# SurrealAI/surreal

Measured on AMD Instinct MI355X. Metric: env-steps/sec (learner ingest) PPO 1024 actors×128 steps, 1/2/4/8 MI355X, higher is better.
Workload: dtype f32

## Files before the change

### include/surreal_amd.h

```cpp
#ifndef SURREAL_AMD_H
#define SURREAL_AMD_H

#include <stddef.h>
#include <stdint.h>

#ifdef __cplusplus
extern "C" {
#endif

typedef void* smx_stream_t;

enum {
    SMX_OK = 0,
    SMX_E_NULL = -1,
    SMX_E_SHAPE = -2,
    SMX_E_UNSUPPORTED = -3,
    SMX_E_WORKSPACE = -4,
    SMX_E_ALIGN = -5
};

enum { SMX_ACT_NONE = 0, SMX_ACT_RELU = 1, SMX_ACT_TANH = 2 };
enum { SMX_PPO_CLIP = 0, SMX_PPO_ADAPT = 1 };

int smx_abi_version(void);
const char* smx_error_string(int code);

typedef struct {
    const float* W1; const float* b1;
    const float* W2; const float* b2;
    const float* W3; const float* b3;
    int32_t D, H1, H2, OUT;
} smx_mlp3_t;

int smx_zfilter_stats_f32(const float* running_sum, const float* running_sumsq,
                          const float* count, int32_t D, float eps,
                          float* mean_out, float* std_out, smx_stream_t stream);
int smx_zfilter_forward_f32(const float* x, int64_t ldx, int64_t rows, int32_t D,
                            const float* mean, const float* std, float* out,
                            smx_stream_t stream);
int smx_zfilter_forward_sums_f32(const float* x, int64_t ldx, int64_t rows, int32_t D,
                                 const float* running_sum, const float* running_sumsq,
                                 const float* count, float eps, float* out, smx_stream_t stream);
int smx_zfilter_update_f32(const float* x, int64_t ldx, int64_t rows, int32_t D,
                           float* running_sum, float* running_sumsq, float* count,
                           float count_rows, smx_stream_t stream);
int64_t smx_zfilter_update_ws_floats(int64_t rows, int32_t D);
int smx_zfilter_update_ws_f32(const float* x, int64_t ldx, int64_t rows, int32_t D, float* running_sum,
                              float* running_sumsq, float* count, float count_rows, float* ws, int64_t ws_floats,
                              smx_stream_t stream);

int smx_mlp3_fused_exact_zfilter(int32_t on);

size_t smx_mlp3_packed_bytes(int32_t D, int32_t H1, int32_t H2, int32_t OUT);
int smx_mlp3_pack_f32(const smx_mlp3_t* net, float* packed, size_t packed_bytes,
                      smx_stream_t stream);
int smx_mlp3_pack_zstats_f32(const smx_mlp3_t* net, float* packed, size_t packed_bytes,
                             const float* running_sum, const float* running_sumsq, const float* count,
                             int32_t D, float eps, float* mean_out, float* std_out, smx_stream_t stream);
int smx_mlp3_forward_fused_f32(const float* packed, int32_t D, int32_t H1, int32_t H2,
                               int32_t OUT, const float* x_main, const float* x_tail,
                               int64_t G, int32_t T0, int32_t T1, const float* zmean,
                               const float* zstd, float* out, int32_t out_act,
                               smx_stream_t stream);

int smx_linear_f32(const float* A, int32_t lda, int32_t a_kcontig, const float* B,
                   int32_t ldb, int32_t b_kcontig, const float* bias, float* C,
                   int32_t ldc, int32_t M, int32_t N, int32_t K, int32_t act,
                   const float* relu_mask, const int32_t* stop_flag, smx_stream_t stream);

typedef struct smx_linear_job {
    int32_t kind, act;
    const float* A; const float* B; const float* bias; const float* relu_mask;
    float* C; float* dbias;
    int32_t lda, ldb, ldc, a_kcontig, b_kcontig, M, N, K;
    const int32_t* stop_flag;
} smx_linear_job_t;
int smx_linear_multi_f32(const smx_linear_job_t* jobs, int32_t njobs, smx_stream_t stream);

int smx_linear_wgrad_f32(const float* dZ, int32_t ldz, const float* X, int32_t ldx, float* dW,
                         int32_t ldw, float* db, int32_t M, int32_t N, int32_t rows,
                         smx_stream_t stream);

int64_t smx_linear_wgrad_ws_floats(int32_t M, int32_t N, int32_t rows);
int smx_linear_wgrad_splitk_f32(const float* dZ, int32_t ldz, const float* X, int32_t ldx,
                                float* dW, int32_t ldw, float* db, int32_t M, int32_t N,
                                int32_t rows, float* ws, int64_t ws_floats, smx_stream_t stream);
int smx_linear_wgrad_splitk_pair_f32(const float* dZ, int32_t ldz, int32_t M, int32_t rows, const float* X1,
                                     int32_t ldx1, float* dW1, float* db1, int32_t N1, const float* X2,
                                     int32_t ldx2, float* dW2, float* db2, int32_t N2, float* ws,
                                     int64_t ws_floats, smx_stream_t stream);

typedef struct {
    const smx_mlp3_t* net;
    const float* x;
    int64_t rows;
    float* h1;
    float* h2;
    float* out;
    int32_t out_act;
    int32_t out_ld;
    const float* dz3;
    float* dz2;
    float* dz1;
    float* grads;
    float* sumsq_partials;
    const int32_t* stop_flag;
    float* h1T;
    float* h2T;
    const float* xT;
    const float* dz3T;
    float* dz2T;
    float* dz1T;
    int64_t ldT;
} smx_mlp3_job_t;
int smx_mlp3_forward_multi_f32(const smx_mlp3_job_t* jobs, int32_t njobs, smx_stream_t stream);
int smx_mlp3_backward_multi_f32(const smx_mlp3_job_t* jobs, int32_t njobs, smx_stream_t stream);

int smx_mlp3_forward_f32(const smx_mlp3_t* net, const float* x, int64_t rows, float* h1,
                         float* h2, float* out, int32_t out_act,
                         const int32_t* stop_flag, smx_stream_t stream);
int32_t smx_mlp3_forward_rows_supported(int32_t D, int32_t H1, int32_t H2, int32_t OUT);
int smx_mlp3_forward_rows_f32(const smx_mlp3_t* net, const float* x, int64_t rows, float* h1, float* h2,
                              float* out, int32_t out_act, int32_t out_ld, float* packed, size_t packed_bytes,
                              const int32_t* stop_flag, smx_stream_t stream);

int32_t smx_mlp3_backward_partials(int32_t D, int32_t H1, int32_t H2, int32_t OUT);
int smx_mlp3_backward_f32(const smx_mlp3_t* net, const float* x, const float* h1,
                          const float* h2, const float* dz3, int64_t rows, float* dz2,
                          float* dz1, float* grads, float* sumsq_partials,
                          const int32_t* stop_flag, smx_stream_t stream);
int64_t smx_mlp3_backward_ws_floats(int32_t D, int32_t H1, int32_t H2, int32_t OUT, int64_t rows);
int smx_mlp3_backward_splitk_f32(const smx_mlp3_t* net, const float* x, const float* h1, const float* h2,
                                 const float* dz3, int64_t rows, float* dz2, float* dz1, float* grads, float* ws,
                                 int64_t ws_floats, const int32_t* stop_flag, smx_stream_t stream);
int32_t smx_mlp3_dgrad_rows_supported(int32_t D, int32_t H1, int32_t H2, int32_t OUT);
int64_t smx_mlp3_dgrad_rows_ws_floats(int32_t D, int32_t H1, int32_t H2, int32_t OUT);
int smx_mlp3_backward_rows_f32(const smx_mlp3_t* net, const float* x, const float* h1, const float* h2,
                               const float* dz3, int64_t rows, float* dz2, float* dz1, float* dx, float* grads,
                               float* ws, int64_t ws_floats, float* packedT, int64_t packedT_floats,
                               const int32_t* stop_flag, smx_stream_t stream);

int smx_windowed_gae_returns_f32(const float* values, const float* values_tail,
                                 const float* rewards,
                                 const float* dones, const float* gamma_pow,
                                 const float* lam_pow, float gamma, float gamma_H,
                                 int32_t B, int32_t N, int32_t H, float* adv, float* ret,
// ... 74 lines not shown
    const float* actions;
    const float* behave;
    const float* ref;
    const float* adv;
    int32_t ld_act, ld_beh, ld_ref, check_stop;
    int64_t rows;
    float* g_surr;
    float* g_kl;
    float* row_partials;
    float* dz3;
    float* dz3_t;
    int64_t ld_t;
    float* dlogvar;
    float* dlogvar_sumsq;
    float* stats;
    const float* values;
    const float* returns;
    float* v_dz3;
    float* v_partials;
    int32_t will_update, v_will_update;
} smx_ppo_losses_t;
int smx_ppo_epoch_losses_f32(const smx_ppo_losses_t* args, smx_ppo_ctrl_t* ctrl,
                             smx_stream_t stream);
int smx_ppo_epoch_losses_dp_f32(const smx_ppo_losses_t* args, int64_t n_total, float* g_surr_t,
                                float* g_kl_t, smx_ppo_ctrl_t* ctrl, smx_stream_t stream);
typedef struct smx_ppo_combine {
    int32_t mode, A;
    const float* row_partials;
    int32_t nblk;
    int32_t check_stop;
    int64_t n_total;
    const float* log_var;
    float* stats;
    float* grads_a;
    const float* grads_kl;
    int64_t n_mlp, n_a;
    float* sumsq_a;
    const float* grads_c;
    int64_t n_c;
    float* sumsq_c;
    int32_t will_update, reserved;
} smx_ppo_combine_t;
int smx_ppo_epoch_combine_f32(const smx_ppo_combine_t* args, smx_ppo_ctrl_t* ctrl,
                              smx_stream_t stream);
int smx_mlp3_wgrad_multi_f32(const smx_mlp3_job_t* jobs, int32_t njobs, smx_stream_t stream);

enum { SMX_EPOCH_LOSS_NONE = 0, SMX_EPOCH_LOSS_POLICY = 1, SMX_EPOCH_LOSS_VALUE = 2, SMX_EPOCH_RHS_SURR = 3,
       SMX_EPOCH_RHS_KL = 4 };
typedef struct smx_epoch_job {
    const smx_mlp3_t* net;
    const float* x;
    int64_t rows;
    float* h1T;
    float* h2T;
    int64_t ldT;
    float* out;
    int32_t out_ld;
    int32_t out_act;
    int32_t loss;
    int32_t reserved;
    const int32_t* stop_flag;
    const float* dz3;
    float* dz3T;
    float* dz2T;
    float* dz1T;
    const float* packed;
} smx_epoch_job_t;
typedef struct smx_epoch_pack {
    const smx_mlp3_t* net;
    float* packed;
} smx_epoch_pack_t;
int64_t smx_epoch_packed_floats(int32_t D, int32_t H1, int32_t H2, int32_t OUT);
int smx_epoch_pack_f32(const smx_epoch_pack_t* items, int32_t n, smx_stream_t stream);
typedef struct smx_epoch_prep {
    const float* obs0; int64_t ld_obs0; int64_t rows; int32_t D; int32_t A;
    const float* zmean; const float* zstd;
    float* xn; float* xnT; int64_t ldT;
    const float* ref_sum; const float* ref_sumsq; const float* ref_count; float ref_eps; int32_t ref_filter;
    float* xr;
    const float* obs_next; int64_t ld_next; float* xnext;
    const float* ref_log_var; float* ref_std; int64_t ld_ref;
    int32_t* zero_words; int32_t n_zero; int32_t n_pack;
    smx_epoch_pack_t pack[4];
} smx_epoch_prep_t;
int smx_epoch_prepare_f32(const smx_epoch_prep_t* args, smx_stream_t stream);
struct smx_ppo_losses;
int32_t smx_epoch_blocks(int64_t rows);
int32_t smx_epoch_supported(int32_t D, int32_t H1, int32_t H2, int32_t OUT);
int smx_epoch_forward_f32(const smx_epoch_job_t* jobs, int32_t njobs, const struct smx_ppo_losses* loss,
                          smx_ppo_ctrl_t* ctrl, int64_t n_total, smx_stream_t stream);
int smx_epoch_backward_f32(const smx_epoch_job_t* jobs, int32_t njobs, const struct smx_ppo_losses* loss,
                           smx_ppo_ctrl_t* ctrl, int64_t n_total, smx_stream_t stream);
int32_t smx_epoch_fwdbwd_supported(int32_t D, int32_t H1, int32_t H2, int32_t OUT);
int smx_epoch_fwdbwd_f32(const smx_epoch_job_t* jobs, int32_t njobs, const struct smx_ppo_losses* loss,
                         smx_ppo_ctrl_t* ctrl, int64_t n_total, int32_t* sync_word, uint64_t* kl_slots,
                         smx_stream_t stream);
int smx_device_occupy(int32_t blocks, int64_t microseconds, smx_stream_t stream);

int smx_diaggauss_sample_f32(const float* mean, int64_t ld_mean, const float* log_var,
                             const float* noise_scale, const float* eps, int64_t ld_eps,
                             int64_t rows, int32_t A, float* actions, int64_t ld_act, float* pd,
                             int64_t ld_pd, smx_stream_t stream);
int smx_ppo_final_stats_f32(const float* log_var, int32_t A, const float* running_sum,
                            const float* running_sumsq, const float* count, int32_t D, float* out4,
                            smx_stream_t stream);
int smx_value_loss_finalize_f32(const float* partials, int32_t count, int32_t nblk,
                                float* stats, int32_t stats_stride, smx_stream_t stream);

int smx_clip_adam_step_f32(float* theta, const float* grads, float* exp_avg,
                           float* exp_avg_sq, int64_t n, const float* sumsq_partials,
                           int32_t npart, const smx_ppo_ctrl_t* ctrl, int32_t which,
                           int32_t honour_stop, float* grad_norm_out, smx_stream_t stream);
typedef struct smx_adam_group {
    float* theta;
    const float* grads;
    float* exp_avg;
    float* exp_avg_sq;
    int64_t n;
    const float* sumsq_partials;
    int32_t npart;
    int32_t honour_stop;
    float* grad_norm_out;
    const smx_mlp3_t* pack_net;
    float* packed;
} smx_adam_group_t;
int smx_clip_adam_step_group_f32(const smx_adam_group_t* group, int32_t which, const smx_ppo_ctrl_t* ctrl,
                                 smx_stream_t stream);
int smx_clip_adam_step_pair_f32(const smx_adam_group_t* actor, const smx_adam_group_t* critic,
                                const smx_ppo_ctrl_t* ctrl, smx_stream_t stream);
int32_t smx_sumsq_blocks(int64_t n);
int smx_sumsq_partials_f32(const float* x, int64_t n, float* partials, smx_stream_t stream);

int smx_ring_insert_f32(float* table, int64_t capacity, int32_t width, int64_t cursor,
                        const float* src, int64_t n, smx_stream_t stream);
int smx_gather_rows_f32(const float* table, int64_t capacity, int32_t width,
                        const int64_t* idx, int64_t n, float* dst, smx_stream_t stream);
int smx_uniform_indices(int64_t* idx, int64_t n, int64_t len, uint64_t seed,
                        uint64_t offset, smx_stream_t stream);
int smx_philox4x32_10(const uint32_t* ctr_key, int64_t n, uint32_t* out, smx_stream_t stream);
typedef struct {
    const void* table;
    void* dst;
    int64_t row_bytes;
} smx_gather_job_t;
int smx_uniform_gather_multi(const smx_gather_job_t* jobs, int32_t njobs, int64_t capacity, int64_t rows,
                             const int64_t* idx, int64_t len, uint64_t seed, uint64_t offset, int64_t* idx_out,
                             smx_stream_t stream);

int smx_ring_insert_bytes(void* table, int64_t capacity, int64_t row_bytes, int64_t cursor,
                          const void* src, int64_t n, smx_stream_t stream);
int smx_gather_rows_bytes(const void* table, int64_t capacity, int64_t row_bytes, const int64_t* idx,
                          int64_t n, void* dst, smx_stream_t stream);

int smx_window_emit_f32(const float* src, int32_t actors, int32_t T, int32_t width,
                        int32_t start, int32_t n_step, int32_t stride, int32_t W, float* dst,
                        smx_stream_t stream);
int smx_window_emit_bytes(const void* src, int32_t actors, int32_t T, int64_t row_bytes, int32_t start,
                          int32_t n_step, int32_t stride, int32_t W, void* dst, smx_stream_t stream);

int smx_frame_stack_u8(const void* frames, int32_t actors, int32_t R, int64_t frame_bytes, int32_t n_stack,
                       const int32_t* episode_first, int32_t start, int32_t n_step, int32_t stride, int32_t W,
                       void* dst, smx_stream_t stream);
int smx_synth_frame_u8(const float* s0, int64_t ld_s0, int32_t n, int32_t C, int32_t H, int32_t W, int32_t t,
                       void* dst, int64_t ld_dst, smx_stream_t stream);

int smx_synth_env_step_f32(float* state, const float* init_state, const float* actions,
// ... 197 lines not shown
```

### surreal_amd/_lib.py

```python
import ctypes
import os
from ctypes import (POINTER, Structure, c_char_p, c_double, c_float, c_int32, c_int64, c_size_t,
                    c_uint64, c_void_p)

_HERE = os.path.dirname(os.path.abspath(__file__))
LIB_PATH = os.environ.get('SMX_LIB_PATH') or os.path.join(_HERE, 'libsurreal_amd.so')

SMX_ACT_NONE, SMX_ACT_RELU, SMX_ACT_TANH = 0, 1, 2
SMX_PPO_CLIP, SMX_PPO_ADAPT = 0, 1
SMX_E_UNSUPPORTED = -3
PS_SURR, PS_LOSS, PS_ENTROPY, PS_KL, PS_GRADNORM, PS_LB, PS_ISW, PS_REFBEH, PS_STRIDE = range(9)
VS_LOSS, VS_EXPVAR, VS_GRADNORM = 0, 1, 2
VS_STRIDE = 4


class Mlp3(Structure):
    _fields_ = [('W1', c_void_p), ('b1', c_void_p), ('W2', c_void_p), ('b2', c_void_p),
                ('W3', c_void_p), ('b3', c_void_p),
                ('D', c_int32), ('H1', c_int32), ('H2', c_int32), ('OUT', c_int32)]


class Mlp3Job(Structure):
    _fields_ = [('net', POINTER(Mlp3)), ('x', c_void_p), ('rows', c_int64), ('h1', c_void_p),
                ('h2', c_void_p), ('out', c_void_p), ('out_act', c_int32), ('out_ld', c_int32),
                ('dz3', c_void_p), ('dz2', c_void_p), ('dz1', c_void_p), ('grads', c_void_p),
                ('sumsq_partials', c_void_p), ('stop_flag', c_void_p),
                ('h1T', c_void_p), ('h2T', c_void_p), ('xT', c_void_p), ('dz3T', c_void_p),
                ('dz2T', c_void_p), ('dz1T', c_void_p), ('ldT', c_int64)]


class EpochJob(Structure):
    _fields_ = [('net', POINTER(Mlp3)), ('x', c_void_p), ('rows', c_int64), ('h1T', c_void_p),
                ('h2T', c_void_p), ('ldT', c_int64), ('out', c_void_p), ('out_ld', c_int32),
                ('out_act', c_int32), ('loss', c_int32), ('reserved', c_int32), ('stop_flag', c_void_p),
                ('dz3', c_void_p), ('dz3T', c_void_p), ('dz2T', c_void_p), ('dz1T', c_void_p),
                ('packed', c_void_p)]


class EpochPack(Structure):
    _fields_ = [('net', POINTER(Mlp3)), ('packed', c_void_p)]


class LearnEpilogue(Structure):
    _fields_ = [('x', c_void_p), ('ldx', c_int64), ('rows', c_int64), ('D', c_int32), ('A', c_int32),
                ('running_sum', c_void_p), ('running_sumsq', c_void_p), ('count', c_void_p), ('count_rows', c_float),
                ('n_epochs', c_int32), ('ret', c_void_p), ('n_ret', c_int64), ('ret_moments', c_void_p),
                ('v_partials', c_void_p), ('nblk', c_int32), ('stats_stride', c_int32), ('v_stats', c_void_p),
                ('log_var', c_void_p), ('out4', c_void_p), ('ticket', c_void_p)]


class EpochPrep(Structure):
    _fields_ = [('obs0', c_void_p), ('ld_obs0', c_int64), ('rows', c_int64), ('D', c_int32), ('A', c_int32),
                ('zmean', c_void_p), ('zstd', c_void_p), ('xn', c_void_p), ('xnT', c_void_p), ('ldT', c_int64),
                ('ref_sum', c_void_p), ('ref_sumsq', c_void_p), ('ref_count', c_void_p), ('ref_eps', c_float),
                ('ref_filter', c_int32), ('xr', c_void_p), ('obs_next', c_void_p), ('ld_next', c_int64),
                ('xnext', c_void_p), ('ref_log_var', c_void_p), ('ref_std', c_void_p), ('ld_ref', c_int64),
                ('zero_words', c_void_p), ('n_zero', c_int32), ('n_pack', c_int32), ('pack', EpochPack * 4)]


EPOCH_LOSS_NONE, EPOCH_LOSS_POLICY, EPOCH_LOSS_VALUE, EPOCH_RHS_SURR, EPOCH_RHS_KL = 0, 1, 2, 3, 4


class Lstm(Structure):
    _fields_ = [('W_ih', c_void_p), ('W_hh', c_void_p), ('b_ih', c_void_p), ('b_hh', c_void_p),
                ('D', c_int32), ('H', c_int32)]


class AdamGroup(Structure):
    _fields_ = [('theta', c_void_p), ('grads', c_void_p), ('exp_avg', c_void_p),
                ('exp_avg_sq', c_void_p), ('n', c_int64), ('sumsq_partials', c_void_p),
                ('npart', c_int32), ('honour_stop', c_int32), ('grad_norm_out', c_void_p),
                ('pack_net', POINTER(Mlp3)), ('packed', c_void_p)]


class PpoLosses(Structure):
    _fields_ = [('mode', c_int32), ('A', c_int32), ('mean', c_void_p), ('log_var', c_void_p),
                ('actions', c_void_p), ('behave', c_void_p), ('ref', c_void_p), ('adv', c_void_p),
                ('ld_act', c_int32), ('ld_beh', c_int32), ('ld_ref', c_int32), ('check_stop', c_int32),
                ('rows', c_int64), ('g_surr', c_void_p), ('g_kl', c_void_p),
                ('row_partials', c_void_p), ('dz3', c_void_p), ('dz3_t', c_void_p), ('ld_t', c_int64),
                ('dlogvar', c_void_p), ('dlogvar_sumsq', c_void_p), ('stats', c_void_p),
                ('values', c_void_p), ('returns', c_void_p), ('v_dz3', c_void_p),
                ('v_partials', c_void_p), ('will_update', c_int32), ('v_will_update', c_int32)]


class PpoCombine(Structure):
    _fields_ = [('mode', c_int32), ('A', c_int32), ('row_partials', c_void_p), ('nblk', c_int32),
                ('check_stop', c_int32), ('n_total', c_int64), ('log_var', c_void_p),
                ('stats', c_void_p), ('grads_a', c_void_p), ('grads_kl', c_void_p),
                ('n_mlp', c_int64), ('n_a', c_int64), ('sumsq_a', c_void_p), ('grads_c', c_void_p),
                ('n_c', c_int64), ('sumsq_c', c_void_p), ('will_update', c_int32),
                ('reserved', c_int32)]


class LinearJob(Structure):
    _fields_ = [('kind', c_int32), ('act', c_int32), ('A', c_void_p), ('B', c_void_p), ('bias', c_void_p),
                ('relu_mask', c_void_p), ('C', c_void_p), ('dbias', c_void_p), ('lda', c_int32), ('ldb', c_int32),
                ('ldc', c_int32), ('a_kcontig', c_int32), ('b_kcontig', c_int32), ('M', c_int32), ('N', c_int32),
                ('K', c_int32), ('stop_flag', c_void_p)]


class DdpgNet(Structure):
    _fields_ = [(n, c_void_p) for n in ('W1', 'b1', 'W2', 'b2', 'W3', 'b3')]


class DdpgUpdate(Structure):
    _fields_ = ([(n, c_void_p) for n in ('theta', 'grads', 'exp_avg', 'exp_avg_sq', 'target')] + [('n', c_int64)] +
                [(n, c_void_p) for n in ('lr', 'step')] +
                [(n, c_float) for n in ('weight_decay', 'clip_value', 'tau')] + [('interval', c_int32), ('stats', c_void_p), ('stats_host', c_void_p)])


class DdpgRows(Structure):
    _fields_ = ([('rows', c_int64)] + [(n, c_int32) for n in ('D', 'A', 'H1', 'H2', 'c1', 'c2')] +
                [(n, DdpgNet) for n in ('actor', 'critic', 'target_actor', 'target_critic')] +
                [(n, c_void_p) for n in ('packed', 'x', 'x_next', 'actions', 'rewards', 'dones')] +
                [('gamma_n', c_float)] +
                [(n, c_void_p) for n in ('xcat', 'h2c', 'q', 'q_next', 'y', 'dz3', 'dz2', 'dxcat', 'h1a', 'h2a', 'act',
                                         'q_actor', 'dz3a', 'dz2a', 'dz1a', 'step')])


class GatherJob(Structure):
    _fields_ = [('table', c_void_p), ('dst', c_void_p), ('row_bytes', c_int64)]


class SynthRollout(Structure):
    _fields_ = [('net', POINTER(Mlp3)), ('packed', c_void_p), ('out_act', c_int32), ('n', c_int32),
                ('log_var', c_void_p), ('noise_scale', c_void_p), ('eps', c_void_p), ('zsum', c_void_p),
                ('zsumsq', c_void_p), ('zcount', c_void_p), ('zeps', c_float), ('t', c_int32),
                ('episode_len', c_int32), ('steps', c_int32), ('rows_per_actor', c_int32), ('slot', c_int32),
                ('state', c_void_p), ('init_state', c_void_p), ('obs_roll', c_void_p), ('act_roll', c_void_p),
                ('rew_roll', c_void_p), ('done_roll', c_void_p), ('pd_roll', c_void_p), ('obs_last', c_void_p)]


class Xchg(Structure):
    _fields_ = [('world', c_int32), ('rank', c_int32), ('capacity', c_int64), ('peer', c_void_p * 8)]


class SynthActStep(Structure):
    _fields_ = [('state', c_void_p), ('init_state', c_void_p), ('mean', c_void_p), ('log_var', c_void_p),
                ('noise_scale', c_void_p), ('eps', c_void_p), ('ld_mean', c_int64), ('ld_eps', c_int64),
                ('n', c_int32), ('D', c_int32), ('A', c_int32), ('t', c_int32), ('episode_len', c_int32),
                ('slot', c_int32), ('T', c_int32), ('reserved', c_int32),
                ('obs_roll', c_void_p), ('act_roll', c_void_p), ('rew_roll', c_void_p),
                ('done_roll', c_void_p), ('pd_roll', c_void_p), ('zsum', c_void_p), ('zsumsq', c_void_p),
                ('zcount', c_void_p), ('zeps', c_float), ('reserved_f', c_float), ('xn_out', c_void_p)]


CTRL_WORDS = 16
(C_LR_ACTOR, C_LR_CRITIC, C_BETA, C_ETA, C_CLIP_EPS, C_KL_TARGET, C_ACTOR_MAX_NORM,
 C_CRITIC_MAX_NORM, C_ACTOR_WD, C_CRITIC_WD, C_STEP_ACTOR, C_STEP_CRITIC, C_STOP,
 C_EPOCHS_DONE) = range(14)
C_XCHG_ERR = 14
C_SYNC_ERR = 15

_P = c_void_p
_SIGS = {
    'smx_abi_version': (c_int32, []),
    'smx_error_string': (c_char_p, [c_int32]),
    'smx_zfilter_stats_f32': (c_int32, [_P, _P, _P, c_int32, c_float, _P, _P, _P]),
    'smx_zfilter_forward_f32': (c_int32, [_P, c_int64, c_int64, c_int32, _P, _P, _P, _P]),
    'smx_zfilter_forward_sums_f32': (c_int32, [_P, c_int64, c_int64, c_int32, _P, _P, _P, c_float, _P, _P]),
    'smx_diaggauss_sample_f32': (c_int32, [_P, c_int64, _P, _P, _P, c_int64, c_int64, c_int32, _P,
                                           c_int64, _P, c_int64, _P]),
    'smx_zfilter_update_f32': (c_int32, [_P, c_int64, c_int64, c_int32, _P, _P, _P, c_float, _P]),
    'smx_mlp3_packed_bytes': (c_size_t, [c_int32, c_int32, c_int32, c_int32]),
    'smx_mlp3_pack_f32': (c_int32, [POINTER(Mlp3), _P, c_size_t, _P]),
    'smx_mlp3_pack_zstats_f32': (c_int32, [POINTER(Mlp3), _P, c_size_t, _P, _P, _P, c_int32, c_float, _P, _P, _P]),
    'smx_mlp3_fused_exact_zfilter': (c_int32, [c_int32]),
    'smx_mlp3_forward_fused_f32': (c_int32, [_P, c_int32, c_int32, c_int32, c_int32, _P, _P,
                                             c_int64, c_int32, c_int32, _P, _P, _P, c_int32, _P]),
    'smx_linear_f32': (c_int32, [_P, c_int32, c_int32, _P, c_int32, c_int32, _P, _P, c_int32,
                                 c_int32, c_int32, c_int32, c_int32, _P, _P, _P]),
    'smx_linear_wgrad_f32': (c_int32, [_P, c_int32, _P, c_int32, _P, c_int32, _P, c_int32, c_int32,
                                       c_int32, _P]),
    'smx_mlp3_forward_f32': (c_int32, [POINTER(Mlp3), _P, c_int64, _P, _P, _P, c_int32, _P, _P]),
    'smx_mlp3_forward_multi_f32': (c_int32, [POINTER(Mlp3Job), c_int32, _P]),
    'smx_mlp3_backward_multi_f32': (c_int32, [POINTER(Mlp3Job), c_int32, _P]),
    'smx_mlp3_wgrad_multi_f32': (c_int32, [POINTER(Mlp3Job), c_int32, _P]),
    'smx_epoch_blocks': (c_int32, [c_int64]),
    'smx_epoch_supported': (c_int32, [c_int32, c_int32, c_int32, c_int32]),
    'smx_epoch_packed_floats': (c_int64, [c_int32, c_int32, c_int32, c_int32]),
    'smx_epoch_pack_f32': (c_int32, [POINTER(EpochPack), c_int32, _P]),
    'smx_epoch_prepare_f32': (c_int32, [POINTER(EpochPrep), _P]),
    'smx_epoch_forward_f32': (c_int32, [POINTER(EpochJob), c_int32, POINTER(PpoLosses), _P, c_int64, _P]),
    'smx_epoch_backward_f32': (c_int32, [POINTER(EpochJob), c_int32, POINTER(PpoLosses), _P, c_int64, _P]),
    'smx_epoch_fwdbwd_supported': (c_int32, [c_int32, c_int32, c_int32, c_int32]),
    'smx_epoch_fwdbwd_f32': (c_int32, [POINTER(EpochJob), c_int32, POINTER(PpoLosses), _P, c_int64, _P, _P, _P]),
    'smx_device_occupy': (c_int32, [c_int32, c_int64, _P]),
    'smx_layernorm_forward_f32': (c_int32, [_P, c_int64, c_int64, c_int32, _P, _P, c_float, _P, c_int64, _P, _P, _P]),
    'smx_layernorm_backward_ws_floats': (c_int64, [c_int64, c_int32]),
    'smx_layernorm_backward_f32': (c_int32, [_P, c_int64, _P, c_int64, _P, _P, _P, c_int64, c_int32, c_int32, _P, c_int64, _P, _P,
                                             _P, c_int64, _P]),
    'smx_zfilter_update_ws_floats': (c_int64, [c_int64, c_int32]),
    'smx_zfilter_update_ws_f32': (c_int32, [_P, c_int64, c_int64, c_int32, _P, _P, _P, c_float, _P, c_int64, _P]),
    'smx_ppo_partials_fold_f32': (c_int32, [_P, c_int32, c_int32, _P, c_int32, _P, _P]),
    'smx_mlp3_forward_rows_supported': (c_int32, [c_int32, c_int32, c_int32, c_int32]),
    'smx_mlp3_forward_rows_f32': (c_int32, [POINTER(Mlp3), _P, c_int64, _P, _P, _P, c_int32, c_int32, _P, c_size_t, _P, _P]),
    'smx_mlp3_backward_partials': (c_int32, [c_int32, c_int32, c_int32, c_int32]),
    'smx_mlp3_backward_f32': (c_int32, [POINTER(Mlp3), _P, _P, _P, _P, c_int64, _P, _P, _P, _P,
                                        _P, _P]),
    'smx_mlp3_backward_ws_floats': (c_int64, [c_int32, c_int32, c_int32, c_int32, c_int64]),
    'smx_mlp3_backward_splitk_f32': (c_int32, [POINTER(Mlp3), _P, _P, _P, _P, c_int64, _P, _P, _P, _P, c_int64, _P, _P]),
    'smx_mlp3_dgrad_rows_supported': (c_int32, [c_int32, c_int32, c_int32, c_int32]),
    'smx_mlp3_dgrad_rows_ws_floats': (c_int64, [c_int32, c_int32, c_int32, c_int32]),
    'smx_mlp3_backward_rows_f32': (c_int32, [POINTER(Mlp3), _P, _P, _P, _P, c_int64, _P, _P, _P, _P, _P, c_int64, _P, c_int64,
                                             _P, _P]),
    'smx_windowed_gae_returns_f32': (c_int32, [_P, _P, _P, _P, _P, _P, c_float, c_float, c_int32,
                                               c_int32, c_int32, _P, _P, _P]),
    'smx_windowed_gae_norm_f32': (c_int32, [_P, _P, _P, _P, _P, _P, c_float, c_float, c_int32, c_int32, c_int32, _P, _P, _P,
                                            c_float, _P, _P]),
    'smx_ppo_learn_epilogue_f32': (c_int32, [POINTER(LearnEpilogue), _P]),
    'smx_reward_filter_f32': (c_int32, [_P, c_int64, c_float, c_int32, _P, c_float, c_int32, _P, _P, _P, _P, _P]),
    'smx_reward_filter_partials': (c_int32, []),
    'smx_moments_f32': (c_int32, [_P, c_int64, _P, _P]),
    'smx_moments_merge_f32': (c_int32, [_P, c_int32, _P, _P]),
    'smx_adv_normalize_f32': (c_int32, [_P, c_int64, _P, c_float, _P]),
    'smx_ppo_loss_blocks': (c_int32, [c_int64]),
    'smx_ppo_loss_partial_stride': (c_int32, [c_int32]),
    'smx_ppo_policy_loss_f32': (c_int32, [c_int32, _P, _P, _P, c_int32, _P, c_int32, _P, c_int32,
                                          _P, c_int64, c_int32, _P, _P, _P, _P, _P]),
    'smx_ppo_loss_finalize_f32': (c_int32, [c_int32, _P, c_int32, _P, _P, _P, c_int64, c_int64,
                                            c_int32, _P, c_int32, c_int32, _P, _P, c_int64, _P, _P,
                                            _P, _P]),
    'smx_ppo_epoch_losses_f32': (c_int32, [POINTER(PpoLosses), _P, _P]),
    'smx_ppo_epoch_losses_dp_f32': (c_int32, [POINTER(PpoLosses), c_int64, _P, _P, _P, _P]),
    'smx_ppo_epoch_combine_f32': (c_int32, [POINTER(PpoCombine), _P, _P]),
    'smx_ppo_final_stats_f32': (c_int32, [_P, c_int32, _P, _P, _P, c_int32, _P, _P]),
    'smx_value_loss_blocks': (c_int32, [c_int64]),
    'smx_value_loss_f32': (c_int32, [_P, _P, c_int64, c_int64, _P, _P, _P, c_int32, _P]),
    'smx_value_loss_finalize_f32': (c_int32, [_P, c_int32, c_int32, _P, c_int32, _P]),
    'smx_clip_adam_step_f32': (c_int32, [_P, _P, _P, _P, c_int64, _P, c_int32, _P, c_int32,
                                         c_int32, _P, _P]),
    'smx_clip_adam_step_group_f32': (c_int32, [POINTER(AdamGroup), c_int32, _P, _P]),
    'smx_clip_adam_step_pair_f32': (c_int32, [POINTER(AdamGroup), POINTER(AdamGroup), _P, _P]),
    'smx_sumsq_blocks': (c_int32, [c_int64]),
    'smx_sumsq_partials_f32': (c_int32, [_P, c_int64, _P, _P]),
    'smx_synth_act_env_step_head_f32': (c_int32, [POINTER(SynthActStep), _P, _P, _P, c_int64, c_int32, c_int32, _P]),
    'smx_conv_u8_forward_f32': (c_int32, [_P, c_int64, c_int32, c_int32, c_int32, c_int32, c_int32, _P, _P, c_int32,
                                          _P, _P, _P]),
    'smx_conv_u8_wgrad_ws_floats': (c_int64, [c_int32, c_int32]),
    'smx_conv_u8_wgrad_f32': (c_int32, [_P, c_int64, c_int32, c_int32, c_int32, c_int32, c_int32, _P, c_int32, _P, _P, _P,
                                        c_int64, _P, _P]),
    'smx_conv_cl_forward_f32': (c_int32, [_P, c_int64, c_int32, c_int32, c_int32, c_int32, c_int32, _P, _P, c_int32,
                                          _P, _P, _P]),
    'smx_conv_cl_wgrad_ws_floats': (c_int64, [c_int32, c_int32]),
    'smx_conv_cl_wgrad_f32': (c_int32, [_P, c_int64, c_int32, c_int32, c_int32, c_int32, c_int32, _P, c_int32, _P, _P, _P,
                                        c_int64, _P, _P]),
    'smx_conv_cl_dgrad_f32': (c_int32, [_P, c_int64, c_int32, c_int32, c_int32, c_int32, c_int32, _P, c_int32, _P, _P,
                                        _P, _P]),
    'smx_ring_insert_bytes': (c_int32, [_P, c_int64, c_int64, c_int64, _P, c_int64, _P]),
    'smx_gather_rows_bytes': (c_int32, [_P, c_int64, c_int64, _P, c_int64, _P, _P]),
    'smx_window_emit_bytes': (c_int32, [_P, c_int32, c_int32, c_int64, c_int32, c_int32, c_int32, c_int32, _P, _P]),
    'smx_ring_insert_f32': (c_int32, [_P, c_int64, c_int32, c_int64, _P, c_int64, _P]),
# ... 124 lines not shown
```

### surreal_amd/csrc/smx_epoch.hip

```cpp
#include "smx_common.h"
#include <stdlib.h>
#include <string.h>

#define SMX_LDS_BARRIER() asm volatile("s_waitcnt lgkmcnt(0)\n\ts_barrier" ::: "memory")

namespace {
#include "smx_ppo_loss.inc.h"
#include "smx_epoch_pack.inc.h"
#include "smx_epoch_mma.inc.h"

constexpr int TB = 3;
constexpr int MAX_EJOBS = 4;
constexpr int XV = 7;
constexpr int LIN = 6;
constexpr int LINF = 3;
constexpr int EXCLUSIVE_LDS = 84 * 1024;
constexpr int LDZ = 68;
constexpr int LDO = 36;
static_assert(ER == LOSS_ROWS_PER_BLOCK, "a row block is a loss block");
static_assert(NTH == 256, "the shared loss code strides by 256 threads");

#ifdef SMX_EPOCH_TIMING
#define TSTAMP(i) do { if (G.tbuf && threadIdx.x == 0) G.tbuf[(size_t)ts_blk * 32 + (i)] = (long long)__builtin_readcyclecounter(); } while (0)
#else
#define TSTAMP(i) do { } while (0)
#endif
struct EJob {
    const float *W1, *b1, *W2, *b2, *W3, *b3;
    int D, H1, H2, OUT;
    const float* x;
    int rows;
    float *h1T, *h2T;
    long ldT;
    float* out;
    int out_ld, out_act, loss, blk_base;
    const int* stop;
    const float* dz3;
    float *dz3T, *dz2T, *dz1T;
    const float *P1, *P2, *P3, *P2T, *P3T;
};

struct PolArgs {
    int mode, A;
    const float *log_var, *actions, *behave, *ref, *adv;
    int ld_act, ld_beh, ld_ref, check_stop, will_update;
    float *g_surr, *g_kl, *row_partials;
    float *dlogvar, *dlogvar_sumsq, *stats;
};

struct ValArgs {
    const float* returns;
    float *v_dz3, *v_partials;
    int will_update;
};

struct EArgs {
    EJob j[MAX_EJOBS];
    int n;
    PolArgs pl;
    ValArgs vl;
    long n_total;
    int ldx, ldh1, ldh2, off_h1, off_h2, off_out, off_red, off_loss;
    int off_g;
    int* sync;
    int nb_pol;
    const int* pol_stop;
    unsigned long long* kl_slots;
    int fsplit;
    int xsplit;
    long long* tbuf;
};

__device__ __forceinline__ int xcd_job_order(const EArgs& G, int raw) {
    const int nb = G.xsplit;
    if (nb == 0) return raw;
    const int xcd = raw & 7, slot = raw >> 3;
    return (xcd >> 2) * nb + slot * 4 + (xcd & 3);
}

__device__ __forceinline__ EJob select_job(const EArgs& G, int bid) {
    int pi = 0;
#pragma unroll
    for (int k = 1; k < MAX_EJOBS; ++k) pi += (k < G.n && bid >= G.j[k].blk_base) ? 1 : 0;
// ... 627 lines not shown
#pragma unroll
            for (int g = 0; g < TB; ++g) {
                if (g < nt) {
                    const int f0 = 16 * (t0 + ts * g) + 4 * kq;
                    float4 v;
                    v.x = (mk[g][0] > 0.f) ? acc[g][0] : 0.f;
                    v.y = (mk[g][1] > 0.f) ? acc[g][1] : 0.f;
                    v.z = (mk[g][2] > 0.f) ? acc[g][2] : 0.f;
                    v.w = (mk[g][3] > 0.f) ? acc[g][3] : 0.f;
                    if (out_lds) *(float4*)(out_lds + fm * ldh2 + f0) = v;
                    const bool ok = outT != nullptr && f0 < M && fm < nrows;
                    const unsigned o = ((unsigned)f0 * (unsigned)J.ldT + (unsigned)(row0 + fm)) * 4u, st = (unsigned)J.ldT * 4u;
                    __builtin_amdgcn_raw_buffer_store_b32(__float_as_uint(v.x), rout, ok ? o : OOB, 0, 0);
                    __builtin_amdgcn_raw_buffer_store_b32(__float_as_uint(v.y), rout, ok ? o + st : OOB, 0, 0);
                    __builtin_amdgcn_raw_buffer_store_b32(__float_as_uint(v.z), rout, ok ? o + 2 * st : OOB, 0, 0);
                    __builtin_amdgcn_raw_buffer_store_b32(__float_as_uint(v.w), rout, ok ? o + 3 * st : OOB, 0, 0);
                }
            }
        }
        TSTAMP(10 + 4 * l);
        SMX_LDS_BARRIER();
        TSTAMP(4 + l);
    }
}

inline int r64(int v) { return (v + 63) & ~63; }

struct PackNet {
    const float *W1, *W2, *W3;
    float* packed;
    int D, H1, H2, OUT;
    long base;
};
struct PackArgs {
    PackNet n[MAX_EJOBS];
    int count;
    long total;
};

__device__ __forceinline__ void pack_word(const PackArgs& P, long i) {
    int pi = 0;
#pragma unroll
    for (int k = 1; k < MAX_EJOBS; ++k) pi += (k < P.count && i >= P.n[k].base) ? 1 : 0;
    const PackNet N = P.n[pi];
    long w = i - N.base;
    int bn = 0;
#pragma unroll
    for (int k = 1; k < 5; ++k) bn += (w >= pack_off(N.D, N.H1, N.H2, N.OUT, k)) ? 1 : 0;
    w -= pack_off(N.D, N.H1, N.H2, N.OUT, bn);
    const float* W = bn == 0 ? N.W1 : ((bn == 1 || bn == 3) ? N.W2 : N.W3);
    const bool tr = bn >= 3;
    const int M = bn == 0 ? N.H1 : (bn == 1 ? N.H2 : (bn == 2 ? N.OUT : (bn == 3 ? N.H1 : N.H2)));
    const int K = bn == 0 ? N.D : (bn == 1 ? N.H1 : (bn == 2 ? N.H2 : (bn == 3 ? N.H2 : N.OUT)));
    const int C2 = pack_chunks(K);
    const int lane = (int)(w & 63), half = (int)((w >> 6) & 1);
    const long tc = w >> 7;
    const int c = (int)(tc % C2), t = (int)(tc / C2);
    const int m = 16 * t + (lane & 15), k = 32 * c + 8 * (lane >> 4) + 4 * half;
    float v[4] = {0.f, 0.f, 0.f, 0.f};
    if (m < M) {
#pragma unroll
        for (int r = 0; r < 4; ++r)
            if (k + r < K) v[r] = tr ? W[(size_t)(k + r) * M + m] : W[(size_t)m * K + k + r];
    }
    *(float4*)(N.packed + 4 * (i - N.base)) = make_float4(v[0], v[1], v[2], v[3]);
}

__global__ __launch_bounds__(256) void epoch_pack_kernel(PackArgs P) {
    const long i = (long)blockIdx.x * 256 + threadIdx.x;
    if (i < P.total) pack_word(P, i);
}

struct PrepArgs {
    const float* obs0; long ld_obs0; long rows; int D;
    const float *zmean, *zstd;
    float *xn, *xnT; long ldT;
    const float *rsum, *rsumsq, *rcount; float reps; int ref_filter;
    float* xr;
    const float* obs_next; long ld_next; float* xnext;
    const float* ref_log_var; int A; float* ref_std; long ld_ref;
    int* zero_words; int n_zero;
    PackArgs pack;
    long n_x, n_std;
};

__device__ __forceinline__ float zclamp_e(float x, float m, float sdev) {
    float v = (x - m) / sdev;
    if (v == v) v = fminf(fmaxf(v, -5.0f), 5.0f);
    return v;
}

__global__ __launch_bounds__(256) void epoch_prepare_kernel(PrepArgs P) {
    const long tid0 = (long)blockIdx.x * 256 + threadIdx.x, stride = (long)gridDim.x * 256;
    for (long i = tid0; i < P.n_zero; i += stride) P.zero_words[i] = 0;
    const long nx = P.n_x, n_next = P.xnext ? nx : 0;
    const long total = 2 * nx + n_next + P.n_std + P.pack.total;
    for (long i = tid0; i < total; i += stride) {
        if (i < 2 * nx + n_next) {
            const int which = i < nx ? 0 : (i < 2 * nx ? 1 : 2);
            const long e = i - (which == 0 ? 0 : (which == 1 ? nx : 2 * nx));
            const long r = e / P.D;
            const int k = (int)(e - r * P.D);
            const float x = which == 2 ? P.obs_next[r * P.ld_next + k] : P.obs0[r * P.ld_obs0 + k];
            float v = x;
            if (which == 1) {
                if (P.ref_filter) {
                    const float c = P.rcount[0];
                    const float m = P.rsum[k] / c;
                    const float var = P.rsumsq[k] / c - m * m;
                    float sd = sqrtf(var);
                    if (sd == sd) sd = fmaxf(sd, P.reps);
                    v = zclamp_e(x, m, sd);
                }
                P.xr[e] = v;
            } else {
                if (P.zmean) v = zclamp_e(x, P.zmean[k], P.zstd[k]);
                if (which == 0) {
                    P.xn[e] = v;
                    if (P.xnT) P.xnT[(size_t)k * P.ldT + r] = v;
                } else {
                    P.xnext[e] = v;
                }
            }
        } else if (i < 2 * nx + n_next + P.n_std) {
            const long e = i - (2 * nx + n_next);
            const long r = e / P.A;
            const int a = (int)(e - r * P.A);
            P.ref_std[r * P.ld_ref + a] = expf(P.ref_log_var[a]);
        } else {
            pack_word(P.pack, i - (2 * nx + n_next + P.n_std));
        }
    }
}

long long* g_tbuf = nullptr;

}

extern "C" int64_t smx_epoch_packed_floats(int32_t D, int32_t H1, int32_t H2, int32_t OUT) {
    return 4 * pack_off(D, H1, H2, OUT, 5);
}

static int fill_pack(PackArgs& P, const smx_epoch_pack_t* items, int32_t n) {
    SMX_REQUIRE(items, SMX_E_NULL);
    SMX_REQUIRE(n >= 1 && n <= MAX_EJOBS, SMX_E_SHAPE);
    P.count = n;
    long base = 0;
    for (int k = 0; k < n; ++k) {
        SMX_REQUIRE(items[k].net && items[k].packed, SMX_E_NULL);
        const smx_mlp3_t& m = *items[k].net;
        SMX_REQUIRE(m.D > 0 && m.H1 > 0 && m.H2 > 0 && m.OUT > 0, SMX_E_SHAPE);
        SMX_REQUIRE(((uintptr_t)items[k].packed & 15) == 0, SMX_E_ALIGN);
        P.n[k].W1 = m.W1; P.n[k].W2 = m.W2; P.n[k].W3 = m.W3; P.n[k].packed = items[k].packed;
        P.n[k].D = m.D; P.n[k].H1 = m.H1; P.n[k].H2 = m.H2; P.n[k].OUT = m.OUT;
        P.n[k].base = base;
        base += smx_epoch_packed_floats(m.D, m.H1, m.H2, m.OUT) / 4;
    }
    P.total = base;
    return SMX_OK;
}

extern "C" int smx_epoch_pack_f32(const smx_epoch_pack_t* items, int32_t n, smx_stream_t stream) {
    PackArgs P;
    const int rc = fill_pack(P, items, n);
    if (rc) return rc;
    hipLaunchKernelGGL(epoch_pack_kernel, dim3((unsigned)((P.total + 255) / 256)), dim3(256), 0, smx_s(stream), P);
    SMX_LAUNCH_CHECK();
    return SMX_OK;
}

extern "C" int smx_epoch_prepare_f32(const smx_epoch_prep_t* a, smx_stream_t stream) {
    SMX_REQUIRE(a && a->obs0 && a->xn && a->xr, SMX_E_NULL);
    SMX_REQUIRE(a->rows > 0 && a->D > 0 && a->ld_obs0 >= a->D, SMX_E_SHAPE);
    SMX_REQUIRE((a->zmean == nullptr) == (a->zstd == nullptr), SMX_E_NULL);
    SMX_REQUIRE(!a->xnT || a->ldT >= a->rows, SMX_E_SHAPE);
    SMX_REQUIRE(!a->ref_filter || (a->ref_sum && a->ref_sumsq && a->ref_count), SMX_E_NULL);
    SMX_REQUIRE(!a->xnext || (a->obs_next && a->ld_next >= a->D), SMX_E_SHAPE);
    SMX_REQUIRE(!a->ref_std || (a->ref_log_var && a->A > 0 && a->ld_ref >= a->A), SMX_E_SHAPE);
    SMX_REQUIRE(a->n_zero >= 0 && a->n_zero <= (1 << 20) && (a->n_zero == 0 || a->zero_words), SMX_E_SHAPE);
    PrepArgs P;
    memset(&P, 0, sizeof(P));
    P.obs0 = a->obs0; P.ld_obs0 = (long)a->ld_obs0; P.rows = (long)a->rows; P.D = a->D;
    P.zmean = a->zmean; P.zstd = a->zstd; P.xn = a->xn; P.xnT = a->xnT; P.ldT = (long)a->ldT;
    P.rsum = a->ref_sum; P.rsumsq = a->ref_sumsq; P.rcount = a->ref_count; P.reps = a->ref_eps;
    P.ref_filter = a->ref_filter; P.xr = a->xr;
    P.obs_next = a->obs_next; P.ld_next = (long)a->ld_next; P.xnext = a->xnext;
    P.ref_log_var = a->ref_log_var; P.A = a->A; P.ref_std = a->ref_std; P.ld_ref = (long)a->ld_ref;
    P.zero_words = a->zero_words; P.n_zero = a->n_zero;
    P.n_x = P.rows * P.D;
    P.n_std = a->ref_std ? P.rows * a->A : 0;
    P.pack.count = 0; P.pack.total = 0;
    if (a->n_pack > 0) {
        const int rc = fill_pack(P.pack, a->pack, a->n_pack);
        if (rc) return rc;
    }
    const long total = 2 * P.n_x + (P.xnext ? P.n_x : 0) + P.n_std + P.pack.total;
    long blocks = (total + 255) / 256;
    if (blocks > 4096) blocks = 4096;
    hipLaunchKernelGGL(epoch_prepare_kernel, dim3((unsigned)blocks), dim3(256), 0, smx_s(stream), P);
    SMX_LAUNCH_CHECK();
    return SMX_OK;
}

extern "C" void smx_epoch_debug_tbuf(void* p) { g_tbuf = (long long*)p; }

extern "C" int32_t smx_epoch_blocks(int64_t rows) { return (int32_t)((rows + ER - 1) / ER); }

static int fwd_lds_bytes(int D, int H1, int H2, int A) {
    const int floats = ER * (r64(D) + 4) + ER * (r64(H1) + 4) + ER * (r64(H2) + 4) + ER * LDO + NWV * 2 * 256 +
                       loss_scratch_floats(A) + ER * (5 * A + 1);
    return floats * (int)sizeof(float);
}
static int fb_loss_floats(int A) {
    const int a = loss_scratch_floats(A) + ER * (5 * A + 1), b = FIN_CH * (8 + 2 * A);
    return a > b ? a : b;
}
static int fb_lds_bytes(int D, int H1, int H2, int A) {
    const int floats = ER * (r64(D) + 4) + ER * (r64(H1) + 4) + ER * (r64(H2) + 4) + ER * LDO + 2 * ER * LDZ +
                       ER * (r64(H2) + 4) + NWV * 2 * 256 + fb_loss_floats(A);
    return floats * (int)sizeof(float);
}
constexpr int MAX_LDS = 128 * 1024;

extern "C" int32_t smx_epoch_supported(int32_t D, int32_t H1, int32_t H2, int32_t OUT) {
    return D > 0 && H1 > 0 && H2 > 0 && OUT > 0 && H1 % 4 == 0 && H2 % 4 == 0 && OUT <= 32 &&
           D <= 2048 && H1 <= 16 * NWV * TG * 2 && H2 <= 16 * NWV * TG * 2 &&
           fwd_lds_bytes(D, H1, H2, OUT) <= MAX_LDS;
}

extern "C" int32_t smx_epoch_fwdbwd_supported(int32_t D, int32_t H1, int32_t H2, int32_t OUT) {
    return smx_epoch_supported(D, H1, H2, OUT) && H2 <= 16 * FNWV * FTG && fb_lds_bytes(D, H1, H2, OUT) <= MAX_LDS;
}

enum { KIND_FWD = 0, KIND_BWD = 1, KIND_FB = 2 };

static int fill_args(EArgs& G, const smx_epoch_job_t* jobs, int32_t njobs, const smx_ppo_losses_t* loss,
                     int64_t n_total, int fsplit, int kind) {
    const bool backward = kind == KIND_BWD;
    SMX_REQUIRE(jobs, SMX_E_NULL);
    SMX_REQUIRE(njobs >= 1 && njobs <= MAX_EJOBS, SMX_E_SHAPE);
    memset(&G, 0, sizeof(G));
    G.n = njobs;
    G.n_total = n_total;
    G.fsplit = fsplit;
    G.tbuf = g_tbuf;
    int base = 0, maxD = 0, maxH1 = 0, maxH2 = 0, A = 0;
    for (int k = 0; k < njobs; ++k) {
        const smx_epoch_job_t& s = jobs[k];
        SMX_REQUIRE(s.net && s.x, SMX_E_NULL);
        const smx_mlp3_t& n = *s.net;
        SMX_REQUIRE(smx_epoch_supported(n.D, n.H1, n.H2, n.OUT), SMX_E_UNSUPPORTED);
        SMX_REQUIRE(s.rows > 0 && s.rows < (1 << 30), SMX_E_SHAPE);
        SMX_REQUIRE(((n.D & 3) || ((uintptr_t)s.x & 15) == 0) && ((uintptr_t)n.W1 & 3) == 0 &&
                        ((uintptr_t)n.W2 & 15) == 0 && ((uintptr_t)n.W3 & 15) == 0 && ((uintptr_t)n.b1 & 15) == 0 &&
                        ((uintptr_t)n.b2 & 15) == 0,
                    SMX_E_ALIGN);
        SMX_REQUIRE((!s.h1T && !s.h2T) || (s.h1T && s.h2T && s.ldT >= s.rows), SMX_E_SHAPE);
        EJob& J = G.j[k];
        J.W1 = n.W1; J.b1 = n.b1; J.W2 = n.W2; J.b2 = n.b2; J.W3 = n.W3; J.b3 = n.b3;
        J.D = n.D; J.H1 = n.H1; J.H2 = n.H2; J.OUT = n.OUT;
        J.x = s.x; J.rows = (int)s.rows; J.h1T = s.h1T; J.h2T = s.h2T; J.ldT = (long)s.ldT;
        J.out = s.out; J.out_ld = s.out_ld ? s.out_ld : n.OUT; J.out_act = s.out_act; J.loss = s.loss;
        J.stop = s.stop_flag;
        J.dz3 = s.dz3; J.dz3T = s.dz3T; J.dz2T = s.dz2T; J.dz1T = s.dz1T;

        {
            SMX_REQUIRE(s.packed, SMX_E_NULL);
            SMX_REQUIRE(((uintptr_t)s.packed & 15) == 0, SMX_E_ALIGN);
            J.P1 = s.packed;
            J.P2 = s.packed + 4 * pack_off(n.D, n.H1, n.H2, n.OUT, 1);
            J.P3 = s.packed + 4 * pack_off(n.D, n.H1, n.H2, n.OUT, 2);
            J.P2T = s.packed + 4 * pack_off(n.D, n.H1, n.H2, n.OUT, 3);
            J.P3T = s.packed + 4 * pack_off(n.D, n.H1, n.H2, n.OUT, 4);
        }
        J.blk_base = base;
        base += smx_epoch_blocks(s.rows) * fsplit;
        if (s.loss == SMX_EPOCH_RHS_SURR || s.loss == SMX_EPOCH_RHS_KL) {
            SMX_REQUIRE(backward, SMX_E_UNSUPPORTED);
            SMX_REQUIRE(loss && loss->g_surr && loss->g_kl && s.dz3T, SMX_E_NULL);
// ... 181 lines not shown
```

### surreal_amd/csrc/smx_mlp3_fused.hip

```cpp
#include "smx_common.h"
#include "smx_mlp3_fused.inc.h"
#include <stdlib.h>
#include <string.h>

namespace {

constexpr int ROWS_PER_WG = 128;
constexpr int LDS_STRIDE = 36;

inline bool pick_variant(int H1, int H2, int* nt1, int* nt2) {
    if (H1 <= 64 && H2 <= 64) { *nt1 = 2; *nt2 = 2; return true; }
    if (H1 <= 320 && H2 <= 224) { *nt1 = 10; *nt2 = 7; return true; }
    return false;
}

__device__ __forceinline__ float zf(float x, float m, float s) {
    float v = (x - m) / s;
    if (v == v) v = fminf(fmaxf(v, -5.0f), 5.0f);
    return v;
}

__device__ __forceinline__ float relu_f(float v) { return (v < 0.f) ? 0.f : v; }

#define MFMA32(a, b, c) __builtin_amdgcn_mfma_f32_32x32x2f32((a), (b), (c), 0, 0, 0)


template <int NT>
__device__ __forceinline__ void load_w(float4 (&wreg)[NT], const float* chunk, int srow, int sk8) {
    const float4* src = reinterpret_cast<const float4*>(chunk);
#pragma unroll
    for (int i = 0; i < NT; ++i) wreg[i] = src[(srow + 32 * i) * 8 + sk8];
}
template <int NT>
__device__ __forceinline__ void store_w(const float4 (&wreg)[NT], float* Wb, int srow, int sk8) {
#pragma unroll
    for (int i = 0; i < NT; ++i)
        *reinterpret_cast<float4*>(Wb + (srow + 32 * i) * LDS_STRIDE + 4 * sk8) = wreg[i];
}

template <bool HASZ>
__device__ __forceinline__ void load_x_vec(float4 (&xreg)[4], float4& zm, float4& zs,
                                           const float* const (&xp)[4], const float* zmean,
                                           const float* zstd, int k0, int D) {
    const int kc = (k0 < D) ? k0 : D - 4;
#pragma unroll
    for (int i = 0; i < 4; ++i) xreg[i] = *reinterpret_cast<const float4*>(xp[i] + kc);
    if (HASZ) {
        zm = *reinterpret_cast<const float4*>(zmean + kc);
        zs = *reinterpret_cast<const float4*>(zstd + kc);
    }
}

template <bool HASZ>
__device__ __forceinline__ void store_x_vec(float* Xb, const float4 (&xreg)[4], const float4 zm,
                                            const float4 zs, const bool (&xok)[4], int k0, int D,
                                            int srow, int sk4) {
    const bool kin = k0 < D;
#pragma unroll
    for (int i = 0; i < 4; ++i) {
        float4 v = xreg[i];
        const bool ok = xok[i] && kin;
        if (HASZ) {
            float a = (v.x - zm.x) * (1.0f / zs.x), b = (v.y - zm.y) * (1.0f / zs.y);
            float c = (v.z - zm.z) * (1.0f / zs.z), d = (v.w - zm.w) * (1.0f / zs.w);
            if (a == a) a = fminf(fmaxf(a, -5.0f), 5.0f);
            if (b == b) b = fminf(fmaxf(b, -5.0f), 5.0f);
            if (c == c) c = fminf(fmaxf(c, -5.0f), 5.0f);
            if (d == d) d = fminf(fmaxf(d, -5.0f), 5.0f);
            v.x = ok ? a : 0.f;
            v.y = ok ? b : 0.f;
            v.z = ok ? c : 0.f;
            v.w = ok ? d : 0.f;
        } else if (!ok) {
            v = make_float4(0.f, 0.f, 0.f, 0.f);
        }
        *reinterpret_cast<float4*>(Xb + (srow + 32 * i) * LDS_STRIDE + sk4) = v;
    }
}

__device__ __forceinline__ float zf_mul(float x, float m, float r) {
    float v = (x - m) * r;
    if (v == v) v = fminf(fmaxf(v, -5.0f), 5.0f);
    return v;
}

template <bool HASZ>
__device__ __forceinline__ void stage_x(float* dst, float4 v, const float4 zm, const float4 rz,
                                        const bool ok) {
    if (HASZ) {
        const float a = zf_mul(v.x, zm.x, rz.x), b = zf_mul(v.y, zm.y, rz.y);
        const float c = zf_mul(v.z, zm.z, rz.z), d = zf_mul(v.w, zm.w, rz.w);
        v.x = ok ? a : 0.f;
        v.y = ok ? b : 0.f;
        v.z = ok ? c : 0.f;
        v.w = ok ? d : 0.f;
    } else if (!ok) {
        v = make_float4(0.f, 0.f, 0.f, 0.f);
// ... 242 lines not shown
            SMX_WST(4, v4); SMX_WST(5, v5); SMX_WST(6, v6);
#undef SMX_WLD
#undef SMX_WST
        }
        __syncthreads();
    }
#pragma unroll
    for (int u = 0; u < NT2; ++u)
#pragma unroll
        for (int g = 0; g < 4; ++g) {
            const float4 bb = *reinterpret_cast<const float4*>(b2s + 32 * u + 8 * g + 4 * kh);
            acc2[u][4 * g + 0] = relu_f(acc2[u][4 * g + 0] + bb.x);
            acc2[u][4 * g + 1] = relu_f(acc2[u][4 * g + 1] + bb.y);
            acc2[u][4 * g + 2] = relu_f(acc2[u][4 * g + 2] + bb.z);
            acc2[u][4 * g + 3] = relu_f(acc2[u][4 * g + 3] + bb.w);
        }

    const long myrow = row0 + wv * 32 + j;
    if (OUT1) {
        float v = 0.f;
#pragma unroll
        for (int u = 0; u < NT2; ++u)
#pragma unroll
            for (int g = 0; g < 4; ++g) {
                const float4 ww = *reinterpret_cast<const float4*>(w3s + 32 * u + 8 * g + 4 * kh);
                v = fmaf(acc2[u][4 * g + 0], ww.x, v);
                v = fmaf(acc2[u][4 * g + 1], ww.y, v);
                v = fmaf(acc2[u][4 * g + 2], ww.z, v);
                v = fmaf(acc2[u][4 * g + 3], ww.w, v);
            }
        v += __shfl_xor(v, 32, 64);
        v += A.packed[L.b3];
        if (A.out_act == SMX_ACT_TANH) v = tanhf(v);
        if (kh == 0 && myrow < A.total_rows) A.out[myrow] = v;
    } else {
        f32x16 acc3;
#pragma unroll
        for (int s = 0; s < 16; ++s) acc3[s] = 0.f;
        {
            const float4* src = reinterpret_cast<const float4*>(W3p);
#pragma unroll
            for (int u = 0; u < NT2; ++u) {
                const float4 t4 = src[(u * 32 + srow) * 8 + sk8];
                *reinterpret_cast<float4*>(Wb0 + (u * 32 + srow) * LDS_STRIDE + sk4) = t4;
            }
        }
        __syncthreads();
        const float* wrow = Wb0 + j * LDS_STRIDE + 4 * kh;
#pragma unroll
        for (int u = 0; u < NT2; ++u)
#pragma unroll
            for (int q = 0; q < 4; ++q) {
                const float4 a = *reinterpret_cast<const float4*>(wrow + u * 32 * LDS_STRIDE + 8 * q);
                acc3 = MFMA32(a.x, acc2[u][4 * q + 0], acc3);
                acc3 = MFMA32(a.y, acc2[u][4 * q + 1], acc3);
                acc3 = MFMA32(a.z, acc2[u][4 * q + 2], acc3);
                acc3 = MFMA32(a.w, acc2[u][4 * q + 3], acc3);
            }
        if (myrow < A.total_rows) {
#pragma unroll
            for (int s = 0; s < 16; ++s) {
                const int o = 8 * (s >> 2) + 4 * kh + (s & 3);
                if (o < A.OUT) {
                    float v = acc3[s] + w3s[o];
                    if (A.out_act == SMX_ACT_TANH) v = tanhf(v);
                    else if (A.out_act == SMX_ACT_RELU) v = relu_f(v);
                    A.out[myrow * A.OUT + o] = v;
                }
            }
        }
    }
}

struct ZStatsRider {
    const float *rs, *rsq, *cnt;
    float *mean, *stdv;
    int D;
    float eps;
};

__global__ __launch_bounds__(256) void mlp3_pack_kernel(smx_mlp3_t net, float* __restrict__ packed,
                                                        int NT1, int NT2, int KC1, ZStatsRider Z) {
    if (Z.rs) {
        for (int k = blockIdx.x * 256 + threadIdx.x; k < Z.D; k += gridDim.x * 256) {
            const float c = Z.cnt[0];
            const float m = Z.rs[k] / c;
            const float var = Z.rsq[k] / c - m * m;
            float sd = sqrtf(var);
            if (sd == sd) sd = fmaxf(sd, Z.eps);
            Z.mean[k] = m;
            Z.stdv[k] = sd;
        }
    }
    const PackLayout L = pack_layout(NT1, NT2, KC1);
    for (size_t i = (size_t)blockIdx.x * 256 + threadIdx.x; i < L.total; i += (size_t)gridDim.x * 256) {
        float v = 0.f;
        if (i < L.b1) {
            const size_t e = i - L.w1;
            const int kk = (int)(e & 31);
            const size_t rc = e >> 5;
            const int f = (int)(rc % (size_t)(NT1 * 32)), c = (int)(rc / (size_t)(NT1 * 32));
            const int k = 32 * c + kk;
            if (f < net.H1 && k < net.D) v = net.W1[(size_t)f * net.D + k];
        } else if (i < L.w2) {
            const int f = (int)(i - L.b1);
            if (f < net.H1) v = net.b1[f];
        } else if (i < L.b2) {
            const size_t e = i - L.w2;
            const int kk = (int)(e & 31);
            const size_t rc = e >> 5;
            const int f = (int)(rc % (size_t)(NT2 * 32)), c = (int)(rc / (size_t)(NT2 * 32));
            const int k = 32 * c + kk;
            if (f < net.H2 && k < net.H1) v = net.W2[(size_t)f * net.H1 + k];
        } else if (i < L.w3) {
            const int f = (int)(i - L.b2);
            if (f < net.H2) v = net.b2[f];
        } else if (i < L.b3) {
            const size_t e = i - L.w3;
            const int kk = (int)(e & 31);
            const size_t rc = e >> 5;
            const int o = (int)(rc & 31), c = (int)(rc >> 5);
            const int k = 32 * c + kk;
            if (o < net.OUT && k < net.H2) v = net.W3[(size_t)o * net.H2 + k];
        } else {
            const int o = (int)(i - L.b3);
            if (o < net.OUT) v = net.b3[o];
        }
        packed[i] = v;
    }
}

template <int NT1, int NT2>
int launch_fused(const FusedArgs& A, hipStream_t st) {
    constexpr int WR = (NT1 > NT2 ? NT1 : NT2) * 32;
    const size_t lds = (size_t)(2 * WR * LDS_STRIDE + 2 * ROWS_PER_WG * LDS_STRIDE + NT1 * 32 +
                                NT2 * 32 + NT2 * 32) * sizeof(float);
    const unsigned grid = (unsigned)((A.total_rows + ROWS_PER_WG - 1) / ROWS_PER_WG);
    const int xmode = (NT1 > 2 && A.xvec && A.D >= 4) ? (A.zmean ? 1 : 2) : 0;
    void (*k)(FusedArgs) = nullptr;
    if (A.OUT == 1) {
        k = xmode == 1 ? mlp3_fused_kernel<NT1, NT2, true, (NT1 > 2 ? 1 : 0)>
          : xmode == 2 ? mlp3_fused_kernel<NT1, NT2, true, (NT1 > 2 ? 2 : 0)>
                       : mlp3_fused_kernel<NT1, NT2, true, 0>;
    } else {
        k = xmode == 1 ? mlp3_fused_kernel<NT1, NT2, false, (NT1 > 2 ? 1 : 0)>
          : xmode == 2 ? mlp3_fused_kernel<NT1, NT2, false, (NT1 > 2 ? 2 : 0)>
                       : mlp3_fused_kernel<NT1, NT2, false, 0>;
    }
    hipError_t e = hipFuncSetAttribute((const void*)k, hipFuncAttributeMaxDynamicSharedMemorySize,
                                       (int)lds);
    if (e != hipSuccess) return (int)e;
    hipLaunchKernelGGL(k, dim3(grid), dim3(256), lds, st, A);
    e = hipGetLastError();
    return e == hipSuccess ? SMX_OK : (int)e;
}

}

static int g_exact_zfilter = 0;
extern "C" int smx_mlp3_fused_exact_zfilter(int32_t on) {
    g_exact_zfilter = on ? 1 : 0;
    return SMX_OK;
}

static long long* g_fused_tbuf = nullptr;
extern "C" void smx_mlp3_fused_debug_tbuf(void* p) { g_fused_tbuf = (long long*)p; }

extern "C" size_t smx_mlp3_packed_bytes(int32_t D, int32_t H1, int32_t H2, int32_t OUT) {
    int nt1, nt2;
    if (D <= 0 || OUT <= 0 || OUT > 32 || !pick_variant(H1, H2, &nt1, &nt2)) return 0;
    return pack_layout(nt1, nt2, (D + 31) / 32).total * sizeof(float);
}

static int pack_launch(const smx_mlp3_t* net, float* packed, size_t packed_bytes, const ZStatsRider& Z,
                       smx_stream_t stream) {
    SMX_REQUIRE(net && packed && net->W1 && net->b1 && net->W2 && net->b2 && net->W3 && net->b3,
                SMX_E_NULL);
    SMX_REQUIRE(net->D > 0 && net->H1 > 0 && net->H2 > 0 && net->OUT > 0, SMX_E_SHAPE);
    int nt1, nt2;
    SMX_REQUIRE(net->OUT <= 32 && pick_variant(net->H1, net->H2, &nt1, &nt2), SMX_E_UNSUPPORTED);
    const int KC1 = (net->D + 31) / 32;
    const PackLayout L = pack_layout(nt1, nt2, KC1);
    SMX_REQUIRE(packed_bytes >= L.total * sizeof(float), SMX_E_WORKSPACE);
    SMX_REQUIRE(((uintptr_t)packed & 15) == 0, SMX_E_ALIGN);
    unsigned blocks = (unsigned)((L.total + 255) / 256);
    if (blocks > 1024) blocks = 1024;
    hipLaunchKernelGGL(mlp3_pack_kernel, dim3(blocks), dim3(256), 0, smx_s(stream), *net, packed, nt1,
                       nt2, KC1, Z);
    SMX_LAUNCH_CHECK();
    return SMX_OK;
}

extern "C" int smx_mlp3_pack_f32(const smx_mlp3_t* net, float* packed, size_t packed_bytes,
                                 smx_stream_t stream) {
    ZStatsRider Z;
    memset(&Z, 0, sizeof(Z));
    return pack_launch(net, packed, packed_bytes, Z, stream);
}

extern "C" int smx_mlp3_pack_zstats_f32(const smx_mlp3_t* net, float* packed, size_t packed_bytes,
                                        const float* running_sum, const float* running_sumsq,
                                        const float* count, int32_t D, float eps, float* mean_out,
                                        float* std_out, smx_stream_t stream) {
    SMX_REQUIRE(running_sum && running_sumsq && count && mean_out && std_out, SMX_E_NULL);
    SMX_REQUIRE(D > 0, SMX_E_SHAPE);
    ZStatsRider Z;
    Z.rs = running_sum; Z.rsq = running_sumsq; Z.cnt = count; Z.mean = mean_out; Z.stdv = std_out;
    Z.D = D; Z.eps = eps;
    return pack_launch(net, packed, packed_bytes, Z, stream);
}

extern "C" int smx_mlp3_forward_fused_f32(const float* packed, int32_t D, int32_t H1, int32_t H2,
                                          int32_t OUT, const float* x_main, const float* x_tail,
                                          int64_t G, int32_t T0, int32_t T1, const float* zmean,
                                          const float* zstd, float* out, int32_t out_act,
                                          smx_stream_t stream) {
    SMX_REQUIRE(packed && x_main && out, SMX_E_NULL);
    SMX_REQUIRE(T1 == 0 || x_tail, SMX_E_NULL);
    SMX_REQUIRE((zmean == nullptr) == (zstd == nullptr), SMX_E_NULL);
    SMX_REQUIRE(G > 0 && T0 > 0 && T1 >= 0 && D > 0 && OUT > 0, SMX_E_SHAPE);
    int nt1, nt2;
    SMX_REQUIRE(OUT <= 32 && pick_variant(H1, H2, &nt1, &nt2), SMX_E_UNSUPPORTED);
    SMX_REQUIRE(((uintptr_t)packed & 15) == 0, SMX_E_ALIGN);
    FusedArgs A;
    A.packed = packed;
    A.x_main = x_main;
    A.x_tail = x_tail ? x_tail : x_main;
    A.zmean = zmean;
    A.zstd = zstd;
    A.out = out;
    A.total_rows = (long)G * (T0 + T1);
    A.T0 = T0;
    A.T1 = T1;
    A.D = D;
    A.OUT = OUT;
    A.KC1 = (D + 31) / 32;
    A.out_act = out_act;
    A.tbuf = g_fused_tbuf;
    A.exp = 0;
    A.h1_out = A.h2_out = nullptr;
    A.H1 = H1; A.H2 = H2; A.out_ld = OUT;
    A.stop = nullptr;
    A.xvec = (D % 4 == 0) && (((uintptr_t)x_main & 15) == 0) &&
             (T1 == 0 || ((uintptr_t)x_tail & 15) == 0) &&
             (zmean == nullptr || ((((uintptr_t)zmean | (uintptr_t)zstd) & 15) == 0));
    if (nt1 == 2) return launch_fused<2, 2>(A, smx_s(stream));
    static const bool force32 = getenv("SMX_FUSED32") != nullptr;
    if (g_exact_zfilter && zmean) A.xvec = 0;
    if (!force32 && A.xvec) {
        const int rc = smx_rows16_launch(A, H1, H2, smx_s(stream));
        if (rc != SMX_E_UNSUPPORTED) return rc;
    }
    return launch_fused<10, 7>(A, smx_s(stream));
}

extern "C" int32_t smx_mlp3_forward_rows_supported(int32_t D, int32_t H1, int32_t H2, int32_t OUT) {
    int nt1, nt2;
    return D >= 4 && D % 4 == 0 && H1 % 4 == 0 && H2 % 4 == 0 && H1 > 64 && H2 > 64 && OUT >= 1 && OUT <= 32 &&
           pick_variant(H1, H2, &nt1, &nt2) && nt1 > 2;
}

extern "C" int smx_mlp3_forward_rows_f32(const smx_mlp3_t* net, const float* x, int64_t rows, float* h1, float* h2,
                                         float* out, int32_t out_act, int32_t out_ld, float* packed,
                                         size_t packed_bytes, const int32_t* stop_flag, smx_stream_t stream) {
    SMX_REQUIRE(net && x && h1 && h2 && out && packed, SMX_E_NULL);
    SMX_REQUIRE(rows > 0, SMX_E_SHAPE);
    if (!smx_mlp3_forward_rows_supported(net->D, net->H1, net->H2, net->OUT)) return SMX_E_UNSUPPORTED;
    if ((((uintptr_t)x | (uintptr_t)h1 | (uintptr_t)h2) & 15) != 0) return SMX_E_UNSUPPORTED;
    int rc = smx_mlp3_pack_f32(net, packed, packed_bytes, stream);
    if (rc) return rc;
    FusedArgs A;
    A.packed = packed;
    A.x_main = x; A.x_tail = x;
    A.zmean = nullptr; A.zstd = nullptr;
    A.out = out;
    A.total_rows = (long)rows;
    A.T0 = 1; A.T1 = 0;
    A.D = net->D; A.OUT = net->OUT; A.KC1 = (net->D + 31) / 32;
    A.out_act = out_act;
    A.tbuf = nullptr; A.exp = 0; A.xvec = 1;
    A.h1_out = h1; A.h2_out = h2;
    A.H1 = net->H1; A.H2 = net->H2; A.out_ld = out_ld > 0 ? out_ld : net->OUT;
    A.stop = (const int*)stop_flag;
    return smx_rows16_launch(A, net->H1, net->H2, smx_s(stream));
}
```

### surreal_amd/csrc/smx_mlp3_fused.inc.h

```cpp
#pragma once
#include "smx_common.h"

namespace smxf {

struct FusedArgs {
    const float* packed;
    const float* x_main;
    const float* x_tail;
    const float* zmean;
    const float* zstd;
    float* out;
    long total_rows;
    int T0, T1, D, OUT, KC1, out_act, xvec;
    long long* tbuf;
    int exp;
    float* h1_out;
    float* h2_out;
    int H1, H2, out_ld;
    const int* stop;
};

struct PackLayout {
    size_t w1, b1, w2, b2, w3, b3, total;
};

__host__ __device__ inline PackLayout pack_layout(int NT1, int NT2, int KC1) {
    PackLayout L;
    L.w1 = 0;
    L.b1 = L.w1 + (size_t)KC1 * NT1 * 32 * 32;
    L.w2 = L.b1 + (size_t)NT1 * 32;
    L.b2 = L.w2 + (size_t)NT1 * NT2 * 32 * 32;
    L.w3 = L.b2 + (size_t)NT2 * 32;
    L.b3 = L.w3 + (size_t)NT2 * 32 * 32;
    L.total = L.b3 + 32;
    return L;
}

}
using smxf::FusedArgs;
using smxf::PackLayout;
using smxf::pack_layout;

__attribute__((visibility("hidden"))) int smx_rows16_launch(const FusedArgs& A, int H1, int H2, hipStream_t st);
```

### surreal_amd/csrc/smx_mlp3_rows16.hip

```cpp
#include "smx_mlp3_fused.inc.h"

namespace {

constexpr int ROWS16 = 128;
constexpr int LDS16 = 36;
constexpr int NTHR = 512;

#ifdef SMX_FUSED_TIMING
#define TSTAMP(i) do { if (A.tbuf && threadIdx.x == 0) A.tbuf[(size_t)blockIdx.x * 16 + (i)] = (long long)__builtin_readcyclecounter(); } while (0)
#else
#define TSTAMP(i) do { } while (0)
#endif
#define TLOOP(i) do { if (c == 5) TSTAMP(8 + (i)); } while (0)
#ifdef SMX_FUSED_EXP
#define EXP(bit) (SMX_FUSED_EXP & (bit))
#else
#define EXP(bit) 0
#endif
#define MFMA16(a, b, c) __builtin_amdgcn_mfma_f32_16x16x4f32((a), (b), (c), 0, 0, 0)

typedef __amdgpu_buffer_rsrc_t rsrc_t;
typedef unsigned int u32x4 __attribute__((ext_vector_type(4)));

__device__ __forceinline__ rsrc_t make_rsrc(const float* p, unsigned bytes) {
    const uintptr_t u = (uintptr_t)p;
    const unsigned lo = __builtin_amdgcn_readfirstlane((unsigned)u);
    const unsigned hi = __builtin_amdgcn_readfirstlane((unsigned)(u >> 32));
    void* q = (void*)(((uintptr_t)hi << 32) | lo);
    return __builtin_amdgcn_make_buffer_rsrc(q, 0, __builtin_amdgcn_readfirstlane(bytes), 0x00020000);
}
__device__ __forceinline__ float4 ld16(rsrc_t R, unsigned off) {
    const u32x4 w = __builtin_amdgcn_raw_buffer_load_b128(R, off, 0, 0);
    return make_float4(__uint_as_float(w.x), __uint_as_float(w.y), __uint_as_float(w.z), __uint_as_float(w.w));
}

__device__ __forceinline__ float relu16(float v) { return (v < 0.f) ? 0.f : v; }

__device__ __forceinline__ float zf16(float x, float m, float r) {
    float v = (x - m) * r;
    if (v == v) v = fminf(fmaxf(v, -5.0f), 5.0f);
    return v;
}
__device__ __forceinline__ void stage_x16(float* dst, float4 v, const float4 zm, const float4 rz, const bool hasz,
                                          const bool ok) {
    const float a = zf16(v.x, zm.x, rz.x), b = zf16(v.y, zm.y, rz.y);
    const float c = zf16(v.z, zm.z, rz.z), d = zf16(v.w, zm.w, rz.w);
    v.x = ok ? (hasz ? a : v.x) : 0.f;
    v.y = ok ? (hasz ? b : v.y) : 0.f;
    v.z = ok ? (hasz ? c : v.z) : 0.f;
    v.w = ok ? (hasz ? d : v.w) : 0.f;
    *reinterpret_cast<float4*>(dst) = v;
}

template <int NT1, int NT2, bool OUT1, bool SAVE>
__global__ __launch_bounds__(NTHR, 1) void mlp3_rows16_kernel(FusedArgs A) {
    constexpr int P1 = (NT1 + 1) / 2, P2 = (NT2 + 1) / 2;
    constexpr int NW1 = (P1 * 32 + 63) / 64, NW2 = (P2 * 32 + 63) / 64;
    constexpr int WR = 64 * (NW1 > NW2 ? NW1 : NW2);
    static_assert(NW1 <= 5 && NW2 <= 4, "staging registers are written out for <= 5 / <= 4 passes");
    extern __shared__ float lds[];
    if (SAVE && A.stop && *A.stop) return;
    TSTAMP(0);
    float* Wb0 = lds;
    float* Wb1 = Wb0 + WR * LDS16;
    float* Xb0 = Wb1 + WR * LDS16;
    float* Xb1 = Xb0 + ROWS16 * LDS16;
    float* b1s = Xb1 + ROWS16 * LDS16;
    float* b2s = b1s + P1 * 32;
    float* w3s = b2s + P2 * 32;
    float* zms = w3s + P2 * 32;
    float* rzl = zms + A.KC1 * 32;

    const int tid = threadIdx.x, lane = tid & 63, wv = tid >> 6;
    const int fm = lane & 15, g = lane >> 4;
    const long row0 = (long)blockIdx.x * ROWS16;
    const PackLayout L = pack_layout(P1, P2, A.KC1);
    const float* W1p = A.packed + L.w1;
    const float* W2p = A.packed + L.w2;
    const float* W3p = A.packed + L.w3;
    const bool hasz = A.zmean != nullptr;
    const rsrc_t rzm = make_rsrc(A.zmean, hasz ? (unsigned)A.D * 4u : 0u);
    const rsrc_t rzs = make_rsrc(A.zstd, hasz ? (unsigned)A.D * 4u : 0u);

    const int srow = tid >> 3, sk8 = tid & 7, sk4 = sk8 * 4;
    const float* xp0;
    const float* xp1;
    bool xok0, xok1;
    {
        const int T = A.T0 + A.T1;
        auto rowptr = [&](long r, bool& ok) {
            ok = r < A.total_rows;
            const long rr = ok ? r : 0;
            const long gq = rr / T;
            const int tt = (int)(rr - gq * T);
            return (tt < A.T0) ? A.x_main + (gq * A.T0 + tt) * (long)A.D
                               : A.x_tail + (gq * A.T1 + (tt - A.T0)) * (long)A.D;
        };
        xp0 = rowptr(row0 + srow, xok0);
        xp1 = rowptr(row0 + srow + 64, xok1);
    }
    for (int i = tid; i < P1 * 32; i += NTHR) b1s[i] = A.packed[L.b1 + i];
    for (int i = tid; i < P2 * 32; i += NTHR) b2s[i] = A.packed[L.b2 + i];
    for (int k = tid; k < A.KC1 * 32; k += NTHR) {
        const bool in = hasz && k < A.D;
        zms[k] = in ? A.zmean[k] : 0.f;
        rzl[k] = in ? 1.0f / A.zstd[k] : 1.0f;
    }
    const float b3v = A.packed[L.b3];
    if (OUT1) {
        for (int i = tid; i < P2 * 32; i += NTHR) w3s[i] = W3p[(size_t)(i >> 5) * 1024 + (i & 31)];
    } else {
        if (tid < 32) w3s[tid] = A.packed[L.b3 + tid];
    }

#define SMX_WLD(src, i) (src)[(srow + 64 * (i)) * 8 + sk8]
#define SMX_WST(dst, i, v) *reinterpret_cast<float4*>((dst) + (srow + 64 * (i)) * LDS16 + sk4) = (v)

    f32x4 acc1[NT1];
#pragma unroll
    for (int t = 0; t < NT1; ++t) acc1[t] = f32x4{0.f, 0.f, 0.f, 0.f};

    {
        const float4* wsrc = reinterpret_cast<const float4*>(W1p);
        const int kc = (sk4 < A.D) ? sk4 : A.D - 4;
        const float4 x0 = *reinterpret_cast<const float4*>(xp0 + kc);
        const float4 x1 = *reinterpret_cast<const float4*>(xp1 + kc);
        const float4 zm = ld16(rzm, (unsigned)kc * 4u);
        float4 zs = ld16(rzs, (unsigned)kc * 4u);
        const float4 w0 = SMX_WLD(wsrc, 0), w1 = SMX_WLD(wsrc, 1), w2 = SMX_WLD(wsrc, 2), w3 = SMX_WLD(wsrc, 3);
        float4 w4 = w3;
        if (NW1 > 4) w4 = SMX_WLD(wsrc, 4);
        const float4 rz = make_float4(1.0f / zs.x, 1.0f / zs.y, 1.0f / zs.z, 1.0f / zs.w);
        const bool kin = sk4 < A.D;
        stage_x16(Xb0 + srow * LDS16 + sk4, x0, zm, rz, hasz, xok0 && kin);
        stage_x16(Xb0 + (srow + 64) * LDS16 + sk4, x1, zm, rz, hasz, xok1 && kin);
        SMX_WST(Wb0, 0, w0); SMX_WST(Wb0, 1, w1); SMX_WST(Wb0, 2, w2); SMX_WST(Wb0, 3, w3);
        if (NW1 > 4) SMX_WST(Wb0, 4, w4);
    }
    __syncthreads();
    TSTAMP(1);

    constexpr int HA = (NT1 + 1) / 2, HB = NT1 - HA;
    constexpr int A1 = HA / 3, A2 = (2 * HA) / 3, B1 = HB / 3, B2 = (2 * HB) / 3;
    float4 fa[HA], fb[HB], bcur, bnxt;
#define SMX_W1(buf) ((buf) + woff)
#define SMX_RD_A(wrow, h, i0, i1)                                                 \
    _Pragma("unroll") for (int t = (i0); t < (i1); ++t)                           \
        fa[t] = *reinterpret_cast<const float4*>((wrow) + t * 16 * LDS16 + 16 * (h));
#define SMX_RD_B(wrow, h, i0, i1)                                                 \
    _Pragma("unroll") for (int t = (i0); t < (i1); ++t)                           \
        fb[t] = *reinterpret_cast<const float4*>((wrow) + (HA + t) * 16 * LDS16 + 16 * (h));
#define SMX_STEP_A(e)                                                             \
    _Pragma("unroll") for (int t = 0; t < HA; ++t) acc1[t] = MFMA16(fa[t].e, bq.e, acc1[t]);
#define SMX_STEP_B(e)                                                             \
    _Pragma("unroll") for (int t = 0; t < HB; ++t) acc1[HA + t] = MFMA16(fb[t].e, bq.e, acc1[HA + t]);
#define SMX_PIN __builtin_amdgcn_sched_barrier(0)
    const int xoff = (wv * 16 + fm) * LDS16 + 4 * g, woff = fm * LDS16 + 4 * g;

    float4 x0, x1, w0, w1, w2, w3, w4;
    const int last = A.KC1 - 1;
    {
        const int cn = 1 < last ? 1 : last;
        const float4* wsrc = reinterpret_cast<const float4*>(W1p + (size_t)cn * P1 * 1024);
        const int k0n = 32 * cn + sk4;
        const int kc = (k0n < A.D) ? k0n : A.D - 4;
        SMX_PIN; w0 = SMX_WLD(wsrc, 0); SMX_PIN; w1 = SMX_WLD(wsrc, 1); SMX_PIN; w2 = SMX_WLD(wsrc, 2); SMX_PIN;
        w3 = SMX_WLD(wsrc, 3); SMX_PIN;
        w4 = w3;
        if (NW1 > 4) w4 = SMX_WLD(wsrc, 4);
        SMX_PIN;
        x0 = *reinterpret_cast<const float4*>(xp0 + kc); SMX_PIN;
        x1 = *reinterpret_cast<const float4*>(xp1 + kc); SMX_PIN;
    }
    bcur = *reinterpret_cast<const float4*>(Xb0 + xoff);
    SMX_RD_A(SMX_W1(Wb0), 0, 0, HA)
#ifdef SMX_FUSED_PRIO
    if (wv >= 4) __builtin_amdgcn_s_setprio(SMX_FUSED_PRIO);
#endif

    for (int c = 0; c < A.KC1; ++c) {
        const float* Wc = (c & 1) ? Wb1 : Wb0;
        const float* Xc = (c & 1) ? Xb1 : Xb0;
        float* Wn = (c & 1) ? Wb0 : Wb1;
        float* Xn = (c & 1) ? Xb0 : Xb1;
        const int cn = (c + 1 < A.KC1) ? c + 1 : c;
        const int c2 = (c + 2 < A.KC1) ? c + 2 : last;
        const bool kin = 32 * cn + sk4 < A.D;
        const int kc2 = (32 * c2 + sk4 < A.D) ? 32 * c2 + sk4 : A.D - 4;
        SMX_PIN;
        TLOOP(0);
        {
            const float4 bq = bcur;
            SMX_RD_B(SMX_W1(Wc), 0, 0, B1) SMX_PIN;
            SMX_STEP_A(x) SMX_PIN; SMX_RD_B(SMX_W1(Wc), 0, B1, B2) SMX_PIN;
            SMX_STEP_A(y) SMX_PIN; SMX_RD_B(SMX_W1(Wc), 0, B2, HB) SMX_PIN;
// ... 139 lines not shown
        }
        {
            const f32x4 bq = acc1[2 * p];
            SMX_STEP2_B(x, 0) SMX_PIN;
            if (!odd_tail) { SMX_RD2_A(Wc + woff, 1, 0, C1) }
            if (!lastp) { SMX_WST(Wn, 0, v0); SMX_WST(Wn, 1, v1); }
            SMX_PIN;
            SMX_STEP2_B(y, 1) SMX_PIN;
            if (!odd_tail) { SMX_RD2_A(Wc + woff, 1, C1, C2) }
            if (!lastp) { SMX_WST(Wn, 2, v2); if (NW2 > 3) SMX_WST(Wn, 3, v3); }
            SMX_PIN;
            SMX_STEP2_B(z, 2) SMX_PIN;
            if (!odd_tail) { SMX_RD2_A(Wc + woff, 1, C2, UA) }
            SMX_PIN;
            SMX_STEP2_B(w, 3) SMX_PIN;
        }
        if (!odd_tail) {
            const f32x4 bq = acc1[2 * p + 1 < NT1 ? 2 * p + 1 : 0];
            SMX_STEP2_A(x, 0) SMX_PIN; SMX_RD2_B(Wc + woff, 1, 0, D1) SMX_PIN;
            SMX_STEP2_A(y, 1) SMX_PIN; SMX_RD2_B(Wc + woff, 1, D1, D2) SMX_PIN;
            SMX_STEP2_A(z, 2) SMX_PIN; SMX_RD2_B(Wc + woff, 1, D2, UB) SMX_PIN;
            SMX_STEP2_A(w, 3) SMX_PIN;
        }
        if (!lastp) __syncthreads();
        if (!odd_tail) {
            const f32x4 bq = acc1[2 * p + 1 < NT1 ? 2 * p + 1 : 0];
            SMX_STEP2_B(x, 0) SMX_PIN;
            if (!lastp) { SMX_RD2_A(Wn + woff, 0, 0, C1) }
            if (p + 2 < P1) SMX_LD2(p + 2);
            SMX_PIN;
            SMX_STEP2_B(y, 1) SMX_PIN;
            if (!lastp) { SMX_RD2_A(Wn + woff, 0, C1, C2) }
            SMX_PIN;
            SMX_STEP2_B(z, 2) SMX_PIN;
            if (!lastp) { SMX_RD2_A(Wn + woff, 0, C2, UA) }
            SMX_PIN;
            SMX_STEP2_B(w, 3) SMX_PIN;
        } else if (!lastp) {
            SMX_RD2_A(Wn + woff, 0, 0, UA)
            if (p + 2 < P1) SMX_LD2(p + 2);
        }
    }
#undef SMX_RD2_A
#undef SMX_RD2_B
#undef SMX_STEP2_A
#undef SMX_STEP2_B
#undef SMX_LD2
    TSTAMP(4);
#pragma unroll
    for (int u = 0; u < NT2; ++u) {
        const float4 bb = *reinterpret_cast<const float4*>(b2s + 16 * u + 4 * g);
        acc2[u][0] = relu16(acc2[u][0] + bb.x);
        acc2[u][1] = relu16(acc2[u][1] + bb.y);
        acc2[u][2] = relu16(acc2[u][2] + bb.z);
        acc2[u][3] = relu16(acc2[u][3] + bb.w);
    }
    if (SAVE && A.h2_out) {
        const long r = row0 + wv * 16 + fm;
        if (r < A.total_rows) {
            float* dst = A.h2_out + r * (long)A.H2 + 4 * g;
#pragma unroll
            for (int u = 0; u < NT2; ++u)
                if (16 * u + 4 * g < A.H2)
                    *reinterpret_cast<float4*>(dst + 16 * u) = make_float4(acc2[u][0], acc2[u][1], acc2[u][2], acc2[u][3]);
        }
    }

    const long myrow = row0 + wv * 16 + fm;
    if (OUT1) {
        float v = 0.f;
#pragma unroll
        for (int u = 0; u < NT2; ++u) {
            const float4 ww = *reinterpret_cast<const float4*>(w3s + 16 * u + 4 * g);
            v = fmaf(acc2[u][0], ww.x, v);
            v = fmaf(acc2[u][1], ww.y, v);
            v = fmaf(acc2[u][2], ww.z, v);
            v = fmaf(acc2[u][3], ww.w, v);
        }
        v += __shfl_xor(v, 16, 64);
        v += __shfl_xor(v, 32, 64);
        v += b3v;
        if (A.out_act == SMX_ACT_TANH) v = tanhf(v);
        if (g == 0 && myrow < A.total_rows) A.out[SAVE ? myrow * A.out_ld : myrow] = v;
    } else {
        f32x4 acc3 = f32x4{0.f, 0.f, 0.f, 0.f}, acc3b = f32x4{0.f, 0.f, 0.f, 0.f};
        {
            const float4* src = reinterpret_cast<const float4*>(W3p);
            for (int i = tid; i < P2 * 32 * 8; i += NTHR)
                *reinterpret_cast<float4*>(Wb0 + (i >> 3) * LDS16 + 4 * (i & 7)) = src[i];
        }
        __syncthreads();
        const float* wrow = Wb0 + fm * LDS16 + 4 * g;
        const bool two = A.OUT > 16;
#pragma unroll
        for (int u = 0; u < NT2; ++u) {
            const float4 a = *reinterpret_cast<const float4*>(wrow + (u >> 1) * 32 * LDS16 + 16 * (u & 1));
            acc3 = MFMA16(a.x, acc2[u][0], acc3);
            acc3 = MFMA16(a.y, acc2[u][1], acc3);
            acc3 = MFMA16(a.z, acc2[u][2], acc3);
            acc3 = MFMA16(a.w, acc2[u][3], acc3);
        }
        if (two) {
#pragma unroll
            for (int u = 0; u < NT2; ++u) {
                const float4 a = *reinterpret_cast<const float4*>(wrow + ((u >> 1) * 32 + 16) * LDS16 + 16 * (u & 1));
                acc3b = MFMA16(a.x, acc2[u][0], acc3b);
                acc3b = MFMA16(a.y, acc2[u][1], acc3b);
                acc3b = MFMA16(a.z, acc2[u][2], acc3b);
                acc3b = MFMA16(a.w, acc2[u][3], acc3b);
            }
        }
        if (myrow < A.total_rows) {
            const int ld = SAVE ? A.out_ld : A.OUT;
#pragma unroll
            for (int r = 0; r < 8; ++r) {
                const int o = (r < 4) ? 4 * g + r : 16 + 4 * g + (r - 4);
                if (o < A.OUT) {
                    float v = ((r < 4) ? acc3[r & 3] : acc3b[r & 3]) + w3s[o];
                    if (A.out_act == SMX_ACT_TANH) v = tanhf(v);
                    else if (A.out_act == SMX_ACT_RELU) v = relu16(v);
                    A.out[myrow * ld + o] = v;
                }
            }
        }
    }
    TSTAMP(5);
#undef SMX_WLD
#undef SMX_WST
}

template <int NT1, int NT2, bool SAVE>
int launch16(const FusedArgs& A, hipStream_t st) {
    constexpr int P1 = (NT1 + 1) / 2, P2 = (NT2 + 1) / 2;
    constexpr int NW1 = (P1 * 32 + 63) / 64, NW2 = (P2 * 32 + 63) / 64;
    constexpr int WR = 64 * (NW1 > NW2 ? NW1 : NW2);
    const size_t lds = (size_t)(2 * WR * LDS16 + 2 * ROWS16 * LDS16 + P1 * 32 + 2 * P2 * 32 + 2 * A.KC1 * 32) * sizeof(float);
    if (lds > 160 * 1024) return SMX_E_UNSUPPORTED;
    const unsigned grid = (unsigned)((A.total_rows + ROWS16 - 1) / ROWS16);
    void (*k)(FusedArgs) = (A.OUT == 1) ? mlp3_rows16_kernel<NT1, NT2, true, SAVE> : mlp3_rows16_kernel<NT1, NT2, false, SAVE>;
    hipError_t e = hipFuncSetAttribute((const void*)k, hipFuncAttributeMaxDynamicSharedMemorySize, (int)lds);
    if (e != hipSuccess) return (int)e;
    hipLaunchKernelGGL(k, dim3(grid), dim3(NTHR), lds, st, A);
    e = hipGetLastError();
    return e == hipSuccess ? SMX_OK : (int)e;
}

}

int smx_rows16_launch(const FusedArgs& A, int H1, int H2, hipStream_t st) {
    const bool save = A.h1_out || A.h2_out;
    if (!A.xvec || A.D < 4 || A.OUT > 32 || H1 <= 64 || H2 <= 64 || H1 > 320 || H2 > 224) return SMX_E_UNSUPPORTED;
    if (save) {
        if ((H1 | H2) & 3) return SMX_E_UNSUPPORTED;
        if (H1 <= 304 && H2 <= 208) return launch16<19, 13, true>(A, st);
        return launch16<20, 14, true>(A, st);
    }
    if (H1 <= 304 && H2 <= 208) return launch16<19, 13, false>(A, st);
    return launch16<20, 14, false>(A, st);
}
```

### surreal_amd/csrc/smx_scan.hip

```cpp
#include "smx_common.h"
#include "smx_moments.inc.h"

__device__ __forceinline__ void gae_body(
    const float* __restrict__ values, const float* __restrict__ values_tail,
    const float* __restrict__ rewards,
    const float* __restrict__ dones, const float* __restrict__ gpow,
    const float* __restrict__ lpow, float gamma, float gamma_H, int B, int N, int H,
    float* __restrict__ adv, float* __restrict__ ret) {
    extern __shared__ float lds[];
    const int lane = threadIdx.x & 63, w = threadIdx.x >> 6;
    const int b = blockIdx.x * 4 + w;
    const int per = 3 * N + 1;
    float* Vm = lds + (size_t)w * per;
    float* R = Vm + (N + 1);
    float* Dl = R + N;
    if (b < B) {
        const float* v = values + (size_t)b * (values_tail ? N : N + 1);
        const float* r = rewards + (size_t)b * N;
        const float* d = dones + (size_t)b * N;
        const float vt = values_tail ? values_tail[b] : 0.f;
        const int vlast = values_tail ? N - 1 : N;
        for (int t0 = 0; t0 <= N; t0 += 256) {
            float xv[4], dv[4], rv[4];
#pragma unroll
            for (int i = 0; i < 4; ++i) {
                const int t = t0 + lane + 64 * i;
                xv[i] = v[t < vlast ? t : vlast];
                dv[i] = d[t >= 1 ? (t - 1 < N ? t - 1 : N - 1) : 0];
                rv[i] = r[t < N ? t : N - 1];
            }
#pragma unroll
            for (int i = 0; i < 4; ++i) {
                const int t = t0 + lane + 64 * i;
                if (t <= N) {
                    float x = (values_tail && t == N) ? vt : xv[i];
                    if (t >= 1) x = x * (1.0f - dv[i]);
                    Vm[t] = x;
                    if (t < N) R[t] = rv[i];
                }
            }
        }
    }
    __syncthreads();
    if (b < B) {
        for (int t = lane; t < N; t += 64) {
            float gv = gamma * Vm[t + 1];
            float s = R[t] + gv;
            Dl[t] = s - Vm[t];
        }
    }
    __syncthreads();
    if (b < B) {
    const int E = N - H + 1;
    if (E == 1) {
        float rs = 0.f, as = 0.f;
        for (int k = lane; k < N; k += 64) {
            rs += gpow[k] * R[k];
            as += (Dl[k] * gpow[k]) * lpow[k];
        }
        rs = smx_wave_sum(rs);
        as = smx_wave_sum(as);
        if (lane == 0) {
            ret[b] = rs + Vm[N] * gamma_H;
            adv[b] = as;
        }
    } else {
        for (int s = lane; s < E; s += 64) {
            float rs = 0.f, as = 0.f;
            for (int k = 0; k < H; ++k) {
                rs += gpow[k] * R[s + k];
                as += (Dl[s + k] * gpow[k]) * lpow[k];
            }
            ret[(size_t)b * E + s] = rs + Vm[s + H] * gamma_H;
            adv[(size_t)b * E + s] = as;
        }
    }
    }
}

__global__ __launch_bounds__(256) void gae_kernel(
    const float* __restrict__ values, const float* __restrict__ values_tail,
    const float* __restrict__ rewards, const float* __restrict__ dones, const float* __restrict__ gpow,
    const float* __restrict__ lpow, float gamma, float gamma_H, int B, int N, int H,
    float* __restrict__ adv, float* __restrict__ ret) {
    gae_body(values, values_tail, rewards, dones, gpow, lpow, gamma, gamma_H, B, N, H, adv, ret);
}

__device__ __forceinline__ bool last_block_done(int* ticket) {
    __shared__ int is_last;
    __syncthreads();
    if (threadIdx.x == 0) {
        __threadfence();
        const int t = atomicAdd(ticket, 1);
        is_last = (t == (int)gridDim.x - 1);
        if (is_last) *ticket = 0;
        __threadfence();
    }
    __syncthreads();
    return is_last != 0;
}

__device__ __forceinline__ void block_moments(const float* __restrict__ x, long n, float* __restrict__ out) {
    __shared__ double red[16];
    __shared__ double bc;
    const int lane = threadIdx.x & 63, w = threadIdx.x >> 6, nw = (blockDim.x + 63) >> 6;
    double s = 0.0;
    for (long i = threadIdx.x; i < n; i += blockDim.x) s += (double)__builtin_nontemporal_load(x + i);
    s = smx_wave_sum_d(s);
    if (lane == 0) red[w] = s;
    __syncthreads();
    if (threadIdx.x == 0) {
        double t = 0.0;
        for (int i = 0; i < nw; ++i) t += red[i];
        bc = t / (double)n;
    }
    __syncthreads();
    const double mean = bc;
    double q = 0.0;
    for (long i = threadIdx.x; i < n; i += blockDim.x) {
        const double d = (double)__builtin_nontemporal_load(x + i) - mean;
        q += d * d;
    }
    q = smx_wave_sum_d(q);
    __syncthreads();
    if (lane == 0) red[w] = q;
    __syncthreads();
    if (threadIdx.x == 0) {
        double t = 0.0;
        for (int i = 0; i < nw; ++i) t += red[i];
        out[0] = (float)n;
        out[1] = (float)mean;
        out[2] = (float)t;
        bc = t;
    }
    __syncthreads();
}

__global__ __launch_bounds__(256) void gae_norm_kernel(
    const float* __restrict__ values, const float* __restrict__ values_tail,
    const float* __restrict__ rewards, const float* __restrict__ dones, const float* __restrict__ gpow,
    const float* __restrict__ lpow, float gamma, float gamma_H, int B, int N, int H,
    float* __restrict__ adv, float* __restrict__ ret, float* __restrict__ norm_mom, float min_std,
    int* __restrict__ ticket) {
    gae_body(values, values_tail, rewards, dones, gpow, lpow, gamma, gamma_H, B, N, H, adv, ret);
    if (!last_block_done(ticket)) return;
    const long n = (long)B * (N - H + 1);
    block_moments(adv, n, norm_mom);
    const float cnt = (float)n, mean = norm_mom[1], m2 = norm_mom[2];
    const float stdv = sqrtf(m2 / (cnt - 1.0f));
    const float den = (min_std > stdv) ? min_std : stdv;
    for (long i = threadIdx.x; i < n; i += blockDim.x) adv[i] = (__builtin_nontemporal_load(adv + i) - mean) / den;
}

extern "C" int smx_windowed_gae_returns_f32(const float* values, const float* values_tail,
                                            const float* rewards,
                                            const float* dones, const float* gamma_pow,
                                            const float* lam_pow, float gamma, float gamma_H,
                                            int32_t B, int32_t N, int32_t H, float* adv,
                                            float* ret, smx_stream_t stream) {
    SMX_REQUIRE(values && rewards && dones && gamma_pow && lam_pow && adv && ret, SMX_E_NULL);
    SMX_REQUIRE(B > 0 && N > 0 && H > 0 && H <= N, SMX_E_SHAPE);
    const size_t lds = (size_t)4 * (3 * (size_t)N + 1) * sizeof(float);
    SMX_REQUIRE(lds <= 160 * 1024, SMX_E_UNSUPPORTED);
    if (lds > 64 * 1024) {
        hipError_t e = hipFuncSetAttribute((const void*)gae_kernel,
                                           hipFuncAttributeMaxDynamicSharedMemorySize, (int)lds);
        if (e != hipSuccess) return (int)e;
    }
    hipLaunchKernelGGL(gae_kernel, dim3((B + 3) / 4), dim3(256), lds, smx_s(stream), values,
                       values_tail, rewards, dones, gamma_pow, lam_pow, gamma, gamma_H, B, N, H, adv, ret);
    SMX_LAUNCH_CHECK();
    return SMX_OK;
}

extern "C" int smx_windowed_gae_norm_f32(const float* values, const float* values_tail, const float* rewards,
                                         const float* dones, const float* gamma_pow, const float* lam_pow,
                                         float gamma, float gamma_H, int32_t B, int32_t N, int32_t H, float* adv,
                                         float* ret, float* adv_moments, float min_std, int32_t* ticket,
                                         smx_stream_t stream) {
    SMX_REQUIRE(values && rewards && dones && gamma_pow && lam_pow && adv && ret && adv_moments && ticket, SMX_E_NULL);
    SMX_REQUIRE(B > 0 && N > 0 && H > 0 && H <= N, SMX_E_SHAPE);
    const size_t lds = (size_t)4 * (3 * (size_t)N + 1) * sizeof(float);
    SMX_REQUIRE(lds <= 128 * 1024, SMX_E_UNSUPPORTED);
    if (lds > 48 * 1024) {
        hipError_t e = hipFuncSetAttribute((const void*)gae_norm_kernel,
                                           hipFuncAttributeMaxDynamicSharedMemorySize, (int)lds);
        if (e != hipSuccess) return (int)e;
    }
    hipLaunchKernelGGL(gae_norm_kernel, dim3((B + 3) / 4), dim3(256), lds, smx_s(stream), values, values_tail,
                       rewards, dones, gamma_pow, lam_pow, gamma, gamma_H, B, N, H, adv, ret, adv_moments, min_std,
                       (int*)ticket);
    SMX_LAUNCH_CHECK();
    return SMX_OK;
}

constexpr int RF_MAX_BLOCKS = 64;

__global__ __launch_bounds__(256) void reward_filter_kernel(const float* __restrict__ r, long n, float scale, int filter,
                                                            float* __restrict__ state, float eps, int update,
                                                            float* __restrict__ out, float* __restrict__ sums,
                                                            double* __restrict__ partials, int* __restrict__ ticket) {
    __shared__ double red[8];
    float mean = 0.f, sd = 1.f;
    if (filter) {
        const float cnt = state[0];
        mean = state[1] / cnt;
        sd = sqrtf(state[2] / cnt - mean * mean);
        if (sd == sd) sd = fmaxf(sd, eps);
    }
    double s1 = 0.0, s2 = 0.0;
    for (long i = (long)blockIdx.x * 256 + threadIdx.x; i < n; i += (long)gridDim.x * 256) {
        const float x = r[i] * scale;
        float v = x;
        if (filter) {
            v = (x - mean) / sd;
            if (v == v) v = fminf(fmaxf(v, -5.0f), 5.0f);
        }
        out[i] = v;
        s1 += (double)x;
        s2 += (double)x * (double)x;
    }
    const int lane = threadIdx.x & 63, w = threadIdx.x >> 6;
    s1 = smx_wave_sum_d(s1);
    s2 = smx_wave_sum_d(s2);
    if (lane == 0) { red[w] = s1; red[4 + w] = s2; }
    __syncthreads();
    if (threadIdx.x == 0) {
        partials[2 * blockIdx.x] = (red[0] + red[1]) + (red[2] + red[3]);
        partials[2 * blockIdx.x + 1] = (red[4] + red[5]) + (red[6] + red[7]);
    }
    if (!last_block_done(ticket)) return;
    if (threadIdx.x == 0) {
        double t1 = 0.0, t2 = 0.0;
        for (unsigned b = 0; b < gridDim.x; ++b) {
// ... 304 lines not shown

extern "C" int64_t smx_zfilter_update_ws_floats(int64_t rows, int32_t D) {
    if (rows < 16384 || D <= 0) return 0;
    const long chunks = rows / 512 < 256 ? rows / 512 : 256;
    return 2 * chunks * (int64_t)D;
}

extern "C" int smx_zfilter_update_ws_f32(const float* x, int64_t ldx, int64_t rows, int32_t D, float* running_sum,
                                         float* running_sumsq, float* count, float count_rows, float* ws, int64_t ws_floats,
                                         smx_stream_t stream) {
    const int64_t need = smx_zfilter_update_ws_floats(rows, D);
    if (need == 0 || !ws || ws_floats < need)
        return smx_zfilter_update_f32(x, ldx, rows, D, running_sum, running_sumsq, count, count_rows, stream);
    SMX_REQUIRE(x && running_sum && running_sumsq && count, SMX_E_NULL);
    SMX_REQUIRE(rows > 0 && D > 0 && ldx >= D, SMX_E_SHAPE);
    const int chunks = (int)(need / (2 * D));
    hipLaunchKernelGGL(zupdate_part_kernel, dim3((unsigned)chunks, (unsigned)((D + 63) / 64)), dim3(1024), 0, smx_s(stream), x,
                       (long)ldx, (long)rows, D, chunks, ws);
    hipLaunchKernelGGL(zupdate_merge_kernel, dim3((unsigned)((D + 255) / 256)), dim3(256), 0, smx_s(stream), ws, chunks, D,
                       running_sum, running_sumsq, count, count_rows);
    SMX_LAUNCH_CHECK();
    return SMX_OK;
}


struct EpilogueArgs {
    const float* x; long ldx; long rows; int D;
    float *rs, *rsq, *cnt; float count_rows;
    const float* ret; long n_ret; float* ret_mom;
    const float* vpartials; int n_epochs, nblk; float* vstats; int vstride;
    const float* log_var; int A; float* out4;
    int* ticket;
    int nz;
};

__global__ __launch_bounds__(1024) void learn_epilogue_kernel(EpilogueArgs P) {
    __shared__ float s1[16][64], s2[16][64];
    __shared__ double red4[16][4];
    const int blk = blockIdx.x;
    if (blk < P.nz) {
        const int c = threadIdx.x & 63, g = threadIdx.x >> 6;
        const int col = blk * 64 + c;
        float a0 = 0.f, a1 = 0.f, a2 = 0.f, a3 = 0.f, q0 = 0.f, q1 = 0.f, q2 = 0.f, q3 = 0.f;
        if (col < P.D) {
            const float* x = P.x;
            const long ldx = P.ldx, rows = P.rows;
            long r = g;
            for (; r + 240 < rows; r += 256) {
                float v[16];
#pragma unroll
                for (int i = 0; i < 16; ++i) v[i] = x[(r + 16 * i) * ldx + col];
#pragma unroll
                for (int i = 0; i < 16; i += 4) {
                    a0 += v[i]; q0 += v[i] * v[i];
                    a1 += v[i + 1]; q1 += v[i + 1] * v[i + 1];
                    a2 += v[i + 2]; q2 += v[i + 2] * v[i + 2];
                    a3 += v[i + 3]; q3 += v[i + 3] * v[i + 3];
                }
            }
            for (; r + 48 < rows; r += 64) {
                const float v0 = x[r * ldx + col], v1 = x[(r + 16) * ldx + col];
                const float v2 = x[(r + 32) * ldx + col], v3 = x[(r + 48) * ldx + col];
                a0 += v0; q0 += v0 * v0;
                a1 += v1; q1 += v1 * v1;
                a2 += v2; q2 += v2 * v2;
                a3 += v3; q3 += v3 * v3;
            }
            for (; r < rows; r += 16) {
                const float v = x[r * ldx + col];
                a0 += v; q0 += v * v;
            }
        }
        s1[g][c] = (a0 + a1) + (a2 + a3);
        s2[g][c] = (q0 + q1) + (q2 + q3);
        __syncthreads();
        if (g == 0 && col < P.D) {
            float ta = 0.f, tq = 0.f;
            for (int k = 0; k < 16; ++k) { ta += s1[k][c]; tq += s2[k][c]; }
            P.rs[col] += ta;
            P.rsq[col] += tq;
        }
        if (blk == 0 && threadIdx.x == 0) P.cnt[0] += P.count_rows;
    } else if (blk == P.nz) {
        block_moments(P.ret, P.n_ret, P.ret_mom);
    } else {
        const int e = (blk - P.nz - 1) * 16 + (threadIdx.x >> 6);
        if (e < P.n_epochs)
            value_finalize_wave(P.vpartials + (size_t)e * P.nblk * 8, P.nblk, P.vstats + (size_t)e * P.vstride,
                                threadIdx.x & 63);
    }
    if (!last_block_done(P.ticket)) return;
    final_stats_block(P.log_var, P.A, P.nz ? P.rs : nullptr, P.rsq, P.cnt, P.D, P.out4, red4);
}

extern "C" int smx_ppo_learn_epilogue_f32(const smx_learn_epilogue_t* a, smx_stream_t stream) {
    SMX_REQUIRE(a && a->ret && a->ret_moments && a->log_var && a->out4 && a->ticket, SMX_E_NULL);
    SMX_REQUIRE(a->n_ret > 0 && a->A > 0, SMX_E_SHAPE);
    SMX_REQUIRE(!a->x || (a->running_sum && a->running_sumsq && a->count && a->rows > 0 && a->D > 0 && a->ldx >= a->D),
                SMX_E_SHAPE);
    SMX_REQUIRE(a->n_epochs == 0 || (a->v_partials && a->v_stats && a->nblk > 0 && a->stats_stride >= 2), SMX_E_SHAPE);
    SMX_REQUIRE(a->n_epochs == 0 || ((uintptr_t)a->v_partials & 15) == 0, SMX_E_ALIGN);
    EpilogueArgs P;
    P.x = a->x; P.ldx = (long)a->ldx; P.rows = (long)a->rows; P.D = a->D;
    P.rs = a->running_sum; P.rsq = a->running_sumsq; P.cnt = a->count; P.count_rows = a->count_rows;
    P.ret = a->ret; P.n_ret = (long)a->n_ret; P.ret_mom = a->ret_moments;
    P.vpartials = a->v_partials; P.n_epochs = a->n_epochs; P.nblk = a->nblk; P.vstats = a->v_stats;
    P.vstride = a->stats_stride;
    P.log_var = a->log_var; P.A = a->A; P.out4 = a->out4; P.ticket = (int*)a->ticket;
    P.nz = a->x ? (a->D + 63) / 64 : 0;
    const int nv = (a->n_epochs + 15) / 16;
    hipLaunchKernelGGL(learn_epilogue_kernel, dim3(P.nz + 1 + nv), dim3(1024), 0, smx_s(stream), P);
    SMX_LAUNCH_CHECK();
    return SMX_OK;
}

extern "C" int smx_abi_version(void) { return 1; }

extern "C" const char* smx_error_string(int code) {
    switch (code) {
        case SMX_OK: return "ok";
        case SMX_E_NULL: return "required pointer is NULL";
        case SMX_E_SHAPE: return "non-positive or inconsistent dimension";
        case SMX_E_UNSUPPORTED: return "shape outside what the kernel is built for";
        case SMX_E_WORKSPACE: return "workspace too small";
        case SMX_E_ALIGN: return "pointer not 16-byte aligned";
        default: return code > 0 ? hipGetErrorString((hipError_t)code) : "unknown smx error";
    }
}
```

### surreal_amd/kernels.py

```python
import ctypes

import torch

from surreal_amd import _lib as L


def _row_stride(view, width):
    assert view.dim() == 2 and view.shape[1] == width and (width == 1 or view.stride(1) == 1), \
        (tuple(view.shape), view.stride())
    return view.stride(0) if view.shape[0] > 1 else max(view.stride(0), width)


class HipKernels(object):
    name = 'hip'

    def __init__(self):
        L.require_gpu()
        self.lib = L.load()

    @staticmethod
    def _st():
        return L.current_stream()

    def zfilter_stats(self, rs, rsq, cnt, eps, mean_out, std_out):
        L.call('smx_zfilter_stats_f32', L.ptr(rs), L.ptr(rsq), L.ptr(cnt), rs.numel(), float(eps),
               L.ptr(mean_out), L.ptr(std_out), self._st())

    def zfilter_forward(self, x_view, mean, std, out):
        rows, D = x_view.shape
        L.call('smx_zfilter_forward_f32', L.ptr(x_view), _row_stride(x_view, D), rows, D,
               L.ptr(mean), L.ptr(std), L.ptr(out), self._st())

    def zfilter_forward_sums(self, x_view, rs, rsq, cnt, eps, out):
        rows, D = x_view.shape
        L.call('smx_zfilter_forward_sums_f32', L.ptr(x_view), _row_stride(x_view, D), rows, D,
               L.ptr(rs), L.ptr(rsq), L.ptr(cnt), float(eps), L.ptr(out), self._st())

    def diaggauss_sample(self, mean, log_var, noise_scale, eps, actions, pd):
        rows, A = mean.shape
        L.call('smx_diaggauss_sample_f32', L.ptr(mean), _row_stride(mean, A), L.ptr(log_var),
               L.ptr(noise_scale), L.ptr(eps), 0 if eps is None else _row_stride(eps, A), rows, A,
               L.ptr(actions), _row_stride(actions, A), L.ptr(pd),
               0 if pd is None else _row_stride(pd, 2 * A), self._st())

    def zfilter_update(self, x_view, rs, rsq, cnt, count_rows, ws=None):
        rows, D = x_view.shape
        if ws is not None:
            L.call('smx_zfilter_update_ws_f32', L.ptr(x_view), _row_stride(x_view, D), rows, D, L.ptr(rs),
                   L.ptr(rsq), L.ptr(cnt), float(count_rows), L.ptr(ws), ws.numel(), self._st())
            return
        L.call('smx_zfilter_update_f32', L.ptr(x_view), _row_stride(x_view, D), rows, D, L.ptr(rs),
               L.ptr(rsq), L.ptr(cnt), float(count_rows), self._st())

    def zfilter_update_ws_floats(self, rows, D):
        return int(self.lib.smx_zfilter_update_ws_floats(int(rows), int(D)))

    def mlp3_packed_numel(self, net):
        nbytes = self.lib.smx_mlp3_packed_bytes(net.D, net.H1, net.H2, net.OUT)
        if nbytes == 0:
            raise L.SmxError('fused MLP kernel does not support D=%d H1=%d H2=%d OUT=%d'
                             % (net.D, net.H1, net.H2, net.OUT))
        return nbytes // 4

    def mlp3_pack(self, net, packed):
        L.call('smx_mlp3_pack_f32', ctypes.byref(net.desc), L.ptr(packed), packed.numel() * 4,
               self._st())

    def mlp3_pack_zstats(self, net, packed, zf):
        L.call('smx_mlp3_pack_zstats_f32', ctypes.byref(net.desc), L.ptr(packed), packed.numel() * 4,
               L.ptr(zf.running_sum), L.ptr(zf.running_sumsq), L.ptr(zf.count), zf.running_sum.numel(),
               float(zf.eps), L.ptr(zf._mean), L.ptr(zf._std), self._st())

    def fused_exact_zfilter(self, on):
        L.call('smx_mlp3_fused_exact_zfilter', 1 if on else 0)

    def mlp3_forward_fused(self, packed, net, x_main, x_tail, zmean, zstd, out, act):
        G, T0, D = x_main.shape
        T1 = 0 if x_tail is None else x_tail.shape[1]
        assert x_main.is_contiguous() and (x_tail is None or x_tail.is_contiguous())
        L.call('smx_mlp3_forward_fused_f32', L.ptr(packed), net.D, net.H1, net.H2, net.OUT,
               L.ptr(x_main), L.ptr(x_tail), G, T0, T1, L.ptr(zmean), L.ptr(zstd), L.ptr(out),
               act, self._st())

    FUSED_ROWS_MIN = 24576

    def mlp3_forward(self, net, x, h1, h2, out, act, stop=None, pack=None):
        assert x.is_contiguous()
        if pack is not None and x.shape[0] >= self.FUSED_ROWS_MIN and h1.is_contiguous() and h2.is_contiguous() and \
                L.load().smx_mlp3_forward_rows_supported(net.D, net.H1, net.H2, net.OUT):
            ld = 0 if out.dim() < 2 or out.stride(0) == out.shape[1] else out.stride(0)
            rc = L.load().smx_mlp3_forward_rows_f32(ctypes.byref(net.desc), L.ptr(x), x.shape[0], L.ptr(h1), L.ptr(h2),
                                                    L.ptr(out), act, ld, L.ptr(pack), pack.numel() * 4, L.ptr(stop), self._st())
            if rc != L.SMX_E_UNSUPPORTED:
                L.check(rc, 'smx_mlp3_forward_rows_f32')
                return
        L.call('smx_mlp3_forward_f32', ctypes.byref(net.desc), L.ptr(x), x.shape[0], L.ptr(h1),
               L.ptr(h2), L.ptr(out), act, L.ptr(stop), self._st())

    def _jobs(self, jobs):
        arr = (L.Mlp3Job * len(jobs))()
        for k, j in enumerate(jobs):
            g = lambda name: L.ptr(j.get(name)) if j.get(name) is not None else None
            arr[k].net = ctypes.pointer(j['net'].desc)
            arr[k].x = g('x')
            arr[k].rows = j['x'].shape[0]
            arr[k].h1, arr[k].h2, arr[k].out = g('h1'), g('h2'), g('out')
            arr[k].out_act = int(j.get('act', 0))
            out = j.get('out')
            arr[k].out_ld = 0 if out is None or out.dim() < 2 or out.stride(0) == out.shape[1] \
                else out.stride(0)
            arr[k].dz3, arr[k].dz2, arr[k].dz1 = g('dz3'), g('dz2'), g('dz1')
            arr[k].grads, arr[k].sumsq_partials = g('grads'), g('sumsq')
            arr[k].stop_flag = g('stop')
            arr[k].h1T, arr[k].h2T, arr[k].xT = g('h1T'), g('h2T'), g('xT')
            arr[k].dz3T, arr[k].dz2T, arr[k].dz1T = g('dz3T'), g('dz2T'), g('dz1T')
            tv = j.get('h1T')
            arr[k].ldT = 0 if tv is None else (tv.stride(0) if tv.shape[0] > 1 else tv.shape[1])
        return arr

    def mlp3_forward_multi(self, jobs):
        L.call('smx_mlp3_forward_multi_f32', self._jobs(jobs), len(jobs), self._st())

    def mlp3_backward_multi(self, jobs):
        L.call('smx_mlp3_backward_multi_f32', self._jobs(jobs), len(jobs), self._st())

    def mlp3_backward_partials(self, net):
        return self.lib.smx_mlp3_backward_partials(net.D, net.H1, net.H2, net.OUT)

    def mlp3_backward(self, net, x, h1, h2, dz3, dz2, dz1, grads, sumsq, stop=None, ws=None, packT=None, dx=None):
        if ws is not None and sumsq is None and packT is not None and x.shape[0] >= self.FUSED_ROWS_MIN and \
                dz2.is_contiguous() and dz1.is_contiguous() and (dx is None or dx.is_contiguous()):
            rc = L.load().smx_mlp3_backward_rows_f32(
                ctypes.byref(net.desc), L.ptr(x), L.ptr(h1), L.ptr(h2), L.ptr(dz3), x.shape[0], L.ptr(dz2), L.ptr(dz1),
                L.ptr(dx), L.ptr(grads), L.ptr(ws), ws.numel(), L.ptr(packT), packT.numel(), L.ptr(stop), self._st())
            if rc != L.SMX_E_UNSUPPORTED:
                L.check(rc, 'smx_mlp3_backward_rows_f32')
                return dx is not None
        if ws is not None and sumsq is None:
            L.call('smx_mlp3_backward_splitk_f32', ctypes.byref(net.desc), L.ptr(x), L.ptr(h1), L.ptr(h2),
                   L.ptr(dz3), x.shape[0], L.ptr(dz2), L.ptr(dz1), L.ptr(grads), L.ptr(ws), ws.numel(),
                   L.ptr(stop), self._st())
            return False
        L.call('smx_mlp3_backward_f32', ctypes.byref(net.desc), L.ptr(x), L.ptr(h1), L.ptr(h2),
               L.ptr(dz3), x.shape[0], L.ptr(dz2), L.ptr(dz1), L.ptr(grads), L.ptr(sumsq),
               L.ptr(stop), self._st())

    def mlp3_backward_ws_floats(self, net, rows):
        return int(self.lib.smx_mlp3_backward_ws_floats(net.D, net.H1, net.H2, net.OUT, int(rows)))

    def mlp3_dgrad_rows_ws_floats(self, net):
        return int(self.lib.smx_mlp3_dgrad_rows_ws_floats(net.D, net.H1, net.H2, net.OUT))

    def epoch_supported(self, *nets):
        ok = all(self.lib.smx_epoch_supported(n.D, n.H1, n.H2, n.OUT) for n in nets)
        return bool(ok and self.lib.smx_epoch_supported(max(n.D for n in nets), max(n.H1 for n in nets),
                                                        max(n.H2 for n in nets), max(n.OUT for n in nets)))

    def epoch_blocks(self, rows):
        return self.lib.smx_epoch_blocks(rows)

    def epoch_packed_numel(self, net):
        return self.lib.smx_epoch_packed_floats(net.D, net.H1, net.H2, net.OUT)

    def epoch_pack(self, items):
        arr = (L.EpochPack * len(items))()
        for k, (net, packed) in enumerate(items):
            arr[k].net = ctypes.pointer(net.desc)
            arr[k].packed = L.ptr(packed)
        L.call('smx_epoch_pack_f32', arr, len(items), self._st())

    def epoch_prepare(self, obs0, xn, xnT, xr, zmean=None, zstd=None, ref_filter=None, obs_next=None, xnext=None,
                      ref_log_var=None, ref_std=None, pack=(), zero_words=None):
        rows, D = obs0.shape
        a = L.EpochPrep()
        a.obs0, a.ld_obs0, a.rows, a.D = L.ptr(obs0), _row_stride(obs0, D), rows, D
        a.zmean, a.zstd = L.ptr(zmean), L.ptr(zstd)
        a.xn, a.xnT = L.ptr(xn), L.ptr(xnT)
        a.ldT = 0 if xnT is None else (xnT.stride(0) if xnT.shape[0] > 1 else xnT.shape[1])
        if ref_filter is not None:
            a.ref_sum, a.ref_sumsq, a.ref_count = L.ptr(ref_filter.running_sum), L.ptr(ref_filter.running_sumsq), \
                L.ptr(ref_filter.count)
            a.ref_eps, a.ref_filter = float(ref_filter.eps), 1
        a.xr = L.ptr(xr)
        if xnext is not None:
            a.obs_next, a.ld_next, a.xnext = L.ptr(obs_next), _row_stride(obs_next, D), L.ptr(xnext)
        if ref_std is not None:
            A = ref_std.shape[1]
            a.A, a.ref_log_var, a.ref_std, a.ld_ref = A, L.ptr(ref_log_var), L.ptr(ref_std), _row_stride(ref_std, A)
        if zero_words is not None:
            a.zero_words, a.n_zero = L.ptr(zero_words), zero_words.numel()
        a.n_pack = len(pack)
        for k, (net, packed) in enumerate(pack):
            a.pack[k].net = ctypes.pointer(net.desc)
            a.pack[k].packed = L.ptr(packed)
        L.call('smx_epoch_prepare_f32', ctypes.byref(a), self._st())

    _EPOCH_LOSS = {None: L.EPOCH_LOSS_NONE, 'policy': L.EPOCH_LOSS_POLICY, 'value': L.EPOCH_LOSS_VALUE,
                   'rhs_surr': L.EPOCH_RHS_SURR, 'rhs_kl': L.EPOCH_RHS_KL}

    def _epoch_jobs(self, jobs):
        arr = (L.EpochJob * len(jobs))()
        for k, j in enumerate(jobs):
            g = lambda name: L.ptr(j.get(name)) if j.get(name) is not None else None
            x = j['x']
            assert x.is_contiguous()
            arr[k].net = ctypes.pointer(j['net'].desc)
            arr[k].x, arr[k].rows = L.ptr(x), x.shape[0]
            arr[k].h1T, arr[k].h2T = g('h1T'), g('h2T')
            tv = j.get('h1T')
            arr[k].ldT = 0 if tv is None else (tv.stride(0) if tv.shape[0] > 1 else tv.shape[1])
            out = j.get('out')
            arr[k].out = g('out')
            arr[k].out_ld = 0 if out is None or out.dim() < 2 or out.stride(0) == out.shape[1] else out.stride(0)
            arr[k].out_act = int(j.get('act', 0))
            arr[k].loss = self._EPOCH_LOSS[j.get('loss')]
            arr[k].stop_flag = g('stop')
            arr[k].dz3, arr[k].dz3T, arr[k].dz2T, arr[k].dz1T = g('dz3'), g('dz3T'), g('dz2T'), g('dz1T')
            arr[k].packed = g('packed')
        return arr

    @staticmethod
    def _epoch_loss(loss):
        if loss is None:
            return None
        a = L.PpoLosses()
        g = lambda name: L.ptr(loss.get(name)) if loss.get(name) is not None else None
        a.mode = int(loss.get('mode', 0))
        if loss.get('log_var') is not None:
            A = loss['log_var'].numel()
            a.A, a.rows = A, int(loss['rows'])
            a.log_var, a.adv = g('log_var'), g('adv')
            if loss.get('actions') is not None:
                a.actions, a.ld_act = g('actions'), _row_stride(loss['actions'], A)
                a.behave, a.ld_beh = g('behave'), _row_stride(loss['behave'], 2 * A)
                a.ref, a.ld_ref = g('ref'), _row_stride(loss['ref'], 2 * A)
            a.g_surr, a.g_kl, a.row_partials = g('g_surr'), g('g_kl'), g('partials')
            a.check_stop, a.will_update = int(loss.get('check_stop', 0)), int(loss.get('will_update', 0))
            a.dlogvar, a.dlogvar_sumsq, a.stats = g('dlogvar'), g('dlogvar_sumsq'), g('stats')
        a.returns, a.v_dz3, a.v_partials = g('returns'), g('v_dz3'), g('v_partials')
        a.v_will_update = int(loss.get('v_will_update', 0))
        return ctypes.byref(a)

    def epoch_forward(self, jobs, loss=None, ctrl=None, n_total=0):
        L.call('smx_epoch_forward_f32', self._epoch_jobs(jobs), len(jobs), self._epoch_loss(loss),
               L.ptr(ctrl), int(n_total), self._st())

    def epoch_backward(self, jobs, loss, ctrl, n_total):
        L.call('smx_epoch_backward_f32', self._epoch_jobs(jobs), len(jobs), self._epoch_loss(loss),
               L.ptr(ctrl), int(n_total), self._st())

    def epoch_fwdbwd_supported(self, *nets):
        return bool(all(self.lib.smx_epoch_fwdbwd_supported(n.D, n.H1, n.H2, n.OUT) for n in nets) and
                    self.lib.smx_epoch_fwdbwd_supported(max(n.D for n in nets), max(n.H1 for n in nets),
                                                        max(n.H2 for n in nets), max(n.OUT for n in nets)))

    def epoch_fwdbwd(self, jobs, loss, ctrl, n_total, sync_word, kl_slots):
        L.call('smx_epoch_fwdbwd_f32', self._epoch_jobs(jobs), len(jobs), self._epoch_loss(loss),
               L.ptr(ctrl), int(n_total), L.ptr(sync_word), L.ptr(kl_slots), self._st())

    def layernorm_forward(self, x, gamma, beta, eps, y, mean=None, rstd=None):
        rows, F = x.shape
        L.call('smx_layernorm_forward_f32', L.ptr(x), x.stride(0), rows, F, L.ptr(gamma), L.ptr(beta), float(eps), L.ptr(y),
               y.stride(0), L.ptr(mean), L.ptr(rstd), self._st())

    def layernorm_backward_ws_floats(self, rows, F):
        return int(self.lib.smx_layernorm_backward_ws_floats(int(rows), int(F)))

    def layernorm_backward(self, dy, x, mean, rstd, gamma, dx, dgamma, dbeta, ws, relu_mask=False):
        rows, F = x.shape
        L.call('smx_layernorm_backward_f32', L.ptr(dy), dy.stride(0), L.ptr(x), x.stride(0), L.ptr(mean), L.ptr(rstd),
               L.ptr(gamma), rows, F, int(bool(relu_mask)), L.ptr(dx), dx.stride(0), L.ptr(dgamma), L.ptr(dbeta), L.ptr(ws),
               ws.numel(), self._st())

    def device_occupy(self, blocks, microseconds):
        L.call('smx_device_occupy', int(blocks), int(microseconds), self._st())

    def mlp3_wgrad_multi(self, jobs):
# ... 510 lines not shown
```

### surreal_amd/learner/ppo.py

```python
import gc
import types

import numpy as np
import torch

from surreal_amd import _lib as L
from surreal_amd import kernels as KN
from surreal_amd.learner.aggregator import MultistepAggregatorWithInfo
from surreal_amd.learner.base import Learner, DeferredStats
from surreal_amd.model.ppo_net import DiagGauss, PPOModel


class LinearWithMinLR(object):

    def __init__(self, initial_lr, num_updates, update_freq=1, min_lr=0.0):
        self.initial_lr = float(initial_lr)
        self.num_updates = max(int(num_updates), 1)
        self.update_freq = max(int(update_freq), 1)
        self.min_lr = float(min_lr)
        self.n = 0
        self.lr = float(initial_lr)

    def get_lr(self):
        return [self.lr]
# ... 275 lines not shown
            rounds(B * (N + 1)) > rounds(B * N) and not stem
        ws.xnext = f(B, D)
        ws.h1t, ws.h2t = f(B, cri.H1), f(B, cri.H2)
        ws.adv = f(B * E)
        ws.ret = f(B * E)
        idx = torch.tensor(range(N), dtype=torch.float32)
        ws.gpow = torch.pow(self.gamma, idx).to(dev)
        ws.lpow = torch.pow(self.lam, idx).to(dev)
        ws.mom_parts = f(self.world_size, 3)
        rows = B * E
        ws.rows = rows
        Dx = self.model.stem_in
        ws.xn = f(rows, Dx)
        ws.xr = f(rows, Dx)
        ws.h1a, ws.h2a, ws.mean = f(rows, act.H1), f(rows, act.H2), f(rows, A)
        ws.h1r, ws.h2r, ws.ref_mean = f(rows, act.H1), f(rows, act.H2), f(rows, A)
        ws.ref_pol = f(rows, 2 * A)
        ws.h1c, ws.h2c, ws.vpred = f(rows, cri.H1), f(rows, cri.H2), f(rows)
        ws.g_surr, ws.g_kl, ws.dz3a = f(rows, A), f(rows, A), f(rows, A)
        ws.dz2a, ws.dz1a = f(rows, act.H2), f(rows, act.H1)
        ws.dz3c, ws.dz2c, ws.dz1c = f(rows), f(rows, cri.H2), f(rows, cri.H1)
        if stem:
            R1 = B * (N + 1)
            ws.h0 = ws.c0 = ws.cnn_it = ws.cnn_gae = ws.frames_it = None
            ws.low_it = f(rows, D)
            ws.act_it, ws.beh_it = f(rows, A), f(rows, 2 * A)
            ws.ztmp = f(R1, D)
            ws.lcat, ws.xcat = f(B, N + 1, D), f(R1, Dx)
            ws.h1G, ws.h2G = f(R1, cri.H1), f(R1, cri.H2)
            n_sk = max(K.mlp3_backward_ws_floats(n, rows) for n in (act, cri))
            ws.mlp_sk = f(n_sk) if n_sk else None
            try:
                ws.pack_stem = f(max(K.mlp3_packed_numel(n) for n in (act, cri)))
            except Exception:
                ws.pack_stem = None
            n_z = K.zfilter_update_ws_floats(rows, D)
            ws.zscratch = f(n_z) if n_z else None
            n_pt = max(K.mlp3_dgrad_rows_ws_floats(n) for n in (act, cri))
            ws.packT_stem = f(n_pt) if n_pt else None
            if rnn:
                F = self.model.rnn_hidden
                nl = self.model.rnn_layers
                ws.h0L, ws.c0L = f(nl, B, F), f(nl, B, F)
                ws.h0, ws.c0 = ws.h0L[0], ws.c0L[0]
                ws.gates, ws.lo, ws.cs, ws.hp, ws.dlo = f(rows, 4 * F), f(rows, F), f(rows, F), f(rows, F), f(rows, F)
                ws.gatesG, ws.loG, ws.csG = f(R1, 4 * F), f(R1, F), f(R1, F)
                ws.upper = [types.SimpleNamespace(gates=f(rows, 4 * F), lo=f(rows, F), cs=f(rows, F),
                                                  hp=f(rows, F), dlo=f(rows, F)) for _ in range(nl - 1)]
                ws.loG2 = f(R1, F) if nl > 1 else None
                n_sk = max(K.lstm_backward_ws_floats(r, B, E) for r in self.model.rnns)
                ws.lstm_sk = f(n_sk) if n_sk else None
            if pixel:
                from surreal_amd.model.cnn_stem import CnnStem
                cnn = self.model.cnn
                cam = (cnn.C, cnn.H, cnn.W)
                ws.frames_it = torch.empty((rows,) + cam, device=dev, dtype=pix_dtype)
                ws.fcat = torch.empty((B, N + 1) + cam, device=dev, dtype=pix_dtype)
                ws.dxn = torch.zeros(rows, Dx, device=dev)
                chunk = int(self.session_config.learner.get('cnn_chunk_frames', 2048))
                ws.cnn_it = CnnStem.workspace(cnn, rows, dev, backward=True)
                ws.cnn_it.sk = self.model._cnn_stem.splitk_workspace(cnn, rows, dev)
                ws.cnn_gae = ws.cnn_it if rows >= min(chunk, R1) else \
                    CnnStem.workspace(cnn, min(chunk, R1), dev, backward=False)
        else:
            ldT = rows + 16
            ft = lambda n: torch.zeros(n, ldT, device=dev, dtype=torch.float32)[:, :rows]
            ws.xnT = ft(D)
            ws.h1aT, ws.h2aT, ws.dz3aT = ft(act.H1), ft(act.H2), ft(A)
            ws.dz2aT, ws.dz1aT = ft(act.H2), ft(act.H1)
            ws.h1cT, ws.h2cT, ws.dz3cT = ft(cri.H1), ft(cri.H2), ft(1)
            ws.dz2cT, ws.dz1cT = ft(cri.H2), ft(cri.H1)
        n_a, n_c = self.model.actor_flat.numel(), self.model.critic_flat.numel()
        ws.nblk_p = K.loss_blocks(rows)
        ws.fused = (self.fused_epochs and not stem and
                    (self.world_size == 1 or self.epoch_policy == self.epoch_baseline) and
                    K.epoch_supported(act, cri))
        ws.fb = (ws.fused and self.world_size == 1 and bool(self.session_config.learner.get('fused_fwdbwd', True)) and
                 bool(self.session_config.learner.get('exclusive_device', True)) and not getattr(self, '_fb_timed_out', False) and
                 n_slots > 0 and K.epoch_fwdbwd_supported(act, cri))
        vblocks = K.epoch_blocks if ws.fused else K.value_loss_blocks
        ws.nblk_v = vblocks(rows)
        ws.merged_tail = ws.fused and self.world_size == 1
        ws.ticket = torch.zeros(2, dtype=torch.int32, device=dev)
        if ws.fused:
            assert ws.nblk_p == K.epoch_blocks(rows)
            ws.pk_actor = torch.zeros(K.epoch_packed_numel(act), device=dev)
            ws.pk_critic = torch.zeros(K.epoch_packed_numel(cri), device=dev)
            ws.pk_ref = torch.zeros(K.epoch_packed_numel(act), device=dev)
        ws.pstride = 8 + 2 * A
        ws.n_total, ws.B_total, nblk_p_all = rows, B, ws.nblk_p
        if self.world_size > 1:
            mine = torch.tensor([rows, B], dtype=torch.int64, device=dev)
            every = torch.empty(2 * self.world_size, dtype=torch.int64, device=dev)
            self._dist.all_gather_into_tensor(every, mine)
            every = every.view(-1, 2).tolist()
            ws.n_total, ws.B_total = sum(r for r, _ in every), sum(b for _, b in every)
            ws.nblk_v = max(vblocks(r) for r, _ in every)
            nblk_p_all = max(K.loss_blocks(r) for r, _ in every)
        ws.dp_epoch = self.world_size > 1 and not stem
        ws.tail_deferred = ws.dp_epoch and self.epoch_policy >= self.epoch_baseline
        if ws.dp_epoch:
            al = lambda n: (n + 3) & ~3
            adapt = self.ppo_mode != 'clip'
            off_k = al(n_a + n_c)
            off_p = off_k + (al(act.numel) if adapt else 0)
            ws.ar = torch.zeros(off_p + nblk_p_all * ws.pstride, device=dev)
            ws.grads_all = ws.ar[:n_a + n_c]
            ws.grads_k = ws.ar[off_k:off_k + act.numel] if adapt else None
            ws.ppart_ar = ws.ar[off_p:].view(nblk_p_all, ws.pstride)
            if adapt:
                ws.dz3k, ws.dz2k, ws.dz1k = f(rows, A), f(rows, act.H2), f(rows, act.H1)
                ws.dz3kT, ws.dz2kT, ws.dz1kT = ft(A), ft(act.H2), ft(act.H1)
                ws.sumsq_k = torch.zeros(K.mlp3_backward_partials(act), device=dev)
            nz = 2 * D + 1 if self.use_z_filter else 0
            cuts = np.cumsum([0, ws.pstride, Ev * ws.nblk_v * 8, 3, nz]).tolist()
            ws.tail_cuts = cuts
            ws.tail_pack = torch.zeros(cuts[-1], device=dev)
            ws.tail_gather = f(self.world_size, cuts[-1])
            ws.tp_ppart = ws.tail_pack[:cuts[1]].view(1, ws.pstride)
            ws.vpart_loc_all = ws.tail_pack[cuts[1]:cuts[2]].view(Ev, ws.nblk_v, 8)
            ws.tp_ret = ws.tail_pack[cuts[2]:cuts[3]]
            ws.zsum = f(nz) if nz else None
        else:
            ws.grads_all = torch.zeros(n_a + n_c, device=dev)
        ws.grads_a, ws.grads_c = ws.grads_all[:n_a], ws.grads_all[n_a:]
        ws.ppart = f(ws.nblk_p, ws.pstride)
        ws.ppart_sum = f(1, ws.pstride)
        ws.ppart_fold = f(64, ws.pstride)
        ws.stem_one_exchange = bool(stem and self.world_size > 1 and self.ppo_mode == 'clip' and
                                    self.session_config.learner.get('stem_one_exchange', True))
        if ws.stem_one_exchange:
            ws.ar_pol = torch.zeros(((n_a + 3) & ~3) + ws.pstride, device=dev)
            ws.grads_a = ws.ar_pol[:n_a]
            ws.ppart_sum = ws.ar_pol[(n_a + 3) & ~3:].view(1, ws.pstride)
        ws.vpart = torch.zeros(Ev, self.world_size * ws.nblk_v, 8, device=dev)
        ws.vpart_local = torch.zeros(ws.nblk_v, 8, device=dev)
        if not ws.dp_epoch:
            ws.vpart_loc_all = torch.zeros(Ev, ws.nblk_v, 8, device=dev)
        ws.vgather = f(self.world_size, Ev, ws.nblk_v, 8)
        ws.np_a = K.mlp3_backward_partials(act)
        ws.np_c = K.mlp3_backward_partials(cri)
        ws.sumsq_a = torch.zeros(max(ws.np_a + 1, K.sumsq_blocks(ws.grads_a.numel())), device=dev)
        ws.sumsq_c = torch.zeros(max(ws.np_c, K.sumsq_blocks(ws.grads_c.numel())), device=dev)
        if self.use_z_filter:
            ws.zdelta = ws.tail_pack[ws.tail_cuts[3]:] if ws.dp_epoch else torch.zeros(2 * D + 1, device=dev)
        ws.xerr = ws.ctrl_i[L.C_XCHG_ERR:L.C_XCHG_ERR + 1]
        if self.world_size > 1:
            self._setup_peer_exchange(ws, n_a + n_c)
        self._ws = ws
        self._graphs = {}
        return ws

    def _setup_peer_exchange(self, ws, n_grads):
        d = self._dist
        d.err_word = ws.xerr
        want = bool(self.session_config.learner.get('peer_exchange', True)) and self.device != 'cpu'
        need = max(ws.ar.numel() if ws.dp_epoch else n_grads, 64)
        if getattr(ws, 'tail_gather', None) is not None:
            need = max(need, ws.tail_gather.numel())
        if not want:
            return
        if d.exchange is not None and d.exchange.capacity >= need:
            return
        if d.exchange is not None:
            d._d.barrier()
            d.exchange.close()
            d.exchange = None
        from surreal_amd.distributed.peer_exchange import PeerExchange
        d.exchange = PeerExchange.create(d._d, need, timeout_s=float(self.session_config.learner.get(
            'peer_exchange_timeout_s', 5.0)))
        self.exchange_kind = 'peer buffers (%s)' % d.exchange.check_message if d.exchange is not None else 'process group'

    def _to_dev(self, x):
        if torch.is_tensor(x):
            return x.to(self.device, torch.float32)
        return torch.as_tensor(np.asarray(x), dtype=torch.float32).to(self.device)

    def _to_dev_pixels(self, x):
        if not torch.is_tensor(x):
            x = torch.as_tensor(np.asarray(x))
        if x.dtype != torch.uint8:
            x = x.to(torch.float32)
        return x.to(self.device)

    def _preprocess_batch_ppo(self, batch):
        obs, obs_next = batch['obs'], batch['obs_next']
        for modality in obs:
            for key in obs[modality]:
                conv = self._to_dev_pixels if modality == 'pixel' else self._to_dev
                obs[modality][key] = conv(obs[modality][key])
                obs_next[modality][key] = conv(obs_next[modality][key])
        batch['actions'] = self._to_dev(batch['actions'])
        batch['rewards'] = self._to_dev(batch['rewards'])
        batch['dones'] = self._to_dev(batch['dones'])
        if batch.get('persistent_infos') is not None:
            batch['persistent_infos'] = [self._to_dev(x) for x in batch['persistent_infos']]
        if batch.get('onetime_infos') is not None:
            batch['onetime_infos'] = [self._to_dev(x) for x in batch['onetime_infos']]
        return batch

    def _flat_obs(self, obs):
        parts = [obs['low_dim'][k] for k in obs['low_dim'].keys()]
        x = parts[0] if len(parts) == 1 else torch.cat(parts, -1)
        return x.contiguous()

    def _enqueue_gae(self, ws, obs, obs_next, rewards, dones):
        tail = self._enqueue_critic_pass(ws, obs, obs_next)
        if tail is not None:
            self.K.mlp3_forward_multi([tail])
        self._enqueue_gae_from_values(ws, obs, rewards, dones)

    def _enqueue_critic_pass(self, ws, obs, obs_next, filter_tail=True):
        K, m = self.K, self.model
        B, N, D = obs.shape
        zm = zs = None
        if self.use_z_filter:
            K.mlp3_pack_zstats(m.critic, ws.packed, m.z_filter)
            zm, zs = m.z_filter._mean, m.z_filter._std
        else:
            K.mlp3_pack(m.critic, ws.packed)
        if not ws.split_tail:
            K.mlp3_forward_fused(ws.packed, m.critic, obs, obs_next, zm, zs, ws.vals, L.SMX_ACT_NONE)
            return None
        K.mlp3_forward_fused(ws.packed, m.critic, obs, None, zm, zs, ws.vals[:B * N], L.SMX_ACT_NONE)
        if not filter_tail:
            pass
        elif self.use_z_filter:
            K.zfilter_forward(obs_next[:, 0, :], zm, zs, ws.xnext)
        else:
            ws.xnext.copy_(obs_next[:, 0, :])
        return dict(net=m.critic, x=ws.xnext, h1=ws.h1t, h2=ws.h2t, out=ws.vals[B * N:].view(B, 1),
                    act=L.SMX_ACT_NONE)

    def _enqueue_gae_from_values(self, ws, obs, rewards, dones):
        K = self.K
        B, N, D = obs.shape
        if ws.merged_tail and self.norm_adv:
            K.gae_norm(ws.vals[:B * N] if ws.split_tail else ws.vals, rewards, dones, ws.gpow, ws.lpow, self.gamma,
                       self.gamma ** N, B, N, N, ws.adv, ws.ret, ws.adv_mom, 1e-4, ws.ticket[0:1],
                       values_tail=ws.vals[B * N:] if ws.split_tail else None)
            return
        if ws.split_tail:
            K.gae(ws.vals[:B * N], rewards, dones, ws.gpow, ws.lpow, self.gamma, self.gamma ** N,
                  B, N, N, ws.adv, ws.ret, values_tail=ws.vals[B * N:])
        else:
            K.gae(ws.vals, rewards, dones, ws.gpow, ws.lpow, self.gamma, self.gamma ** N, B, N, N,
                  ws.adv, ws.ret)
        if self.norm_adv:
            K.moments(ws.adv, ws.adv_mom)
            if self.world_size > 1:
                self._dist.all_gather_into_tensor(ws.mom_parts.view(-1), ws.adv_mom.clone())
                K.moments_merge(ws.mom_parts, ws.adv_mom)
            K.adv_normalize(ws.adv, ws.adv_mom, 1e-4)

    def _enqueue_lockstep_epochs(self, ws, actions0, behave0, first_extra=(), after_first=None):
        K, m = self.K, self.model
        Ep, Ev = self.epoch_policy, self.epoch_baseline
        mode = L.SMX_PPO_CLIP if self.ppo_mode == 'clip' else L.SMX_PPO_ADAPT
        A = self.action_dim
        W = self.world_size
        n_total = ws.n_total
        aj = dict(net=m.actor, x=ws.xn, h1=ws.h1a, h2=ws.h2a, out=ws.mean, act=L.SMX_ACT_TANH,
                  dz3=ws.dz3a, dz2=ws.dz2a, dz1=ws.dz1a, grads=ws.grads_a, sumsq=ws.sumsq_a,
                  stop=ws.stop, xT=ws.xnT, h1T=ws.h1aT, h2T=ws.h2aT, dz3T=ws.dz3aT, dz2T=ws.dz2aT,
                  dz1T=ws.dz1aT)
        cj = dict(net=m.critic, x=ws.xn, h1=ws.h1c, h2=ws.h2c, out=ws.vpred.view(-1, 1),
                  act=L.SMX_ACT_NONE, dz3=ws.dz3c.view(-1, 1), dz2=ws.dz2c, dz1=ws.dz1c,
                  grads=ws.grads_c, sumsq=ws.sumsq_c, xT=ws.xnT, h1T=ws.h1cT, h2T=ws.h2cT,
                  dz3T=ws.dz3c, dz2T=ws.dz2cT, dz1T=ws.dz1cT)
        for e in range(max(Ep + 1, Ev)):
            pol_f, pol_u, val = e <= Ep, e < Ep, e < Ev
            K.mlp3_forward_multi(([aj] if pol_f else []) + ([cj] if val else []) +
                                 (list(first_extra) if e == 0 else []))
            if e == 0 and after_first is not None:
                after_first()
            if ws.dp_epoch and pol_u and val:
                self._enqueue_dp_epoch(ws, e, mode, aj, cj, actions0, behave0)
                continue
            if pol_f and W == 1:
                K.epoch_losses(mode, ws.mean, m.log_var.view(-1), actions0, behave0, ws.ref_pol, ws.adv,
                               ws.ctrl_f, ws.g_surr, ws.g_kl, ws.ppart, e > 0, pol_u, ws.dz3a,
                               ws.grads_a[m.actor.numel:m.actor.numel + A],
                               ws.sumsq_a[ws.np_a:ws.np_a + 1], ws.pstats[e], dz3_t=ws.dz3aT,
                               values=ws.vpred if val else None, returns=ws.ret, v_dz3=ws.dz3c,
                               v_partials=ws.vpart[e] if val else None)
            elif pol_f and ws.tail_deferred and not pol_u and not val:
                K.policy_loss(mode, ws.mean, m.log_var.view(-1), actions0, behave0, ws.ref_pol,
                              ws.adv, ws.ctrl_f, ws.g_surr, ws.g_kl, ws.ppart)
                torch.sum(ws.ppart, 0, keepdim=True, out=ws.tp_ppart)
                continue
            elif pol_f:
                K.policy_loss(mode, ws.mean, m.log_var.view(-1), actions0, behave0, ws.ref_pol,
                              ws.adv, ws.ctrl_f, ws.g_surr, ws.g_kl, ws.ppart)
                part, nblk = ws.ppart, ws.nblk_p
                if W > 1:
                    torch.sum(ws.ppart, 0, keepdim=True, out=ws.ppart_sum)
                    self._dist.all_reduce(ws.ppart_sum)
                    part, nblk = ws.ppart_sum, 1
                K.policy_finalize(mode, part, nblk, ws.g_surr, ws.g_kl, m.log_var.view(-1), n_total,
                                  ws.ctrl_f, e > 0, pol_u, ws.dz3a,
                                  ws.grads_a[m.actor.numel:m.actor.numel + A],
                                  ws.sumsq_a[ws.np_a:ws.np_a + 1], ws.pstats[e], dz3_t=ws.dz3aT)
            if val and not (pol_f and W == 1):
                K.value_loss(ws.vpred, ws.ret, n_total, ws.dz3c,
                             ws.vpart_loc_all[e] if W > 1 else ws.vpart[e], ws.ctrl_f, True)
            if pol_u or val:
                K.mlp3_backward_multi(([aj] if pol_u else []) + ([cj] if val else []))
            np_a, np_c = ws.np_a + 1, ws.np_c
            if W > 1:
                if pol_u and val:
                    if self.rank != 0:
                        ws.grads_a[m.actor.numel:m.actor.numel + A].zero_()
                    self._dist.all_reduce(ws.grads_all)
                elif pol_u:
                    self._dist.all_reduce(ws.grads_a[:m.actor.numel])
# ... 124 lines not shown
        if not ws.merged_tail:
            K.value_finalize(ws.vpart, Ev, ws.vpart.shape[1], ws.vstats, L.VS_STRIDE)

    def _enqueue_tail_exchange(self, ws, obs0, actions0, behave0):
        K, m, W = self.K, self.model, self.world_size
        Ep, Ev, D = self.epoch_policy, self.epoch_baseline, obs0.shape[1]
        mode = L.SMX_PPO_CLIP if self.ppo_mode == 'clip' else L.SMX_PPO_ADAPT
        c = ws.tail_cuts
        K.moments(ws.ret, ws.tp_ret)
        if self.use_z_filter:
            ws.zdelta.zero_()
            K.zfilter_update(obs0, ws.zdelta[:D], ws.zdelta[D:2 * D], ws.zdelta[2 * D:], obs0.shape[0])
        self._dist.all_gather_into_tensor(ws.tail_gather.view(-1), ws.tail_pack)
        G = ws.tail_gather
        torch.sum(G[:, :c[1]], 0, keepdim=True, out=ws.ppart_sum)
        K.policy_finalize(mode, ws.ppart_sum, 1, ws.g_surr, ws.g_kl, m.log_var.view(-1), ws.n_total,
                          ws.ctrl_f, Ep > 0, False, ws.dz3a,
                          ws.grads_a[m.actor.numel:m.actor.numel + self.action_dim],
                          ws.sumsq_a[ws.np_a:ws.np_a + 1], ws.pstats[Ep], dz3_t=ws.dz3aT)
        ws.vpart.view(Ev, W, ws.nblk_v, 8).copy_(G[:, c[1]:c[2]].reshape(W, Ev, ws.nblk_v, 8).permute(1, 0, 2, 3))
        K.value_finalize(ws.vpart, Ev, ws.vpart.shape[1], ws.vstats, L.VS_STRIDE)
        ws.mom_parts.copy_(G[:, c[2]:c[3]])
        K.moments_merge(ws.mom_parts, ws.ret_mom)
        if self.use_z_filter:
            torch.sum(G[:, c[3]:], 0, out=ws.zsum)
            m.z_filter.running_sum += ws.zsum[:D]
            m.z_filter.running_sumsq += ws.zsum[D:2 * D]
            m.z_filter.count += ws.zsum[2 * D:]

    def _enqueue_dp_epoch(self, ws, e, mode, aj, cj, actions0, behave0):
        K, m = self.K, self.model
        adapt = mode == L.SMX_PPO_ADAPT
        self._clear_foreign_partials(ws)
        K.epoch_losses_dp(mode, ws.mean, m.log_var.view(-1), actions0, behave0, ws.ref_pol, ws.adv,
                          ws.ctrl_f, ws.dz3a, ws.dz3k if adapt else ws.g_kl, ws.ppart_ar, ws.n_total,
                          g_surr_t=ws.dz3aT, g_kl_t=ws.dz3kT if adapt else None, values=ws.vpred,
                          returns=ws.ret, v_dz3=ws.dz3c, v_partials=ws.vpart_loc_all[e])
        jobs = [aj]
        if adapt:
            jobs.append(dict(aj, dz3=ws.dz3k, dz2=ws.dz2k, dz1=ws.dz1k, grads=ws.grads_k,
                             sumsq=ws.sumsq_k, dz3T=ws.dz3kT, dz2T=ws.dz2kT, dz1T=ws.dz1kT))
        K.mlp3_backward_multi(jobs + [cj])
        self._dist.all_reduce(ws.ar)
        K.epoch_combine(mode, ws.ppart_ar, ws.ppart_ar.shape[0], ws.n_total, m.log_var.view(-1), ws.ctrl_f,
                        e > 0, True, ws.pstats[e], ws.grads_a, ws.grads_k if adapt else None,
                        m.actor.numel, ws.sumsq_a, ws.grads_c, ws.sumsq_c)
        K.clip_adam_pair((m.actor_flat, ws.grads_a, self.actor_exp_avg, self.actor_exp_avg_sq,
                          ws.sumsq_a, K.sumsq_blocks(ws.grads_a.numel()), True,
                          ws.pstats[e, L.PS_GRADNORM:L.PS_GRADNORM + 1]),
                         (m.critic_flat, ws.grads_c, self.critic_exp_avg, self.critic_exp_avg_sq,
                          ws.sumsq_c, K.sumsq_blocks(ws.grads_c.numel()), False,
                          ws.vstats[e, L.VS_GRADNORM:L.VS_GRADNORM + 1]),
                         ws.ctrl_f)

    def _enqueue_reward_filter(self, ws, rewards):
        K = self.K
        if self.world_size == 1 or not self.use_r_filter:
            K.reward_filter(rewards, self.reward_scale, ws.rf_state, 1e-5, ws.rew, ws.rf_part, ws.rf_ticket,
                            use_filter=self.use_r_filter, update=self.use_r_filter)
            return ws.rew
        K.reward_filter(rewards, self.reward_scale, ws.rf_state, 1e-5, ws.rew, ws.rf_part, ws.rf_ticket,
                        use_filter=True, update=False, sums=ws.rf_sums)
        self._dist.all_reduce(ws.rf_sums)
        ws.rf_state[:2] += ws.rf_sums[:2]
        ws.rf_state[2:] = ws.rf_sums[2:]
        return ws.rew

    def _enqueue_optimize(self, ws, obs, obs_next, actions, rewards, dones, pds, pix=None,
                          pix_next=None):
        pre_zeroed = self.filter_rewards and self.use_r_filter and self.world_size > 1
        if pre_zeroed:
            ws.zero_block.zero_()
        if self.filter_rewards:
            rewards = self._enqueue_reward_filter(ws, rewards)
        if self.if_rnn_policy or self.model.if_pixel:
            return self._enqueue_optimize_stem(ws, obs, obs_next, actions, rewards, dones, pds, pix,
                                               pix_next, pre_zeroed)
        K, m, ref = self.K, self.model, self.ref_target_model
        B, N, D = obs.shape
        A = self.action_dim
        fused = ws.fused
        if not fused and not pre_zeroed:
            ws.zero_block.zero_()
        tail = self._enqueue_critic_pass(ws, obs, obs_next, filter_tail=not fused)

        obs0 = obs[:, 0, :]
        actions0 = actions[:, 0, :]
        behave0 = pds[:, 0, :]
        if fused:
            zf = m.z_filter if self.use_z_filter else None
            K.epoch_prepare(obs0, ws.xn, ws.xnT, ws.xr, zmean=zf._mean if zf else None, zstd=zf._std if zf else None,
                            ref_filter=ref.z_filter if self.use_z_filter else None,
                            obs_next=obs_next[:, 0, :] if tail is not None else None,
                            xnext=ws.xnext if tail is not None else None,
                            ref_log_var=ref.log_var.view(-1), ref_std=ws.ref_pol[:, A:],
                            pack=[(m.actor, ws.pk_actor), (m.critic, ws.pk_critic), (ref.actor, ws.pk_ref)],
                            zero_words=None if pre_zeroed else ws.zero_block.view(torch.int32))
        elif self.use_z_filter:
            zm, zs = m.z_filter._mean, m.z_filter._std
            K.zfilter_forward(obs0, zm, zs, ws.xn)
            rz = ref.z_filter
            K.zfilter_forward_sums(obs0, rz.running_sum, rz.running_sumsq, rz.count, rz.eps, ws.xr)
        else:
            ws.xn.copy_(obs0)
            ws.xr.copy_(obs0)
        ref_job = dict(net=ref.actor, x=ws.xr, h1=ws.h1r, h2=ws.h2r, out=ws.ref_pol[:, :A],
                       act=L.SMX_ACT_TANH)
        if not fused:
            ws.xnT.copy_(ws.xn.t())
            ws.ref_pol[:, A:].copy_(torch.exp(ref.log_var).expand(ws.rows, A))
        if fused:
            self._enqueue_fused_epochs(ws, actions0, behave0, ref_job, tail,
                                       lambda: self._enqueue_gae_from_values(ws, obs, rewards, dones))
        else:
            self._enqueue_lockstep_epochs(
                ws, actions0, behave0, first_extra=[ref_job] + ([tail] if tail is not None else []),
                after_first=lambda: self._enqueue_gae_from_values(ws, obs, rewards, dones))

        if ws.tail_deferred:
            self._enqueue_tail_exchange(ws, obs0, actions0, behave0)
            self._enqueue_final_stats(ws)
            return
        if fused and ws.merged_tail:
            K.learn_epilogue(ws.ret, ws.ret_mom, m.log_var.view(-1), ws.fin, ws.ticket[1:2],
                             zfilter=m.z_filter if self.use_z_filter else None, x=obs0, count_rows=B,
                             v_partials=ws.vpart, n_epochs=self.epoch_baseline, nblk=ws.vpart.shape[1],
                             v_stats=ws.vstats, stats_stride=L.VS_STRIDE)
            return
        K.moments(ws.ret, ws.ret_mom)
        if self.world_size > 1:
            self._dist.all_gather_into_tensor(ws.mom_parts.view(-1), ws.ret_mom.clone())
            K.moments_merge(ws.mom_parts, ws.ret_mom)
        if self.use_z_filter:
            if self.world_size > 1:
                ws.zdelta.zero_()
                K.zfilter_update(obs0, ws.zdelta[:D], ws.zdelta[D:2 * D], ws.zdelta[2 * D:], B)
                self._dist.all_reduce(ws.zdelta)
                m.z_filter.running_sum += ws.zdelta[:D]
                m.z_filter.running_sumsq += ws.zdelta[D:2 * D]
                m.z_filter.count += ws.zdelta[2 * D:]
            else:
                K.zfilter_update(obs0, m.z_filter.running_sum, m.z_filter.running_sumsq,
                                 m.z_filter.count, B)
        self._enqueue_final_stats(ws)

    def _stem_inputs(self, ws, mm, low2d, frames, xin, cnn_ws, zstats, stop=None):
        K = self.K
        D = low2d.shape[1]
        if zstats is not False:
            if self.use_z_filter:
                K.zfilter_forward(low2d, zstats[0], zstats[1], ws.ztmp[:low2d.shape[0]])
                xin[:, :D].copy_(ws.ztmp[:low2d.shape[0]])
            else:
                xin[:, :D].copy_(low2d)
        if frames is not None:
            nF = frames.shape[0]
            tag = (getattr(ws, 'frames_epoch', 0), frames.data_ptr(), nF) if nF <= cnn_ws.F else None
            for f0 in range(0, nF, cnn_ws.F):
                f1 = min(nF, f0 + cnn_ws.F)
                mm._cnn_stem.forward(mm.cnn, frames[f0:f1], f1 - f0, cnn_ws, xin[f0:f1, D:], stop, cols1_tag=tag)

    def _enqueue_gae_stem(self, ws, obs, obs_next, pix, pix_next, rewards, dones):
        K, m = self.K, self.model
        B, N, D = obs.shape
        rnn = self.if_rnn_policy
        ws.lcat[:, :N].copy_(obs)
        ws.lcat[:, N:].copy_(obs_next)
        frames = None
        if m.if_pixel:
            ws.fcat[:, :N].copy_(pix)
            ws.fcat[:, N:].copy_(pix_next)
            frames = ws.fcat.view((B * (N + 1),) + tuple(ws.fcat.shape[2:]))
        zst = m.z_filter.refresh_stats() if self.use_z_filter else None
        self._stem_inputs(ws, m, ws.lcat.view(B * (N + 1), D), frames, ws.xcat, ws.cnn_gae, zst)
        x = ws.xcat
        if rnn:
            x = self._lstm_forward_only(ws, m, ws.xcat, B, N + 1, ws.gatesG, ws.csG, ws.loG, ws.loG2)
        K.mlp3_forward(m.critic, x, ws.h1G, ws.h2G, ws.vals.view(-1, 1), L.SMX_ACT_NONE, pack=ws.pack_stem)
        H = self.horizon if rnn else N
        K.gae(ws.vals, rewards, dones, ws.gpow, ws.lpow, self.gamma, self.gamma ** H, B, N, H,
              ws.adv, ws.ret)
        if self.norm_adv:
            K.moments(ws.adv, ws.adv_mom)
            if self.world_size > 1:
                self._dist.all_gather_into_tensor(ws.mom_parts.view(-1), ws.adv_mom.clone())
                K.moments_merge(ws.mom_parts, ws.adv_mom)
            K.adv_normalize(ws.adv, ws.adv_mom, 1e-4)

    def _lstm_forward_only(self, ws, mm, xin, B, T, gates, cs, lo_a, lo_b):
        x, out, other = xin, lo_a, lo_b
        for layer, rnn in enumerate(mm.rnns):
            self.K.lstm_forward(rnn, x, B, T, ws.h0L[layer], ws.c0L[layer], gates, out, cs)
            x, out, other = out, other, out
        return x

    def _stem_forward(self, ws, mm, xin, stop, save=True):
# ... 450 lines not shown
```

Baseline: 122.0 million.

## Fold critic packing and z-stats into epoch prepare; fuse critic forward with GAE

Moves the critic weight packing and z-filter mean/std computation into the existing epoch_prepare kernel, so these no longer need separate launches. It also adds a fused critic-forward plus GAE plus advantage-normalization kernel that uses a last-block ticket, and it is used when the tail is split, the tail is merged, and advantages are normalized. The aim is to cut kernel launches and round trips of values through global memory in the learner step. Existing pack and GAE helpers are refactored into shared include headers. The cost is extra complexity and a fallback path when the fused variant is unsupported.

```diff
diff --git a/include/surreal_amd.h b/include/surreal_amd.h
--- a/include/surreal_amd.h
+++ b/include/surreal_amd.h
@@ -62,6 +62,12 @@
                                int64_t G, int32_t T0, int32_t T1, const float* zmean,
                                const float* zstd, float* out, int32_t out_act,
                                smx_stream_t stream);
+int smx_mlp3_forward_fused_gae_f32(const float* packed, int32_t D, int32_t H1, int32_t H2, const float* x,
+                                   int32_t B, int32_t N, const float* zmean, const float* zstd, float* values,
+                                   const float* values_tail, const float* rewards, const float* dones,
+                                   const float* gamma_pow, const float* lam_pow, float gamma, float gamma_H,
+                                   float* adv, float* ret, float* adv_moments, float min_std, int32_t* ticket,
+                                   smx_stream_t stream);
 
 int smx_linear_f32(const float* A, int32_t lda, int32_t a_kcontig, const float* B,
                    int32_t ldb, int32_t b_kcontig, const float* bias, float* C,
@@ -302,6 +308,9 @@
     const float* ref_log_var; float* ref_std; int64_t ld_ref;
     int32_t* zero_words; int32_t n_zero; int32_t n_pack;
     smx_epoch_pack_t pack[4];
+    const smx_mlp3_t* critic; float* critic_packed; int64_t critic_packed_bytes;
+    const float* z_sum; const float* z_sumsq; const float* z_count; float z_eps; int32_t z_stats;
+    float* zmean_out; float* zstd_out;
 } smx_epoch_prep_t;
 int smx_epoch_prepare_f32(const smx_epoch_prep_t* args, smx_stream_t stream);
 struct smx_ppo_losses;
diff --git a/surreal_amd/_lib.py b/surreal_amd/_lib.py
--- a/surreal_amd/_lib.py
+++ b/surreal_amd/_lib.py
@@ -55,7 +55,10 @@
                 ('ref_sum', c_void_p), ('ref_sumsq', c_void_p), ('ref_count', c_void_p), ('ref_eps', c_float),
                 ('ref_filter', c_int32), ('xr', c_void_p), ('obs_next', c_void_p), ('ld_next', c_int64),
                 ('xnext', c_void_p), ('ref_log_var', c_void_p), ('ref_std', c_void_p), ('ld_ref', c_int64),
-                ('zero_words', c_void_p), ('n_zero', c_int32), ('n_pack', c_int32), ('pack', EpochPack * 4)]
+                ('zero_words', c_void_p), ('n_zero', c_int32), ('n_pack', c_int32), ('pack', EpochPack * 4),
+                ('critic', POINTER(Mlp3)), ('critic_packed', c_void_p), ('critic_packed_bytes', c_int64),
+                ('z_sum', c_void_p), ('z_sumsq', c_void_p), ('z_count', c_void_p), ('z_eps', c_float),
+                ('z_stats', c_int32), ('zmean_out', c_void_p), ('zstd_out', c_void_p)]
 
 
 EPOCH_LOSS_NONE, EPOCH_LOSS_POLICY, EPOCH_LOSS_VALUE, EPOCH_RHS_SURR, EPOCH_RHS_KL = 0, 1, 2, 3, 4
@@ -169,6 +172,8 @@
     'smx_mlp3_fused_exact_zfilter': (c_int32, [c_int32]),
     'smx_mlp3_forward_fused_f32': (c_int32, [_P, c_int32, c_int32, c_int32, c_int32, _P, _P,
                                              c_int64, c_int32, c_int32, _P, _P, _P, c_int32, _P]),
+    'smx_mlp3_forward_fused_gae_f32': (c_int32, [_P, c_int32, c_int32, c_int32, _P, c_int32, c_int32, _P, _P, _P, _P,
+                                                 _P, _P, _P, _P, c_float, c_float, _P, _P, _P, c_float, _P, _P]),
     'smx_linear_f32': (c_int32, [_P, c_int32, c_int32, _P, c_int32, c_int32, _P, _P, c_int32,
                                  c_int32, c_int32, c_int32, c_int32, _P, _P, _P]),
     'smx_linear_wgrad_f32': (c_int32, [_P, c_int32, _P, c_int32, _P, c_int32, _P, c_int32, c_int32,
diff --git a/surreal_amd/csrc/smx_epoch.hip b/surreal_amd/csrc/smx_epoch.hip
--- a/surreal_amd/csrc/smx_epoch.hip
+++ b/surreal_amd/csrc/smx_epoch.hip
@@ -1,4 +1,5 @@
 #include "smx_common.h"
+#include "smx_mlp3_fused.inc.h"
 #include <stdlib.h>
 #include <string.h>
 
@@ -792,6 +793,11 @@
     int* zero_words; int n_zero;
     PackArgs pack;
     long n_x, n_std;
+    const float *zsum, *zsumsq, *zcount; float zeps; int zstats;
+    float *zmean_out, *zstd_out;
+    long n_zout;
+    smx_mlp3_t critic; float* cpacked; PackLayout cl; int cnt1, cnt2;
+    long n_cpack;
 };
 
 __device__ __forceinline__ float zclamp_e(float x, float m, float sdev) {
@@ -804,7 +810,8 @@
     const long tid0 = (long)blockIdx.x * 256 + threadIdx.x, stride = (long)gridDim.x * 256;
     for (long i = tid0; i < P.n_zero; i += stride) P.zero_words[i] = 0;
     const long nx = P.n_x, n_next = P.xnext ? nx : 0;
-    const long total = 2 * nx + n_next + P.n_std + P.pack.total;
+    const long n_front = 2 * nx + n_next + P.n_std + P.pack.total;
+    const long total = n_front + P.n_zout + P.n_cpack;
     for (long i = tid0; i < total; i += stride) {
         if (i < 2 * nx + n_next) {
             const int which = i < nx ? 0 : (i < 2 * nx ? 1 : 2);
@@ -824,7 +831,13 @@
                 }
                 P.xr[e] = v;
             } else {
-                if (P.zmean) v = zclamp_e(x, P.zmean[k], P.zstd[k]);
+                if (P.zstats) {
+                    float m, sd;
+                    zfilter_stat(P.zsum, P.zsumsq, P.zcount, P.zeps, k, m, sd);
+                    v = zclamp_e(x, m, sd);
+                } else if (P.zmean) {
+                    v = zclamp_e(x, P.zmean[k], P.zstd[k]);
+                }
                 if (which == 0) {
                     P.xn[e] = v;
                     if (P.xnT) P.xnT[(size_t)k * P.ldT + r] = v;
@@ -837,8 +850,14 @@
             const long r = e / P.A;
             const int a = (int)(e - r * P.A);
             P.ref_std[r * P.ld_ref + a] = expf(P.ref_log_var[a]);
+        } else if (i < n_front) {
+            pack_word(P.pack, i - (2 * nx + n_next + P.n_std));
+        } else if (i < n_front + P.n_zout) {
+            const int k = (int)(i - n_front);
+            zfilter_stat(P.zsum, P.zsumsq, P.zcount, P.zeps, k, P.zmean_out[k], P.zstd_out[k]);
         } else {
-            pack_word(P.pack, i - (2 * nx + n_next + P.n_std));
+            const size_t j = (size_t)(i - n_front - P.n_zout);
+            P.cpacked[j] = mlp3_pack_value(P.critic, P.cl, P.cnt1, P.cnt2, j);
         }
     }
 }
@@ -888,6 +907,9 @@
     SMX_REQUIRE(!a->xnext || (a->obs_next && a->ld_next >= a->D), SMX_E_SHAPE);
     SMX_REQUIRE(!a->ref_std || (a->ref_log_var && a->A > 0 && a->ld_ref >= a->A), SMX_E_SHAPE);
     SMX_REQUIRE(a->n_zero >= 0 && a->n_zero <= (1 << 20) && (a->n_zero == 0 || a->zero_words), SMX_E_SHAPE);
+    SMX_REQUIRE(!a->z_stats || (a->z_sum && a->z_sumsq && a->z_count && a->zmean_out && a->zstd_out), SMX_E_NULL);
+    SMX_REQUIRE(!a->z_stats || !a->zmean, SMX_E_SHAPE);
+    SMX_REQUIRE(!a->critic_packed || a->critic, SMX_E_NULL);
     PrepArgs P;
     memset(&P, 0, sizeof(P));
     P.obs0 = a->obs0; P.ld_obs0 = (long)a->ld_obs0; P.rows = (long)a->rows; P.D = a->D;
@@ -904,7 +926,23 @@
         const int rc = fill_pack(P.pack, a->pack, a->n_pack);
         if (rc) return rc;
     }
-    const long total = 2 * P.n_x + (P.xnext ? P.n_x : 0) + P.n_std + P.pack.total;
+    if (a->z_stats) {
+        P.zsum = a->z_sum; P.zsumsq = a->z_sumsq; P.zcount = a->z_count; P.zeps = a->z_eps; P.zstats = 1;
+        P.zmean_out = a->zmean_out; P.zstd_out = a->zstd_out;
+        P.n_zout = a->D;
+    }
+    if (a->critic_packed) {
+        const smx_mlp3_t& c = *a->critic;
+        SMX_REQUIRE(c.W1 && c.b1 && c.W2 && c.b2 && c.W3 && c.b3, SMX_E_NULL);
+        SMX_REQUIRE(c.D > 0 && c.H1 > 0 && c.H2 > 0 && c.OUT > 0, SMX_E_SHAPE);
+        SMX_REQUIRE(c.OUT <= 32 && pick_variant(c.H1, c.H2, &P.cnt1, &P.cnt2), SMX_E_UNSUPPORTED);
+        P.cl = pack_layout(P.cnt1, P.cnt2, (c.D + 31) / 32);
+        SMX_REQUIRE(a->critic_packed_bytes >= (int64_t)(P.cl.total * sizeof(float)), SMX_E_WORKSPACE);
+        SMX_REQUIRE(((uintptr_t)a->critic_packed & 15) == 0, SMX_E_ALIGN);
+        P.critic = c; P.cpacked = a->critic_packed;
+        P.n_cpack = (long)P.cl.total;
+    }
+    const long total = 2 * P.n_x + (P.xnext ? P.n_x : 0) + P.n_std + P.pack.total + P.n_zout + P.n_cpack;
     long blocks = (total + 255) / 256;
     if (blocks > 4096) blocks = 4096;
     hipLaunchKernelGGL(epoch_prepare_kernel, dim3((unsigned)blocks), dim3(256), 0, smx_s(stream), P);
diff --git a/surreal_amd/csrc/smx_gae.inc.h b/surreal_amd/csrc/smx_gae.inc.h
--- /dev/null
+++ b/surreal_amd/csrc/smx_gae.inc.h
@@ -0,0 +1,130 @@
+#pragma once
+
+
+__device__ __forceinline__ void gae_row_stage(float* Vm, float* R, const float* v, bool has_tail, float vt,
+                                              const float* __restrict__ r, const float* __restrict__ d, int N,
+                                              int lane) {
+    const int vlast = has_tail ? N - 1 : N;
+    for (int t0 = 0; t0 <= N; t0 += 256) {
+        float xv[4], dv[4], rv[4];
+#pragma unroll
+        for (int i = 0; i < 4; ++i) {
+            const int t = t0 + lane + 64 * i;
+            xv[i] = v[t < vlast ? t : vlast];
+            dv[i] = d[t >= 1 ? (t - 1 < N ? t - 1 : N - 1) : 0];
+            rv[i] = r[t < N ? t : N - 1];
+        }
+#pragma unroll
+        for (int i = 0; i < 4; ++i) {
+            const int t = t0 + lane + 64 * i;
+            if (t <= N) {
+                float x = (has_tail && t == N) ? vt : xv[i];
+                if (t >= 1) x = x * (1.0f - dv[i]);
+                Vm[t] = x;
+                if (t < N) R[t] = rv[i];
+            }
+        }
+    }
+}
+
+__device__ __forceinline__ void gae_row_delta(const float* Vm, const float* R, float* Dl, float gamma, int N, int lane) {
+    for (int t = lane; t < N; t += 64) {
+        float gv = gamma * Vm[t + 1];
+        float s = R[t] + gv;
+        Dl[t] = s - Vm[t];
+    }
+}
+
+__device__ __forceinline__ void gae_row_out(const float* Vm, const float* R, const float* Dl, const float* __restrict__ gpow,
+                                            const float* __restrict__ lpow, float gamma_H, int N, int H, long b, int lane,
+                                            float* __restrict__ adv, float* __restrict__ ret) {
+    const int E = N - H + 1;
+    if (E == 1) {
+        float rs = 0.f, as = 0.f;
+        for (int k = lane; k < N; k += 64) {
+            rs += gpow[k] * R[k];
+            as += (Dl[k] * gpow[k]) * lpow[k];
+        }
+        rs = smx_wave_sum(rs);
+        as = smx_wave_sum(as);
+        if (lane == 0) {
+            ret[b] = rs + Vm[N] * gamma_H;
+            adv[b] = as;
+        }
+    } else {
+        for (int s = lane; s < E; s += 64) {
+            float rs = 0.f, as = 0.f;
+            for (int k = 0; k < H; ++k) {
+                rs += gpow[k] * R[s + k];
+                as += (Dl[s + k] * gpow[k]) * lpow[k];
+            }
+            ret[(size_t)b * E + s] = rs + Vm[s + H] * gamma_H;
+            adv[(size_t)b * E + s] = as;
+        }
+    }
+}
+
+__device__ __forceinline__ bool last_block_done(int* ticket) {
+    __shared__ int is_last;
+    __syncthreads();
+    if (threadIdx.x == 0) {
+        __builtin_amdgcn_fence(__ATOMIC_RELEASE, "agent");
+        const int t = atomicAdd(ticket, 1);
+        is_last = (t == (int)gridDim.x - 1);
+        if (is_last) {
+            *ticket = 0;
+            __builtin_amdgcn_fence(__ATOMIC_ACQUIRE, "agent");
+        }
+    }
+    __syncthreads();
+    return is_last != 0;
+}
+
+__device__ __forceinline__ void block_moments(const float* __restrict__ x, long n, float* __restrict__ out, int nthr) {
+    __shared__ double red[16];
+    __shared__ double bc;
+    const int lane = threadIdx.x & 63, w = threadIdx.x >> 6, nw = nthr >> 6;
+    const bool in = (int)threadIdx.x < nthr;
+    double s = 0.0;
+    if (in)
+        for (long i = threadIdx.x; i < n; i += nthr) s += (double)__builtin_nontemporal_load(x + i);
+    s = smx_wave_sum_d(s);
+    if (lane == 0 && in) red[w] = s;
+    __syncthreads();
+    if (threadIdx.x == 0) {
+        double t = 0.0;
+        for (int i = 0; i < nw; ++i) t += red[i];
+        bc = t / (double)n;
+    }
+    __syncthreads();
+    const double mean = bc;
+    double q = 0.0;
+    if (in)
+        for (long i = threadIdx.x; i < n; i += nthr) {
+            const double d = (double)__builtin_nontemporal_load(x + i) - mean;
+            q += d * d;
+        }
+    q = smx_wave_sum_d(q);
+    __syncthreads();
+    if (lane == 0 && in) red[w] = q;
+    __syncthreads();
+    if (threadIdx.x == 0) {
+        double t = 0.0;
+        for (int i = 0; i < nw; ++i) t += red[i];
+        out[0] = (float)n;
+        out[1] = (float)mean;
+        out[2] = (float)t;
+        bc = t;
+    }
+    __syncthreads();
+}
+
+constexpr int GAE_NORM_THREADS = 256;
+__device__ __forceinline__ void adv_normalize_block(float* __restrict__ adv, long n, float* __restrict__ norm_mom,
+                                                    float min_std) {
+    block_moments(adv, n, norm_mom, GAE_NORM_THREADS);
+    const float cnt = (float)n, mean = norm_mom[1], m2 = norm_mom[2];
+    const float stdv = sqrtf(m2 / (cnt - 1.0f));
+    const float den = (min_std > stdv) ? min_std : stdv;
+    for (long i = threadIdx.x; i < n; i += blockDim.x) adv[i] = (__builtin_nontemporal_load(adv + i) - mean) / den;
+}
diff --git a/surreal_amd/csrc/smx_mlp3_fused.hip b/surreal_amd/csrc/smx_mlp3_fused.hip
--- a/surreal_amd/csrc/smx_mlp3_fused.hip
+++ b/surreal_amd/csrc/smx_mlp3_fused.hip
@@ -7,12 +7,6 @@
 
 constexpr int ROWS_PER_WG = 128;
 constexpr int LDS_STRIDE = 36;
-
-inline bool pick_variant(int H1, int H2, int* nt1, int* nt2) {
-    if (H1 <= 64 && H2 <= 64) { *nt1 = 2; *nt2 = 2; return true; }
-    if (H1 <= 320 && H2 <= 224) { *nt1 = 10; *nt2 = 7; return true; }
-    return false;
-}
 
 __device__ __forceinline__ float zf(float x, float m, float s) {
     float v = (x - m) / s;
@@ -421,52 +415,12 @@
 __global__ __launch_bounds__(256) void mlp3_pack_kernel(smx_mlp3_t net, float* __restrict__ packed,
                                                         int NT1, int NT2, int KC1, ZStatsRider Z) {
     if (Z.rs) {
-        for (int k = blockIdx.x * 256 + threadIdx.x; k < Z.D; k += gridDim.x * 256) {
-            const float c = Z.cnt[0];
-            const float m = Z.rs[k] / c;
-            const float var = Z.rsq[k] / c - m * m;
-            float sd = sqrtf(var);
-            if (sd == sd) sd = fmaxf(sd, Z.eps);
-            Z.mean[k] = m;
-            Z.stdv[k] = sd;
-        }
+        for (int k = blockIdx.x * 256 + threadIdx.x; k < Z.D; k += gridDim.x * 256)
+            zfilter_stat(Z.rs, Z.rsq, Z.cnt, Z.eps, k, Z.mean[k], Z.stdv[k]);
     }
     const PackLayout L = pack_layout(NT1, NT2, KC1);
-    for (size_t i = (size_t)blockIdx.x * 256 + threadIdx.x; i < L.total; i += (size_t)gridDim.x * 256) {
-        float v = 0.f;
-        if (i < L.b1) {
-            const size_t e = i - L.w1;
-            const int kk = (int)(e & 31);
-            const size_t rc = e >> 5;
-            const int f = (int)(rc % (size_t)(NT1 * 32)), c = (int)(rc / (size_t)(NT1 * 32));
-            const int k = 32 * c + kk;
-            if (f < net.H1 && k < net.D) v = net.W1[(size_t)f * net.D + k];
-        } else if (i < L.w2) {
-            const int f = (int)(i - L.b1);
-            if (f < net.H1) v = net.b1[f];
-        } else if (i < L.b2) {
-            const size_t e = i - L.w2;
-            const int kk = (int)(e & 31);
-            const size_t rc = e >> 5;
-            const int f = (int)(rc % (size_t)(NT2 * 32)), c = (int)(rc / (size_t)(NT2 * 32));
-            const int k = 32 * c + kk;
-            if (f < net.H2 && k < net.H1) v = net.W2[(size_t)f * net.H1 + k];
-        } else if (i < L.w3) {
-            const int f = (int)(i - L.b2);
-            if (f < net.H2) v = net.b2[f];
-        } else if (i < L.b3) {
-            const size_t e = i - L.w3;
-            const int kk = (int)(e & 31);
-            const size_t rc = e >> 5;
-            const int o = (int)(rc & 31), c = (int)(rc >> 5);
-            const int k = 32 * c + kk;
-            if (o < net.OUT && k < net.H2) v = net.W3[(size_t)o * net.H2 + k];
-        } else {
-            const int o = (int)(i - L.b3);
-            if (o < net.OUT) v = net.b3[o];
-        }
-        packed[i] = v;
-    }
+    for (size_t i = (size_t)blockIdx.x * 256 + threadIdx.x; i < L.total; i += (size_t)gridDim.x * 256)
+        packed[i] = mlp3_pack_value(net, L, NT1, NT2, i);
 }
 
 template <int NT1, int NT2>
@@ -549,19 +503,11 @@
     return pack_launch(net, packed, packed_bytes, Z, stream);
 }
 
-extern "C" int smx_mlp3_forward_fused_f32(const float* packed, int32_t D, int32_t H1, int32_t H2,
-                                          int32_t OUT, const float* x_main, const float* x_tail,
-                                          int64_t G, int32_t T0, int32_t T1, const float* zmean,
-                                          const float* zstd, float* out, int32_t out_act,
-                                          smx_stream_t stream) {
-    SMX_REQUIRE(packed && x_main && out, SMX_E_NULL);
-    SMX_REQUIRE(T1 == 0 || x_tail, SMX_E_NULL);
-    SMX_REQUIRE((zmean == nullptr) == (zstd == nullptr), SMX_E_NULL);
-    SMX_REQUIRE(G > 0 && T0 > 0 && T1 >= 0 && D > 0 && OUT > 0, SMX_E_SHAPE);
-    int nt1, nt2;
-    SMX_REQUIRE(OUT <= 32 && pick_variant(H1, H2, &nt1, &nt2), SMX_E_UNSUPPORTED);
-    SMX_REQUIRE(((uintptr_t)packed & 15) == 0, SMX_E_ALIGN);
+static FusedArgs fused_args(const float* packed, int32_t D, int32_t H1, int32_t H2, int32_t OUT, const float* x_main,
+                            const float* x_tail, int64_t G, int32_t T0, int32_t T1, const float* zmean,
+                            const float* zstd, float* out, int32_t out_act) {
     FusedArgs A;
+    memset(&A, 0, sizeof(A));
     A.packed = packed;
     A.x_main = x_main;
     A.x_tail = x_tail ? x_tail : x_main;
@@ -583,14 +529,63 @@
     A.xvec = (D % 4 == 0) && (((uintptr_t)x_main & 15) == 0) &&
              (T1 == 0 || ((uintptr_t)x_tail & 15) == 0) &&
              (zmean == nullptr || ((((uintptr_t)zmean | (uintptr_t)zstd) & 15) == 0));
+    if (g_exact_zfilter && zmean) A.xvec = 0;
+    return A;
+}
+
+extern "C" int smx_mlp3_forward_fused_f32(const float* packed, int32_t D, int32_t H1, int32_t H2,
+                                          int32_t OUT, const float* x_main, const float* x_tail,
+                                          int64_t G, int32_t T0, int32_t T1, const float* zmean,
+                                          const float* zstd, float* out, int32_t out_act,
+                                          smx_stream_t stream) {
+    SMX_REQUIRE(packed && x_main && out, SMX_E_NULL);
+    SMX_REQUIRE(T1 == 0 || x_tail, SMX_E_NULL);
+    SMX_REQUIRE((zmean == nullptr) == (zstd == nullptr), SMX_E_NULL);
+    SMX_REQUIRE(G > 0 && T0 > 0 && T1 >= 0 && D > 0 && OUT > 0, SMX_E_SHAPE);
+    int nt1, nt2;
+    SMX_REQUIRE(OUT <= 32 && pick_variant(H1, H2, &nt1, &nt2), SMX_E_UNSUPPORTED);
+    SMX_REQUIRE(((uintptr_t)packed & 15) == 0, SMX_E_ALIGN);
+    FusedArgs A = fused_args(packed, D, H1, H2, OUT, x_main, x_tail, G, T0, T1, zmean, zstd, out, out_act);
     if (nt1 == 2) return launch_fused<2, 2>(A, smx_s(stream));
     static const bool force32 = getenv("SMX_FUSED32") != nullptr;
-    if (g_exact_zfilter && zmean) A.xvec = 0;
     if (!force32 && A.xvec) {
         const int rc = smx_rows16_launch(A, H1, H2, smx_s(stream));
         if (rc != SMX_E_UNSUPPORTED) return rc;
     }
     return launch_fused<10, 7>(A, smx_s(stream));
+}
+
+extern "C" int smx_mlp3_forward_fused_gae_f32(const float* packed, int32_t D, int32_t H1, int32_t H2,
+                                              const float* x, int32_t B, int32_t N, const float* zmean,
+                                              const float* zstd, float* values, const float* values_tail,
+                                              const float* rewards, const float* dones, const float* gamma_pow,
+                                              const float* lam_pow, float gamma, float gamma_H, float* adv, float* ret,
+                                              float* adv_moments, float min_std, int32_t* ticket,
+                                              smx_stream_t stream) {
+    SMX_REQUIRE(packed && x && values && values_tail && rewards && dones && gamma_pow && lam_pow && adv && ret &&
+                adv_moments && ticket, SMX_E_NULL);
+    SMX_REQUIRE((zmean == nullptr) == (zstd == nullptr), SMX_E_NULL);
+    SMX_REQUIRE(B > 0 && N > 0 && D > 0, SMX_E_SHAPE);
+    int nt1, nt2;
+    SMX_REQUIRE(pick_variant(H1, H2, &nt1, &nt2), SMX_E_UNSUPPORTED);
+    SMX_REQUIRE(((uintptr_t)packed & 15) == 0, SMX_E_ALIGN);
+    FusedArgs A = fused_args(packed, D, H1, H2, 1, x, nullptr, B, N, 0, zmean, zstd, values, SMX_ACT_NONE);
+    if (nt1 == 2 || !A.xvec || getenv("SMX_FUSED32") != nullptr) return SMX_E_UNSUPPORTED;
+    A.gae.values_tail = values_tail;
+    A.gae.rewards = rewards;
+    A.gae.dones = dones;
+    A.gae.gpow = gamma_pow;
+    A.gae.lpow = lam_pow;
+    A.gae.gamma = gamma;
+    A.gae.gamma_H = gamma_H;
+    A.gae.min_std = min_std;
+    A.gae.B = B;
+    A.gae.N = N;
+    A.gae.adv = adv;
+    A.gae.ret = ret;
+    A.gae.adv_moments = adv_moments;
+    A.gae.ticket = (int*)ticket;
+    return smx_rows16_launch(A, H1, H2, smx_s(stream));
 }
 
 extern "C" int32_t smx_mlp3_forward_rows_supported(int32_t D, int32_t H1, int32_t H2, int32_t OUT) {
@@ -609,6 +604,7 @@
     int rc = smx_mlp3_pack_f32(net, packed, packed_bytes, stream);
     if (rc) return rc;
     FusedArgs A;
+    memset(&A, 0, sizeof(A));
     A.packed = packed;
     A.x_main = x; A.x_tail = x;
     A.zmean = nullptr; A.zstd = nullptr;
diff --git a/surreal_amd/csrc/smx_mlp3_fused.inc.h b/surreal_amd/csrc/smx_mlp3_fused.inc.h
--- a/surreal_amd/csrc/smx_mlp3_fused.inc.h
+++ b/surreal_amd/csrc/smx_mlp3_fused.inc.h
@@ -18,6 +18,13 @@
     float* h2_out;
     int H1, H2, out_ld;
     const int* stop;
+    struct Gae {
+        const float *values_tail, *rewards, *dones, *gpow, *lpow;
+        float gamma, gamma_H, min_std;
+        int B, N;
+        float *adv, *ret, *adv_moments;
+        int* ticket;
+    } gae;
 };
 
 struct PackLayout {
@@ -36,9 +43,65 @@
     return L;
 }
 
+inline bool pick_variant(int H1, int H2, int* nt1, int* nt2) {
+    if (H1 <= 64 && H2 <= 64) { *nt1 = 2; *nt2 = 2; return true; }
+    if (H1 <= 320 && H2 <= 224) { *nt1 = 10; *nt2 = 7; return true; }
+    return false;
+}
+
+__device__ __forceinline__ float mlp3_pack_value(const smx_mlp3_t& net, const PackLayout& L, int NT1, int NT2, size_t i) {
+    float v = 0.f;
+    if (i < L.b1) {
+        const size_t e = i - L.w1;
+        const int kk = (int)(e & 31);
+        const size_t rc = e >> 5;
+        const int f = (int)(rc % (size_t)(NT1 * 32)), c = (int)(rc / (size_t)(NT1 * 32));
+        const int k = 32 * c + kk;
+        if (f < net.H1 && k < net.D) v = net.W1[(size_t)f * net.D + k];
+    } else if (i < L.w2) {
+        const int f = (int)(i - L.b1);
+        if (f < net.H1) v = net.b1[f];
+    } else if (i < L.b2) {
+        const size_t e = i - L.w2;
+        const int kk = (int)(e & 31);
+        const size_t rc = e >> 5;
+        const int f = (int)(rc % (size_t)(NT2 * 32)), c = (int)(rc / (size_t)(NT2 * 32));
+        const int k = 32 * c + kk;
+        if (f < net.H2 && k < net.H1) v = net.W2[(size_t)f * net.H1 + k];
+    } else if (i < L.w3) {
+        const int f = (int)(i - L.b2);
+        if (f < net.H2) v = net.b2[f];
+    } else if (i < L.b3) {
+        const size_t e = i - L.w3;
+        const int kk = (int)(e & 31);
+        const size_t rc = e >> 5;
+        const int o = (int)(rc & 31), c = (int)(rc >> 5);
+        const int k = 32 * c + kk;
+        if (o < net.OUT && k < net.H2) v = net.W3[(size_t)o * net.H2 + k];
+    } else {
+        const int o = (int)(i - L.b3);
+        if (o < net.OUT) v = net.b3[o];
+    }
+    return v;
+}
+
+__device__ __forceinline__ void zfilter_stat(const float* __restrict__ rs, const float* __restrict__ rsq,
+                                             const float* __restrict__ cnt, float eps, int k, float& mean, float& sd) {
+    const float c = cnt[0];
+    const float m = rs[k] / c;
+    const float var = rsq[k] / c - m * m;
+    float s = sqrtf(var);
+    if (s == s) s = fmaxf(s, eps);
+    mean = m;
+    sd = s;
+}
+
 }
 using smxf::FusedArgs;
 using smxf::PackLayout;
 using smxf::pack_layout;
+using smxf::pick_variant;
+using smxf::mlp3_pack_value;
+using smxf::zfilter_stat;
 
 __attribute__((visibility("hidden"))) int smx_rows16_launch(const FusedArgs& A, int H1, int H2, hipStream_t st);
diff --git a/surreal_amd/csrc/smx_mlp3_rows16.hip b/surreal_amd/csrc/smx_mlp3_rows16.hip
--- a/surreal_amd/csrc/smx_mlp3_rows16.hip
+++ b/surreal_amd/csrc/smx_mlp3_rows16.hip
@@ -1,4 +1,5 @@
 #include "smx_mlp3_fused.inc.h"
+#include "smx_gae.inc.h"
 
 namespace {
 
@@ -52,7 +53,7 @@
     *reinterpret_cast<float4*>(dst) = v;
 }
 
-template <int NT1, int NT2, bool OUT1, bool SAVE>
+template <int NT1, int NT2, bool OUT1, bool SAVE, bool GAE = false>
 __global__ __launch_bounds__(NTHR, 1) void mlp3_rows16_kernel(FusedArgs A) {
     constexpr int P1 = (NT1 + 1) / 2, P2 = (NT2 + 1) / 2;
     constexpr int NW1 = (P1 * 32 + 63) / 64, NW2 = (P2 * 32 + 63) / 64;
@@ -70,6 +71,10 @@
     float* w3s = b2s + P2 * 32;
     float* zms = w3s + P2 * 32;
     float* rzl = zms + A.KC1 * 32;
+    float* gvl = rzl + A.KC1 * 32;
+    float* grw = gvl + ROWS16;
+    float* gdn = grw + ROWS16;
+    float* gvt = gdn + ROWS16;
 
     const int tid = threadIdx.x, lane = tid & 63, wv = tid >> 6;
     const int fm = lane & 15, g = lane >> 4;
@@ -111,6 +116,18 @@
         for (int i = tid; i < P2 * 32; i += NTHR) w3s[i] = W3p[(size_t)(i >> 5) * 1024 + (i & 31)];
     } else {
         if (tid < 32) w3s[tid] = A.packed[L.b3 + tid];
+    }
+
+    if constexpr (GAE) {
+        if (tid < ROWS16) {
+            const long r = row0 + tid;
+            const bool ok = r < A.total_rows;
+            grw[tid] = ok ? A.gae.rewards[r] : 0.f;
+            gdn[tid] = ok ? A.gae.dones[r] : 0.f;
+        } else if (tid < ROWS16 + ROWS16 / A.gae.N) {
+            const long b = (long)blockIdx.x * (ROWS16 / A.gae.N) + (tid - ROWS16);
+            gvt[tid - ROWS16] = b < A.gae.B ? A.gae.values_tail[b] : 0.f;
+        }
     }
 
 #define SMX_WLD(src, i) (src)[(srow + 64 * (i)) * 8 + sk8]
@@ -416,6 +433,24 @@
         v += b3v;
         if (A.out_act == SMX_ACT_TANH) v = tanhf(v);
         if (g == 0 && myrow < A.total_rows) A.out[SAVE ? myrow * A.out_ld : myrow] = v;
+        if constexpr (GAE) {
+            const FusedArgs::Gae& G = A.gae;
+            if (g == 0) gvl[wv * 16 + fm] = v;
+            const int N = G.N;
+            const long b = (long)blockIdx.x * (ROWS16 / N) + wv;
+            const bool mine = wv < ROWS16 / N && b < G.B;
+            float* Vm = gvt + 8 + wv * (3 * N + 1);
+            float* R = Vm + (N + 1);
+            float* Dl = R + N;
+            __syncthreads();
+            if (mine)
+                gae_row_stage(Vm, R, gvl + wv * N, true, gvt[wv], grw + wv * N, gdn + wv * N, N, lane);
+            __syncthreads();
+            if (mine) gae_row_delta(Vm, R, Dl, G.gamma, N, lane);
+            __syncthreads();
+            if (mine) gae_row_out(Vm, R, Dl, G.gpow, G.lpow, G.gamma_H, N, N, b, lane, G.adv, G.ret);
+            if (last_block_done(G.ticket)) adv_normalize_block(G.adv, (long)G.B, G.adv_moments, G.min_std);
+        }
     } else {
         f32x4 acc3 = f32x4{0.f, 0.f, 0.f, 0.f}, acc3b = f32x4{0.f, 0.f, 0.f, 0.f};
         {
@@ -463,15 +498,17 @@
 #undef SMX_WST
 }
 
-template <int NT1, int NT2, bool SAVE>
+template <int NT1, int NT2, bool SAVE, bool GAE = false>
 int launch16(const FusedArgs& A, hipStream_t st) {
     constexpr int P1 = (NT1 + 1) / 2, P2 = (NT2 + 1) / 2;
     constexpr int NW1 = (P1 * 32 + 63) / 64, NW2 = (P2 * 32 + 63) / 64;
     constexpr int WR = 64 * (NW1 > NW2 ? NW1 : NW2);
-    const size_t lds = (size_t)(2 * WR * LDS16 + 2 * ROWS16 * LDS16 + P1 * 32 + 2 * P2 * 32 + 2 * A.KC1 * 32) * sizeof(float);
+    const size_t lds = (size_t)(2 * WR * LDS16 + 2 * ROWS16 * LDS16 + P1 * 32 + 2 * P2 * 32 + 2 * A.KC1 * 32 +
+                                (GAE ? 6 * ROWS16 + 16 : 0)) * sizeof(float);
     if (lds > 160 * 1024) return SMX_E_UNSUPPORTED;
     const unsigned grid = (unsigned)((A.total_rows + ROWS16 - 1) / ROWS16);
-    void (*k)(FusedArgs) = (A.OUT == 1) ? mlp3_rows16_kernel<NT1, NT2, true, SAVE> : mlp3_rows16_kernel<NT1, NT2, false, SAVE>;
+    void (*k)(FusedArgs) = GAE ? mlp3_rows16_kernel<NT1, NT2, true, SAVE, GAE>
+                         : (A.OUT == 1) ? mlp3_rows16_kernel<NT1, NT2, true, SAVE> : mlp3_rows16_kernel<NT1, NT2, false, SAVE>;
     hipError_t e = hipFuncSetAttribute((const void*)k, hipFuncAttributeMaxDynamicSharedMemorySize, (int)lds);
     if (e != hipSuccess) return (int)e;
     hipLaunchKernelGGL(k, dim3(grid), dim3(NTHR), lds, st, A);
@@ -484,6 +521,12 @@
 int smx_rows16_launch(const FusedArgs& A, int H1, int H2, hipStream_t st) {
     const bool save = A.h1_out || A.h2_out;
     if (!A.xvec || A.D < 4 || A.OUT > 32 || H1 <= 64 || H2 <= 64 || H1 > 320 || H2 > 224) return SMX_E_UNSUPPORTED;
+    if (A.gae.ticket) {
+        if (save || A.OUT != 1 || A.gae.N < 16 || ROWS16 % A.gae.N != 0 || A.total_rows != (long)A.gae.B * A.gae.N)
+            return SMX_E_UNSUPPORTED;
+        if (H1 <= 304 && H2 <= 208) return launch16<19, 13, false, true>(A, st);
+        return launch16<20, 14, false, true>(A, st);
+    }
     if (save) {
         if ((H1 | H2) & 3) return SMX_E_UNSUPPORTED;
         if (H1 <= 304 && H2 <= 208) return launch16<19, 13, true>(A, st);
diff --git a/surreal_amd/csrc/smx_scan.hip b/surreal_amd/csrc/smx_scan.hip
--- a/surreal_amd/csrc/smx_scan.hip
+++ b/surreal_amd/csrc/smx_scan.hip
@@ -1,5 +1,6 @@
 #include "smx_common.h"
 #include "smx_moments.inc.h"
+#include "smx_gae.inc.h"
 
 __device__ __forceinline__ void gae_body(
     const float* __restrict__ values, const float* __restrict__ values_tail,
@@ -14,68 +15,13 @@
     float* Vm = lds + (size_t)w * per;
     float* R = Vm + (N + 1);
     float* Dl = R + N;
-    if (b < B) {
-        const float* v = values + (size_t)b * (values_tail ? N : N + 1);
-        const float* r = rewards + (size_t)b * N;
-        const float* d = dones + (size_t)b * N;
-        const float vt = values_tail ? values_tail[b] : 0.f;
-        const int vlast = values_tail ? N - 1 : N;
-        for (int t0 = 0; t0 <= N; t0 += 256) {
-            float xv[4], dv[4], rv[4];
-#pragma unroll
-            for (int i = 0; i < 4; ++i) {
-                const int t = t0 + lane + 64 * i;
-                xv[i] = v[t < vlast ? t : vlast];
-                dv[i] = d[t >= 1 ? (t - 1 < N ? t - 1 : N - 1) : 0];
-                rv[i] = r[t < N ? t : N - 1];
-            }
-#pragma unroll
-            for (int i = 0; i < 4; ++i) {
-                const int t = t0 + lane + 64 * i;
-                if (t <= N) {
-                    float x = (values_tail && t == N) ? vt : xv[i];
-                    if (t >= 1) x = x * (1.0f - dv[i]);
-                    Vm[t] = x;
-                    if (t < N) R[t] = rv[i];
-                }
-            }
-        }
-    }
-    __syncthreads();
-    if (b < B) {
-        for (int t = lane; t < N; t += 64) {
-            float gv = gamma * Vm[t + 1];
-            float s = R[t] + gv;
-            Dl[t] = s - Vm[t];
-        }
-    }
-    __syncthreads();
-    if (b < B) {
-    const int E = N - H + 1;
-    if (E == 1) {
-        float rs = 0.f, as = 0.f;
-        for (int k = lane; k < N; k += 64) {
-            rs += gpow[k] * R[k];
-            as += (Dl[k] * gpow[k]) * lpow[k];
-        }
-        rs = smx_wave_sum(rs);
-        as = smx_wave_sum(as);
-        if (lane == 0) {
-            ret[b] = rs + Vm[N] * gamma_H;
-            adv[b] = as;
-        }
-    } else {
-        for (int s = lane; s < E; s += 64) {
-            float rs = 0.f, as = 0.f;
-            for (int k = 0; k < H; ++k) {
-                rs += gpow[k] * R[s + k];
-                as += (Dl[s + k] * gpow[k]) * lpow[k];
-            }
-            ret[(size_t)b * E + s] = rs + Vm[s + H] * gamma_H;
-            adv[(size_t)b * E + s] = as;
-        }
-    }
-    }
+    if (b < B)
+        gae_row_stage(Vm, R, values + (size_t)b * (values_tail ? N : N + 1), values_tail != nullptr,
+                      values_tail ? values_tail[b] : 0.f, rewards + (size_t)b * N, dones + (size_t)b * N, N, lane);
+    __syncthreads();
+    if (b < B) gae_row_delta(Vm, R, Dl, gamma, N, lane);
+    __syncthreads();
+    if (b < B) gae_row_out(Vm, R, Dl, gpow, lpow, gamma_H, N, H, b, lane, adv, ret);
 }
 
 __global__ __launch_bounds__(256) void gae_kernel(
@@ -84,56 +30,6 @@
     const float* __restrict__ lpow, float gamma, float gamma_H, int B, int N, int H,
     float* __restrict__ adv, float* __restrict__ ret) {
     gae_body(values, values_tail, rewards, dones, gpow, lpow, gamma, gamma_H, B, N, H, adv, ret);
-}
-
-__device__ __forceinline__ bool last_block_done(int* ticket) {
-    __shared__ int is_last;
-    __syncthreads();
-    if (threadIdx.x == 0) {
-        __threadfence();
-        const int t = atomicAdd(ticket, 1);
-        is_last = (t == (int)gridDim.x - 1);
-        if (is_last) *ticket = 0;
-        __threadfence();
-    }
-    __syncthreads();
-    return is_last != 0;
-}
-
-__device__ __forceinline__ void block_moments(const float* __restrict__ x, long n, float* __restrict__ out) {
-    __shared__ double red[16];
-    __shared__ double bc;
-    const int lane = threadIdx.x & 63, w = threadIdx.x >> 6, nw = (blockDim.x + 63) >> 6;
-    double s = 0.0;
-    for (long i = threadIdx.x; i < n; i += blockDim.x) s += (double)__builtin_nontemporal_load(x + i);
-    s = smx_wave_sum_d(s);
-    if (lane == 0) red[w] = s;
-    __syncthreads();
-    if (threadIdx.x == 0) {
-        double t = 0.0;
-        for (int i = 0; i < nw; ++i) t += red[i];
-        bc = t / (double)n;
-    }
-    __syncthreads();
-    const double mean = bc;
-    double q = 0.0;
-    for (long i = threadIdx.x; i < n; i += blockDim.x) {
-        const double d = (double)__builtin_nontemporal_load(x + i) - mean;
-        q += d * d;
-    }
-    q = smx_wave_sum_d(q);
-    __syncthreads();
-    if (lane == 0) red[w] = q;
-    __syncthreads();
-    if (threadIdx.x == 0) {
-        double t = 0.0;
-        for (int i = 0; i < nw; ++i) t += red[i];
-        out[0] = (float)n;
-        out[1] = (float)mean;
-        out[2] = (float)t;
-        bc = t;
-    }
-    __syncthreads();
 }
 
 __global__ __launch_bounds__(256) void gae_norm_kernel(
@@ -144,12 +40,7 @@
     int* __restrict__ ticket) {
     gae_body(values, values_tail, rewards, dones, gpow, lpow, gamma, gamma_H, B, N, H, adv, ret);
     if (!last_block_done(ticket)) return;
-    const long n = (long)B * (N - H + 1);
-    block_moments(adv, n, norm_mom);
-    const float cnt = (float)n, mean = norm_mom[1], m2 = norm_mom[2];
-    const float stdv = sqrtf(m2 / (cnt - 1.0f));
-    const float den = (min_std > stdv) ? min_std : stdv;
-    for (long i = threadIdx.x; i < n; i += blockDim.x) adv[i] = (__builtin_nontemporal_load(adv + i) - mean) / den;
+    adv_normalize_block(adv, (long)B * (N - H + 1), norm_mom, min_std);
 }
 
 extern "C" int smx_windowed_gae_returns_f32(const float* values, const float* values_tail,
@@ -620,7 +511,7 @@
         }
         if (blk == 0 && threadIdx.x == 0) P.cnt[0] += P.count_rows;
     } else if (blk == P.nz) {
-        block_moments(P.ret, P.n_ret, P.ret_mom);
+        block_moments(P.ret, P.n_ret, P.ret_mom, blockDim.x);
     } else {
         const int e = (blk - P.nz - 1) * 16 + (threadIdx.x >> 6);
         if (e < P.n_epochs)
diff --git a/surreal_amd/kernels.py b/surreal_amd/kernels.py
--- a/surreal_amd/kernels.py
+++ b/surreal_amd/kernels.py
@@ -13,6 +13,7 @@
 
 class HipKernels(object):
     name = 'hip'
+    folded_critic = True
 
     def __init__(self):
         L.require_gpu()
@@ -81,6 +82,19 @@
         L.call('smx_mlp3_forward_fused_f32', L.ptr(packed), net.D, net.H1, net.H2, net.OUT,
                L.ptr(x_main), L.ptr(x_tail), G, T0, T1, L.ptr(zmean), L.ptr(zstd), L.ptr(out),
                act, self._st())
+
+    def mlp3_forward_fused_gae(self, packed, net, x, zmean, zstd, values, values_tail, rewards, dones, gpow, lpow, gamma,
+                               gamma_H, adv, ret, adv_mom, min_std, ticket):
+        B, N, D = x.shape
+        assert x.is_contiguous()
+        rc = L.load().smx_mlp3_forward_fused_gae_f32(
+            L.ptr(packed), net.D, net.H1, net.H2, L.ptr(x), B, N, L.ptr(zmean), L.ptr(zstd), L.ptr(values),
+            L.ptr(values_tail), L.ptr(rewards), L.ptr(dones), L.ptr(gpow), L.ptr(lpow), float(gamma), float(gamma_H),
+            L.ptr(adv), L.ptr(ret), L.ptr(adv_mom), float(min_std), L.ptr(ticket), self._st())
+        if rc == L.SMX_E_UNSUPPORTED:
+            return False
+        L.check(rc, 'smx_mlp3_forward_fused_gae_f32')
+        return True
 
     FUSED_ROWS_MIN = 24576
 
@@ -170,7 +184,7 @@
         L.call('smx_epoch_pack_f32', arr, len(items), self._st())
 
     def epoch_prepare(self, obs0, xn, xnT, xr, zmean=None, zstd=None, ref_filter=None, obs_next=None, xnext=None,
-                      ref_log_var=None, ref_std=None, pack=(), zero_words=None):
+                      ref_log_var=None, ref_std=None, pack=(), zero_words=None, critic_pack=None, zfilter=None):
         rows, D = obs0.shape
         a = L.EpochPrep()
         a.obs0, a.ld_obs0, a.rows, a.D = L.ptr(obs0), _row_stride(obs0, D), rows, D
@@ -193,6 +207,14 @@
         for k, (net, packed) in enumerate(pack):
             a.pack[k].net = ctypes.pointer(net.desc)
             a.pack[k].packed = L.ptr(packed)
+        if critic_pack is not None:
+            net, packed = critic_pack
+            a.critic, a.critic_packed, a.critic_packed_bytes = ctypes.pointer(net.desc), L.ptr(packed), packed.numel() * 4
+        if zfilter is not None:
+            assert zmean is None and zstd is None
+            a.z_sum, a.z_sumsq, a.z_count = L.ptr(zfilter.running_sum), L.ptr(zfilter.running_sumsq), L.ptr(zfilter.count)
+            a.z_eps, a.z_stats = float(zfilter.eps), 1
+            a.zmean_out, a.zstd_out = L.ptr(zfilter._mean), L.ptr(zfilter._std)
         L.call('smx_epoch_prepare_f32', ctypes.byref(a), self._st())
 
     _EPOCH_LOSS = {None: L.EPOCH_LOSS_NONE, 'policy': L.EPOCH_LOSS_POLICY, 'value': L.EPOCH_LOSS_VALUE,
diff --git a/surreal_amd/learner/ppo.py b/surreal_amd/learner/ppo.py
--- a/surreal_amd/learner/ppo.py
+++ b/surreal_amd/learner/ppo.py
@@ -381,6 +381,8 @@
         ws.nblk_v = vblocks(rows)
         ws.merged_tail = ws.fused and self.world_size == 1
         ws.ticket = torch.zeros(2, dtype=torch.int32, device=dev)
+        ws.critic_gae = False
+        ws.folded_critic = bool(getattr(K, 'folded_critic', False))
         if ws.fused:
             assert ws.nblk_p == K.epoch_blocks(rows)
             ws.pk_actor = torch.zeros(K.epoch_packed_numel(act), device=dev)
@@ -528,8 +530,26 @@
             K.zfilter_forward(obs_next[:, 0, :], zm, zs, ws.xnext)
         else:
             ws.xnext.copy_(obs_next[:, 0, :])
-        return dict(net=m.critic, x=ws.xnext, h1=ws.h1t, h2=ws.h2t, out=ws.vals[B * N:].view(B, 1),
+        return self._critic_tail_job(ws, B, N)
+
+    def _critic_tail_job(self, ws, B, N):
+        return dict(net=self.model.critic, x=ws.xnext, h1=ws.h1t, h2=ws.h2t, out=ws.vals[B * N:].view(B, 1),
                     act=L.SMX_ACT_NONE)
+
+    def _enqueue_critic_gae(self, ws, obs, obs_next, rewards, dones):
+        K, m = self.K, self.model
+        B, N, D = obs.shape
+        zm, zs = (m.z_filter._mean, m.z_filter._std) if self.use_z_filter else (None, None)
+        ws.critic_gae = bool(ws.folded_critic and ws.split_tail and ws.merged_tail and self.norm_adv) and K.mlp3_forward_fused_gae(
+            ws.packed, m.critic, obs, zm, zs, ws.vals[:B * N], ws.vals[B * N:], rewards, dones, ws.gpow, ws.lpow,
+            self.gamma, self.gamma ** N, ws.adv, ws.ret, ws.adv_mom, 1e-4, ws.ticket[0:1])
+        if ws.critic_gae:
+            return
+        if ws.split_tail:
+            K.mlp3_forward_fused(ws.packed, m.critic, obs, None, zm, zs, ws.vals[:B * N], L.SMX_ACT_NONE)
+        else:
+            K.mlp3_forward_fused(ws.packed, m.critic, obs, obs_next, zm, zs, ws.vals, L.SMX_ACT_NONE)
+        self._enqueue_gae_from_values(ws, obs, rewards, dones)
 
     def _enqueue_gae_from_values(self, ws, obs, rewards, dones):
         K = self.K
@@ -820,14 +840,24 @@
         fused = ws.fused
         if not fused and not pre_zeroed:
             ws.zero_block.zero_()
-        tail = self._enqueue_critic_pass(ws, obs, obs_next, filter_tail=not fused)
+        if fused:
+            tail = self._critic_tail_job(ws, B, N) if ws.split_tail else None
+            if not ws.folded_critic:
+                if self.use_z_filter:
+                    K.mlp3_pack_zstats(m.critic, ws.packed, m.z_filter)
+                else:
+                    K.mlp3_pack(m.critic, ws.packed)
+        else:
+            tail = self._enqueue_critic_pass(ws, obs, obs_next)
 
         obs0 = obs[:, 0, :]
         actions0 = actions[:, 0, :]
         behave0 = pds[:, 0, :]
         if fused:
             zf = m.z_filter if self.use_z_filter else None
-            K.epoch_prepare(obs0, ws.xn, ws.xnT, ws.xr, zmean=zf._mean if zf else None, zstd=zf._std if zf else None,
+            fold = dict(zfilter=zf, critic_pack=(m.critic, ws.packed)) if ws.folded_critic else \
+                dict(zmean=zf._mean if zf else None, zstd=zf._std if zf else None)
+            K.epoch_prepare(obs0, ws.xn, ws.xnT, ws.xr, **fold,
                             ref_filter=ref.z_filter if self.use_z_filter else None,
                             obs_next=obs_next[:, 0, :] if tail is not None else None,
                             xnext=ws.xnext if tail is not None else None,
@@ -849,7 +879,7 @@
             ws.ref_pol[:, A:].copy_(torch.exp(ref.log_var).expand(ws.rows, A))
         if fused:
             self._enqueue_fused_epochs(ws, actions0, behave0, ref_job, tail,
-                                       lambda: self._enqueue_gae_from_values(ws, obs, rewards, dones))
+                                       lambda: self._enqueue_critic_gae(ws, obs, obs_next, rewards, dones))
         else:
             self._enqueue_lockstep_epochs(
                 ws, actions0, behave0, first_extra=[ref_job] + ([tail] if tail is not None else []),
```

Result: no change. 121.2 million, median of 6 (-0.6%).
